# renmengye/rec-attend-public

Hardware: AMD Instinct MI355X
Metric: instance-timesteps/sec, full_model forward 512x512 T=16 (whole job; pipelined throughput: 8 batches in flight per GPU, fill and drain of the pipeline inside the timed region; config.lone_batch_* = one sync-bracketed forward) (higher is better)
Workload: dtype f32; 1 GPU; cfg2: CVPPP-arch full_model eval forward, 512x512, T=16, B=8 per GPU, y_out+s_out; arch=cvppp, H=512, W=512, T=16, batch_per_gpu=8, global_batch=8, parallelism=batch-sharded x1, no collective, ranks_in_communicator=1, hip_graph=True, tile_tickets=False, batches_in_flight=8, pipeline_slots=4, batches_per_launch=2, input=resident in HBM, output=left in HBM

## Files before the change

### include/recattend.h

```cpp
#ifndef RECATTEND_H_
#define RECATTEND_H_

#include <stddef.h>
#include <stdint.h>

#ifdef __cplusplus
extern "C" {
#endif

#define RA_E_INVALID (-1)
#define RA_E_SHAPE (-2)
#define RA_E_WORKSPACE (-3)
#define RA_E_HUNG_BFS (-12)
#define RA_E_HUNG_PATH (-13)
#define RA_E_HUNG_FLOW (-14)
#define RA_E_HUNG_EQUALIZE (-15)

#define RA_ABI_VERSION 115
int ra_version(void);
const char *ra_last_error_string(void);

int ra_debug_poison_lds(void *stream);
int ra_debug_park_xcd(int xcd, int n_wg, int lds_bytes, int millis, int *resident, void *stream);

#define RA_PLAN_INTS 24
#define RA_PLAN_FAMILY 0
#define RA_PLAN_FORM 1
#define RA_PLAN_CK 2
#define RA_PLAN_NC 3
#define RA_PLAN_WN 4
#define RA_PLAN_GX 5
#define RA_PLAN_GY 6
#define RA_PLAN_KF 7
#define RA_PLAN_TILE_H 8
#define RA_PLAN_TILE_W 9
#define RA_PLAN_TILES_X 10
#define RA_PLAN_TILES_Y 11
#define RA_PLAN_NTILES 12
#define RA_PLAN_GRID 13
#define RA_PLAN_TILES_MIN 14
#define RA_PLAN_TILES_MAX 15
#define RA_PLAN_XCD_MAP 16
#define RA_PLAN_TICKETS 17
#define RA_PLAN_CMID 18
#define RA_PLAN_SLICES 19
#define RA_PLAN_POOL 20
#define RA_PLAN_FAMILY_K1 1
#define RA_PLAN_FAMILY_CONV8 2
#define RA_PLAN_FAMILY_PAIR 3
#define RA_PLAN_FAMILY_SPLIT 4
#define RA_PLAN_FAMILY_WINO 5
#define RA_PLAN_FAMILY_PAIR_WINO 6
#define RA_PLAN_FORM_SWAP 1
#define RA_PLAN_FORM_SUBPIXEL 2
#define RA_PLAN_FORM_BF16 4
#define RA_PLAN_FORM_MOMENTS 8
#define RA_PLAN_FORM_KXK 16
#define RA_PLAN_FORM_PERSIST 32
#define RA_PLAN_FORM_NPACKED 64
#define RA_PLAN_FORM_CACHED 128
#define RA_PLAN_FORM_SPLIT 256
#define RA_PLAN_FORM_PLANE 512
int ra_conv3x3_plan(int C0, int C1, int B, int Hs, int Ws, int upsample, int KF, int Cout, int pool, int has_plane,
                    int bf16_operands, int moments, int store_flags, int *plan);
int ra_conv_pair_plan(int Cin, int B, int Hs, int Ws, int upsampleA, int CoutA, int CoutB, int poolB, int has_plane,
                      int cache_form, int *plan);
int ra_conv_split_plan(int B, int H, int W, int Cin, int Cout, int pool, int has_plane, int *plan);
int ra_conv_wino_plan(int B, int H, int W, int Cin, int Cout, int pool, int *plan);
int ra_conv_pair_wino_plan(int B, int H, int W, int *plan);
int ra_conv_pair16_plan(int B, int H, int W, int *plan);
#define RA_PASTE_PLAN_INTS 8
#define RA_PASTE_PLAN_KERNEL 0
#define RA_PASTE_PLAN_ROWS 1
#define RA_PASTE_PLAN_GRID_X 2
#define RA_PASTE_PLAN_THREADS 3
#define RA_PASTE_PLAN_LDS 4
#define RA_PASTE_KERNEL_GENERAL 1
#define RA_PASTE_KERNEL_WINDOW 2
int ra_paste_plan(int mode, int B, int H, int W, int Fh, int Fw, int Cp, int pc, int has_canvas, int has_img,
                  size_t y_stride_b, int aligned16, int *plan);

int ra_hungarian_f32(const float *weights, int B, int N, int M, float *matching,
                     float *cover_x, float *cover_y);

size_t ra_hungarian_dev_workspace_bytes(int B, int N, int M);
int ra_hungarian_f32_dev(const float *weights, int B, int N, int M, float *matching,
                         float *cover_x, float *cover_y, int *status_dev, void *ws,
                         size_t ws_bytes, void *stream);

#define RA_CONV_TRANSPOSED 1

int ra_conv_cout_padded(int Cout);
size_t ra_conv_packed_floats(int Cin, int Cout);
int ra_conv_pack_weights(const float *w, int Cin_w, int Cout, int Cin, const int *chan_map,
                         int flags, float *out);
size_t ra_conv_packed_floats_k(int KF, int Cin, int Cout);
int ra_conv_pack_weights_k(const float *w, int KF, int Cin_w, int Cout, int Cin, const int *chan_map, int flags,
                           float *out);
int ra_conv_fold_bn(const float *bias, const float *beta, const float *gamma, const float *mean,
                    const float *var, int Cout, float eps, float *scale, float *shift);

int ra_conv3x3_f32(const float *src0, int C0, const float *src1, int C1, int B, int Hs, int Ws,
                   int upsample, const float *wpacked, const float *scale, const float *shift,
                   int Cout, int relu, int pool, const float *plane, int plane_chan, float *y,
                   void *stream);

int ra_convkxk_f32(const float *src0, int C0, const float *src1, int C1, int B, int Hs, int Ws, int upsample,
                   const float *wpacked, int KF, const float *scale, const float *shift, int Cout, int relu, int pool,
                   const float *plane, int plane_chan, float *y, void *stream);

int ra_conv_wide_supported(int Cin, int Cout);
size_t ra_conv_wide_packed_floats(int Cin, int Cout);
int ra_conv_wide_pack_weights(const float *w, int Cin_w, int Cout, int Cin, const int *chan_map, int flags, float *out);
int ra_conv3x3_wide_f32(const float *src0, int C0, const float *src1, int C1, int B, int Hs, int Ws, int upsample,
                        const float *wpacked, const float *scale, const float *shift, int Cout, int relu, int pool,
                        float *y, void *stream);

int ra_fg_head_f32(const float *logits, size_t npix, int nsc, int no, int quantise, float *y_out, float *d_out,
                   const float *x, int D, float *packed, int Cp, float *canvas_plane, void *stream);

int ra_conv3x3_bf16ops_f32(const float *src0, int C0, const float *src1, int C1, int B, int Hs, int Ws,
                           int upsample, const float *wpacked, const float *scale, const float *shift,
                           int Cout, int relu, int pool, const float *plane, int plane_chan, float *y,
                           void *stream);

int ra_conv3x3_bf16_f32(const void *src0, int C0, const void *src1, int C1, int B, int Hs, int Ws, int upsample,
                        const float *wpacked, const float *scale, const float *shift, int Cout, int relu, int pool, void *y,
                        float *part, size_t part_floats, int *nparts, int store_flags, void *stream);
int ra_bn_act_pool_bf16_f32(const void *u, const float *mean, const float *var, const float *gamma, const float *beta, float eps,
                            int relu, int pool, int B, int H, int W, int C, void *y, int flags, void *stream);
int ra_bn_act_pool_bwd_acc_bf16_f32(const void *u, const void *dy, const float *mean, const float *var, const float *gamma,
                                    const float *beta, float eps, int relu, int pool, int B, int H, int W, int C, float *ws,
                                    size_t ws_floats, float *dgamma, float *dbeta, void *du, float *acc_gamma, float *acc_beta,
                                    int flags, void *stream);
int ra_bn_act_pool_bwd_grouped_bf16_f32(const void *u, const void *dy, const void *const *tabs, int G, float eps, int relu, int pool,
                                        int B, int H, int W, int C, float *ws, size_t ws_floats, float *dgamma, float *dbeta,
                                        void *du, int flags, void *stream);
int ra_conv3x3_wgrad_acc_bf16_f32(const void *x, int Cin, int B, int Hs, int Ws, int upsample, const void *du, int Cout, float *ws,
                                  size_t ws_floats, const int *chan_map, int cin_w, int transposed, float *gw, float *gb, int fmt,
                                  void *stream);

size_t ra_conv3x3_moments_part_floats(int Cout);
int ra_conv3x3_moments_f32(const float *src0, int C0, const float *src1, int C1, int B, int Hs, int Ws,
                           int upsample, const float *wpacked, const float *scale, const float *shift,
                           int Cout, int relu, int bf16_operands, float *y, float *part, size_t part_floats,
                           int *nparts, void *stream);
int ra_bn_moments_from_partials_f32(const float *part, int nparts, int C, float *mean, float *var, void *stream);

int ra_conv_pair_supported(int Cin, int CoutA, int CoutB);
int ra_conv_pair_f32(const float *src, int Cin, int B, int Hs, int Ws, int upsampleA,
                     const float *wpA, const float *scaleA, const float *shiftA, int CoutA, int reluA,
                     const float *wpB, const float *scaleB, const float *shiftB, int CoutB, int reluB,
                     int poolB, const float *plane, int plane_chan, float *y, void *stream);

int ra_conv_split_supported(int Cin, int Cout, int pool, int H, int W);
size_t ra_conv_split_packed_halfs(int Cin, int Cout);
int ra_conv_split_pack_weights(const float *w, int Cin, int Cout, unsigned short *out);
int ra_conv_split_pack_weights_dev(const float *w, int Cin, int Cout, int transposed, unsigned short *out, void *stream);
int ra_conv_split_f32(const float *x, int B, int H, int W, int Cin, const unsigned short *wpacked, const float *scale,
                      const float *shift, int Cout, int relu, int pool, float *y, void *stream);
int ra_conv_split_plane_f32(const float *x, int B, int H, int W, int Cin, const float *plane, int plane_chan,
                            const unsigned short *wpacked, const float *scale, const float *shift, int Cout, int relu, int pool,
                            float *y, void *stream);

int ra_conv_wino_supported(int Cin, int Cout, int pool, int H, int W);
size_t ra_conv_wino_packed_floats(int Cin, int Cout);
int ra_conv_wino_pack_weights(const float *w, int Cin, int Cout, float *out);
int ra_conv_wino_f32(const float *x, int B, int H, int W, int Cin, const float *wpacked,
                     const float *scale, const float *shift, int Cout, int relu, int pool, float *y,
                     void *stream);

int ra_conv_pair_wino_supported(int Cin, int CoutA, int CoutB, int poolB, int H, int W);
int ra_conv_pair_wino_f32(const float *x, int B, int H, int W, const float *wpA, const float *scaleA,
                          const float *shiftA, int reluA, const float *wpB_wino, const float *scaleB,
                          const float *shiftB, int reluB, float *y, void *stream);

int ra_conv_pair16_supported(int Cin, int CoutA, int CoutB, int poolB, int H, int W);
int ra_conv_pair16_f32(const float *x, int B, int H, int W, const float *wpA, const float *scaleA, const float *shiftA,
                       int reluA, const float *wpB, const float *scaleB, const float *shiftB, int reluB, float *y,
                       void *stream);

int ra_conv_first_cache_supported(int Cin, int CoutA, int CoutB, int poolB, int H, int W);
size_t ra_conv_first_cache_floats(int B, int H, int W);
int ra_conv_first_cache_f32(const float *src, int B, int H, int W, const float *wpA, int CoutA,
                            int plane_chan, float *cache, void *stream);
int ra_conv_pair_fill_cache_f32(const float *src, const float *plane, int plane_chan, int B, int H,
                                int W, const float *wpA, const float *scaleA, const float *shiftA,
                                int reluA, const float *wpB, const float *scaleB,
                                const float *shiftB, int CoutB, int reluB, float *cache, float *y,
                                void *stream);
int ra_conv_pair_fill_cache_rider_f32(const float *src, const float *plane, int plane_chan, int B, int H, int W,
                                      const float *wpA, const float *scaleA, const float *shiftA, int reluA,
                                      const float *wpB, const float *scaleB, const float *shiftB, int CoutB,
                                      int reluB, float *cache, float *y, float *fill_dst, size_t fill_floats,
                                      float fill_value, void *stream);
int ra_conv_pair_cached_f32(const float *cache, const float *plane, int plane_chan, int B, int H,
                            int W, const float *wpA, const float *scaleA, const float *shiftA,
                            int reluA, const float *wpB, const float *scaleB, const float *shiftB,
                            int CoutB, int reluB, float *y, void *stream);

typedef struct ra_ctrl_desc {
  int G;
  int Cf;
  int hid;
  int iters;
  int n_gmlp;
  int n_cmlp;
  int mlp_dim;
  int H, W;
  int Fh, Fw;
  int squash;
  int fixed_var;
  int dynamic_var;
  int fixed_gamma;
} ra_ctrl_desc;

size_t ra_ctrl_packed_floats(const ra_ctrl_desc *d);
int ra_ctrl_pack_weights(const ra_ctrl_desc *d, const float *const *lstm_w,
                         const float *const *gmlp_w, const float *const *cmlp_w, float *out);

#define RA_ATTN_STRIDE 16
int ra_controller_f32(const ra_ctrl_desc *d, const float *feat , const float *wpacked,
                      int B, float *h_last , float *ctrl_out ,
                      float *glimpse_maps ,
                      float *attn , void *stream);

int ra_ctrl_split_supported(const ra_ctrl_desc *d);
size_t ra_ctrl_split_packed_floats(const ra_ctrl_desc *d);
size_t ra_ctrl_split_workspace_bytes(const ra_ctrl_desc *d, int B);
int ra_ctrl_split_pack_weights(const ra_ctrl_desc *d, const float *const *lstm_w,
                               const float *const *gmlp_w, const float *const *cmlp_w, float *out);
int ra_controller_split_f32(const ra_ctrl_desc *d, const float *feat, const float *wpacked, int B,
                            float *h_last, float *ctrl_out, float *glimpse_maps, float *attn,
                            void *ws, size_t ws_bytes, int *status_dev, void *stream);
int ra_ctrl_batch_group_images(const ra_ctrl_desc *d, int B);
int ra_ctrl_batch_supported(const ra_ctrl_desc *d);
size_t ra_ctrl_batch_workspace_bytes(const ra_ctrl_desc *d, int B);
int ra_controller_batch_f32(const ra_ctrl_desc *d, const float *feat, const float *wpacked, int B,
                            float *h_last, float *ctrl_out, float *glimpse_maps, float *attn, void *ws,
                            size_t ws_bytes, int *status_dev, void *stream);
int ra_controller_batch_xcd_f32(const ra_ctrl_desc *d, const float *feat, const float *wpacked, int B,
                                float *h_last, float *ctrl_out, float *glimpse_maps, float *attn, void *ws,
                                size_t ws_bytes, int *status_dev, int xcd_offset, void *stream);

int ra_gaussian_filter_f32(const float *center, const float *size, const float *lg_var, int B,
                           int L, int F, float *out, void *stream);

int ra_extract_direct_f32(const float *img, int Ci, int chan0, const float *canvas, int canvas_chan,
                          const float *attn, int B, int H, int W, int Fh, int Fw, int Cp,
                          int use_gamma, float *patch, void *stream);
int ra_extract_conv0_supported(int Cp, int Fh, int Fw, int Cout, int pool);
int ra_extract_conv0_f32(const float *img, int Ci, int chan0, const float *canvas, int canvas_chan,
                         const float *attn_rec, int B, int H, int W, int Fh, int Fw, int use_gamma, float *patch,
                         const float *w0, const float *scale, const float *shift, int Cout, int relu, float *y0,
                         void *stream);
#define RA_PASTE_Y_PREFILLED 1
#define RA_PASTE_CANVAS_FLOORED 2
int ra_paste_direct_f32(const float *patch, int Cp, int pc, const float *attn, int B, int H, int W,
                        int Fh, int Fw, float beta, int disable_overwrite, float *canvas, float *img,
                        int Ci, int canvas_chan, float *y_out, size_t y_stride_b, int flags,
                        void *stream);
int ra_paste_score_direct_f32(const float *patch, int Cp, int pc, const float *attn, int B, int H,
                              int W, int Fh, int Fw, float beta, int disable_overwrite,
                              float *canvas, float *y_out, size_t y_stride_b, int flags,
                              const float *h, int K0, const float *core, int K1, const float *w,
                              const float *bias, float *s_out, size_t s_stride_b, void *stream);

#define RA_RESAMPLE_READ 0
#define RA_RESAMPLE_WRITE 1
#define RA_RESAMPLE_BOX 2
int ra_ctrl_train_supported(int G, int Cf, int hid, int iters, int nout);
size_t ra_ctrl_train_save_floats(int G, int Cf, int hid, int iters);
int ra_ctrl_train_fwd_f32(int B, int G, int Cf, int hid, int iters, int nout, const float *feat, const float *Wg,
                          const float *bg, const float *W0, const float *b0, const float *W1, const float *b1,
                          const float *Wc, const float *bc, float *h_last, float *co, float *save, void *stream);
int ra_ctrl_train_bwd_f32(int B, int G, int Cf, int hid, int iters, int nout, const float *feat, const float *Wg,
                          const float *W0, const float *W1, const float *Wc, const float *save, const float *dh_last,
                          const float *dco, float *dfeat, float *dpre, float *dz1, float *dlog, void *stream);
int ra_ctrl_train_supported_n(int G, int Cf, int hid, int iters, int nout, int n_glimpse, int n_ctrl, int mlp_dim);
size_t ra_ctrl_train_save_floats_n(int G, int Cf, int hid, int iters, int n_glimpse);
int ra_ctrl_train_fwd_n_f32(int B, int G, int Cf, int hid, int iters, int nout, int n_glimpse, int n_ctrl, int mlp_dim,
                            const float *feat, const float *Wg, const float *bg, const float *const *gW,
                            const float *const *gb, const float *const *cW, const float *const *cb, float *h_last,
                            float *co, float *save, float *save_c, void *stream);
int ra_ctrl_train_bwd_n_f32(int B, int G, int Cf, int hid, int iters, int nout, int n_glimpse, int n_ctrl, int mlp_dim,
                            const float *feat, const float *Wg, const float *const *gW, const float *const *cW,
                            const float *save, const float *save_c, const float *dh_last, const float *dco, float *dfeat,
                            float *dpre, float *dlog, float *dzg, size_t dzg_stride, float *dzc, size_t dzc_stride,
                            void *stream);

size_t ra_resample_bwd_workspace_floats(int B, int Fh, int C);
int ra_resample_bwd_f32(int mode, const float *X, int Cx, int chan0, int C, const float *dY, const float *Y,
                        const float *attn_rec, const float *Q, int Cq, float *E, int Ce, int B, int H, int W, int Fh,
                        int Fw, const float *scale, int scale_stride, const float *div, int div_stride, float *ws,
                        size_t ws_floats, float *out, void *stream);
int ra_attn_box_direct_f32(const float *attn, int B, int H, int W, int Fh, int Fw, float beta,
                           float *box_out, size_t stride_b, void *stream);

int ra_extract_patch_dense_f32(const float *x, const float *f_y, const float *f_x, int B, int H,
                               int W, int D, int FH, int FW, float *out, void *stream);

int ra_dense_f32(const float *x0, int K0, const float *x1, int K1, const float *W, const float *b,
                 int B, int N, int act, float *out, size_t out_stride_b, void *stream);

int ra_pack_input_f32(const float *x, int D, const float *d_in, int Dd, const float *y_in, int Dy,
                      int B, int H, int W, int Cp, float *packed, void *stream);
int ra_pack_input_plane_f32(const float *x, int D, const float *d_in, int Dd, const float *y_in, int Dy,
                            int B, int H, int W, int Cp, float *packed, float *canvas_plane, void *stream);
int ra_canvas_max_f32(float *img, int Ci, int canvas_chan, const float *ysel, const float *noise,
                      int B, int H, int W, void *stream);

int ra_affine_act_f32(const float *x, const float *scale, const float *shift, size_t npix, int C,
                      int relu, float *y, void *stream);
int ra_max_pool_f32(const float *x, int B, int H, int W, int C, int ratio, float *y, void *stream);

enum {
  RA_STAT_LOSS = 0, RA_STAT_BOX_LOSS, RA_STAT_SEGM_LOSS, RA_STAT_CONF_LOSS, RA_STAT_IOU_SOFT,
  RA_STAT_IOU_SOFT_BOX, RA_STAT_WT_COV_SOFT, RA_STAT_UNWT_COV_SOFT, RA_STAT_IOU_HARD,
  RA_STAT_WT_COV_HARD, RA_STAT_UNWT_COV_HARD, RA_STAT_DICE, RA_STAT_COUNT_ACC, RA_STAT_DIC,
  RA_STAT_DIC_ABS, RA_STAT_COUNT
};
size_t ra_pair_stats_workspace_floats(int B, int HW);
int ra_pair_stats_f32(const float *a, const float *b, int B, int N, int M, int HW, float *ws,
                      size_t ws_floats, float *iou_soft, float *iou_hard, float *dice_hard,
                      float *sum_a, float *sum_b, float *inter, float *sum_a_hard, void *stream);
int ra_pair_stats_strided_f32(const float *a, size_t a_img, size_t a_row, const float *b, int B, int N, int M, int HW, float *ws,
                              size_t ws_floats, float *iou_soft, float *iou_hard, float *dice_hard, float *sum_a, float *sum_b,
                              float *inter, float *sum_a_hard, void *stream);
size_t ra_box_iou_rects_workspace_floats(int B);
int ra_box_iou_rects_f32(const float *box, const float *params, int B, int T, int H, int W, float *ws,
                         size_t ws_floats, float *iou, void *stream);
size_t ra_gt_box_workspace_floats(int B, int T);
int ra_gt_box_f32(const float *y_gt, int B, int T, int H, int W, float padding_ratio,
                  float min_padding, float *ws, size_t ws_floats, float *params, float *box,
                  void *stream);

int ra_knob_setup_f32(const float *gt_box_ws, int B, int T, const float *pad, const float *shift, const float *u_box,
                      const float *u_segm, const float *sched, float min_padding, int timescale, float *ctr, float *size,
                      float *knob_box, float *knob_segm, void *stream);
size_t ra_segm_match_workspace_bytes(int B, int N);
int ra_segm_match_f32(const float *iou, const float *s_gt, int B, int N, void *ws, size_t ws_bytes,
                      float *match, int *status, void *stream);
size_t ra_segm_match_host_block_bytes(int B, int N);
int ra_segm_match_host_f32(const float *iou, const float *s_gt, int B, int N, float *w_dev, void *pinned, size_t pinned_bytes,
                           int threads, float *match, int *status, void *stream);
int ra_loss_stats_f32(const float *iou_soft, const float *iou_hard, const float *dice,
                      const float *match_real, const float *iou_box, const float *match_box,
                      const float *s_out, const float *s_gt, const float *sum_gt, int B, int T,
                      int fixed_order, int segm_loss_fn, float loss_mix_ratio, float *ws,
                      size_t ws_floats, float *out, void *stream);
size_t ra_loss_stats_workspace_floats(int B);

enum {
  RA_EVAL_SBD = 0, RA_EVAL_WT_COV, RA_EVAL_UNWT_COV, RA_EVAL_FG_IOU, RA_EVAL_FG_DICE, RA_EVAL_FP,
  RA_EVAL_FN, RA_EVAL_COUNT_ACC, RA_EVAL_COUNT_MSE, RA_EVAL_DIC, RA_EVAL_DIC_ABS, RA_EVAL_NUM_OBJ,
  RA_EVAL_COUNT_OUT, RA_EVAL_COUNT
};
enum {
  RA_EVALI_OBJ_PR = 0, RA_EVALI_OBJ_RE, RA_EVALI_PIX_PR, RA_EVALI_PIX_RE, RA_EVALI_HAS_OUT,
  RA_EVALI_IS_GT, RA_EVALI_COUNT
};
int ra_postprocess_f32(const float *y_out, const float *s_out, int B, int T, int H, int W,
                       float thresh, const float *fg, float *y_bin, float *s_hard,
                       float *union_out, void *stream);
int ra_union_f32(const float *y, int B, int T, int HW, float *union_out, void *stream);
int ra_dilate_f32(const float *y, int N, int H, int W, int radius, float *out, void *stream);
int ra_resize_linear_f32(const float *y, int N, int Hs, int Ws, int H, int W, float *out, void *stream);
int ra_bilateral5_f32(const float *y, int N, int H, int W, float sigma_color, float sigma_space, float *out, void *stream);
int ra_remove_tiny_f32(float *y_bin, const float *sizes, float *conf, int B, int T, int HW,
                       float threshold, void *stream);
int ra_eval_metrics_f32(const float *inter, const float *sum_a, const float *sum_b,
                        const float *s_gt, const float *fg_inter, const float *fg_a,
                        const float *fg_b, const float *a_in_fgb, const float *b_in_fga, int B,
                        int T, float *iou_pairwise, float *stats, float *inst, void *stream);

int ra_random_transform_f32(const float *x, int N, int H, int W, int C, int padding, int off_y,
                            int off_x, int flip_v, int flip_h, int transpose, float *out,
                            void *stream);
size_t ra_colour_jitter_workspace_floats(int B);
int ra_colour_jitter_f32(const float *x, int B, int HW, float hue_delta, float saturation_factor, float brightness_delta,
                         float contrast_factor, float *ws, size_t ws_floats, float *out, void *stream);

int ra_weighted_sum_f32(const float *w, const float *y, int B, int T, int HW, float *out,
                        void *stream);

int ra_sem_foreground_f32(const float *sem, int B, int Hs, int Ws, int C, int H, int W, float thresh, float *fg,
                          void *stream);
size_t ra_instance_class_vote_workspace_floats(int B, int T, int H, int W, int C);
int ra_instance_class_vote_f32(const float *y, const float *sem, int B, int T, int H, int W, int Hs, int Ws, int C,
                               const float *conf, float *ws, size_t ws_floats, float *vote, int *class_idx,
                               int *label_id, void *stream);
int ra_instance_class_pick_f32(const float *vote, const float *conf, int B, int T, int C, int *class_idx, int *label_id,
                               void *stream);

int ra_label_vote_sweep_f32(const float *y, const unsigned char *labels, const unsigned char *lut, int B, int T, int H,
                            int W, const double *thresholds, int K, const float *conf_in, int remove_tiny, int *counts,
                            int *sizes, unsigned char *keep, float *conf, float *vote, int *class_idx, int *label_id,
                            void *stream);
int ra_label_planes_f32(const float *y, const unsigned char *labels, const unsigned char *lut, int B, int T, int H, int W,
                        double thresh, const unsigned char *keep, float *y_bin, void *stream);

#define RA_OVERLAP_MAX_GT 256
#define RA_GT_STATUS_RANGE 1
#define RA_GT_STATUS_COUNT 2
size_t ra_gt_instance_catalog_workspace_ints(int B, int H, int W);
int ra_gt_instance_catalog_i32(const int *gt_ids, int B, int H, int W, int *ws, size_t ws_ints, int *ids, int *pixels,
                               int *count, int *status, void *stream);
size_t ra_instance_overlap_workspace_ints(int B, int T, int H, int W);
int ra_instance_overlap_f32(const float *y, const int *gt_ids, const int *ids, const int *count, int B, int T, int H, int W,
                            int *ws, size_t ws_ints, int *inter, int *pred_pixels, void *stream);

#define RA_PIXEL_LABELS 34
#define RA_PIXEL_TILE 1024
#define RA_PIXEL_STATUS_GT 1
#define RA_PIXEL_STATUS_PRED 2
int ra_sem_labels_u8(const float *sem, int B, int Hs, int Ws, int C, int H, int W, unsigned char *labels, void *stream);
size_t ra_pixel_confusion_workspace_ints(int B, int H, int W);
int ra_pixel_confusion_u8(const unsigned char *pred, const int *gt_ids, const unsigned char *gt_labels, const int *ids,
                          const int *count, int B, int H, int W, int *ws, size_t ws_ints, unsigned long long *conf,
                          int *inst_tp, int *inst_cat_tp, int *status, void *stream);
int ra_pixel_confusion_sem_f32(const float *sem, int Hs, int Ws, int C, const int *gt_ids, const unsigned char *gt_labels,
                               const int *ids, const int *count, int B, int H, int W, int *ws, size_t ws_ints,
                               unsigned long long *conf, int *inst_tp, int *inst_cat_tp, int *status, void *stream);

#define RA_LABELS_PLAIN 0
#define RA_LABELS_CITYSCAPES 1
#define RA_LABELS_MAX_T 32
size_t ra_labels_workspace_bytes(int B, int H, int W);
int ra_labels_assemble_i32(const int *gt_ids, const int *ids, const int *count, int B, int Hf, int Wf, int H, int W, int T,
                           int dataset, void *ws, size_t ws_bytes, int *num_obj, float *s_gt, int *inst_id, int *area,
                           int *sem_cls, float *y_gt, unsigned char *d_cls, float *d_gt, float *c_gt,
                           unsigned char *fg_gt_full, void *stream);

int ra_resize_cubic_tables(int S, int D, int *ofs, short *coef);
int ra_resize_cubic_u8(const unsigned char *src, int N, int Hs, int Ws, int C, int H, int W, const int *ofs_y,
                       const short *coef_y, const int *ofs_x, const short *coef_x, unsigned char *dst_u8, float *dst_f32,
                       void *stream);
int ra_png_unfilter_u8(const unsigned char *raw, int H, int stride, int bpp, unsigned char *out);

#define RA_RENDER_ADD 0
#define RA_RENDER_FIRST 1
#define RA_RENDER_MAX_T 1024
int ra_render_instances_u8(const float *y, int B, int T, int H, int W, const unsigned char *colour, int mode,
                           unsigned char *img, void *stream);
int ra_render_orientation_u8(const float *d, int B, int Hs, int Ws, int C, const float *mask, int H, int W,
                             const unsigned char *wheel, unsigned char *img, void *stream);

#define RA_PNG_GRAY8 0
#define RA_PNG_BGR8 1
#define RA_PNG_F32 2
#define RA_PNG_MAX_ROW_BYTES 24576
#define RA_PNG_MAX_IMAGES 65535
int ra_png_deflate_bound(int N, int H, int W, int bpp, unsigned long long *stream_bytes, unsigned long long *workspace_bytes);
int ra_png_deflate_u8(const void *src, int kind, int M, int N, int H, int W, const int *plane, unsigned char *out,
                      size_t out_bytes, int *sizes, unsigned long long *offsets, unsigned int *adler, void *ws, size_t ws_bytes,
                      void *stream);
int ra_png_deflate_host(const void *src, int kind, int M, int N, int H, int W, const int *plane, unsigned char *out,
                        size_t out_bytes, int *sizes, unsigned long long *offsets, unsigned int *adler, void *ws,
                        size_t ws_bytes);

#define RA_FG_STAT_INTER_SOFT 0
#define RA_FG_STAT_SUM_SOFT 1
#define RA_FG_STAT_SUM_GT 2
#define RA_FG_STAT_INTER_HARD 3
#define RA_FG_STAT_SUM_HARD 4
#define RA_FG_STAT_SEG_CE 5
#define RA_FG_STAT_ORI_CE 6
#define RA_FG_STAT_ORI_CORRECT 7
#define RA_FG_STAT_MASK 8
#define RA_FG_STAT_COUNT 9
#define RA_FG_SWEEP_MAX_K 16
#define RA_FG_SWEEP_SLOTS 33
size_t ra_fg_stats_workspace_bytes(size_t npix);
int ra_fg_stats_f32(const float *logits, const float *y_gt, const float *d_gt, size_t npix, int nsc, int no, void *ws,
                    size_t ws_bytes, double *sums, void *stream);
int ra_fg_sweep_counts_f32(const float *src, const unsigned char *gt, int N, int Hs, int Ws, int H, int W,
                           const float *thresholds, int K, unsigned long long *counts, void *stream);

#define RA_INS_EVAL_MAX_K 16
int ra_instance_eval_counts_f32(const float *yc, const int *gt_ids, const int *inst_id, const unsigned char *fg, int B, int T,
                                int Hs, int Ws, int Hf, int Wf, int morph, const float *thresholds, int K, int *inter,
                                int *area_b, void *stream);

typedef struct ra_image_geo {
  long long offset;
  int h;
  int w;
} ra_image_geo;
size_t ra_gt_instance_catalog_ragged_workspace_ints(const ra_image_geo *geo, int B);
int ra_gt_instance_catalog_ragged_i32(const int *gt_ids, size_t total, const ra_image_geo *geo, ra_image_geo *geo_dev, int B,
                                      int *ws, size_t ws_ints, int *ids, int *pixels, int *count, int *status, void *stream);
int ra_labels_assemble_ragged_i32(const int *gt_ids, size_t total, const ra_image_geo *geo, ra_image_geo *geo_dev,
                                  const int *ids, const int *count, int B, int H, int W, int T, int dataset, void *ws,
                                  size_t ws_bytes, int *num_obj, float *s_gt, int *inst_id, int *area, int *sem_cls, float *y_gt,
// ... 181 lines not shown
```

### rec-attend-public_amd/csrc/ra_conv_pair.hip

```cpp
#include <cstdlib>

#include "ra_conv_pair_parts.h"
#include "ra_split3.h"

namespace ra {
namespace cpair {

template <int CINA, int CMID, int NCB, int GX, int GYB>
struct PGeo {
  static constexpr int NCA = (CMID + 15) / 16;
  static constexpr int TWB = 8 * GX, THB = 8 * GYB, PMB = GX * GYB;
  static constexpr int GXA = GX + 1, GRA = THB / 2 + 1, NGA = GXA * GRA;
  static constexpr int AW = 8 * GXA, AH = 2 * GRA;
  static constexpr int LWA = AW + 2, LHA = AH + 2;
  static constexpr int NCGA = CINA / 4, CKA = CINA < 16 ? CINA : 16, NCHA = CINA / CKA, NCGAC = CKA / 4;
  static constexpr int NCGB = CMID / 4, CKB = CMID < 16 ? CMID : 16, NCHB = CMID / CKB, NCGBC = CKB / 4;
  static constexpr int KSA = 9 * NCGAC, KSB = 9 * NCGBC;
  static constexpr int IN_FLOATS = LHA * LWA * CINA;
  static constexpr int MID_FLOATS = AH * AW * CMID;
  static constexpr int RA = 4;
  static constexpr int GPW = (NGA + 3) / 4;
  static constexpr int ROUNDS = (GPW + RA - 1) / RA;
  typedef typename vec_of<NCGAC>::type avecA;
  typedef typename vec_of<NCGBC>::type avecB;
// ... 227 lines not shown
                &tin[gbase[j] + (ky * G::LWA + kx) * CINA + ch * G::NCGAC]);
#pragma unroll
          for (int cg = 0; cg < G::NCGAC; ++cg)
#pragma unroll
            for (int j = 0; j < G::RA; ++j)
#pragma unroll
              for (int n = 0; n < NCA; ++n)
                acc[j][n] = __builtin_amdgcn_mfma_f32_16x16x4f32(av[j][cg], bregA[tap * G::NCGAC + cg][n],
                                                                 acc[j][n], 0, 0, 0);
        }
      }
      const bool interior = (ty0 >= 1) & (ty0 - 1 + G::AH <= a.H) & (tx0 >= 1) & (tx0 + G::TWB + 1 <= a.W);
      const float loA = a.reluA ? 0.f : -__builtin_inff();
#pragma unroll
      for (int j = 0; j < G::RA; ++j) {
        const bool live = (wave + 4 * (rd * G::RA + j)) < G::NGA;
#pragma unroll
        for (int n = 0; n < NCA; ++n) {
          const int co = 16 * n + co_lane;
          float o[4];
#pragma unroll
          for (int r = 0; r < 4; ++r) o[r] = fmaxf(acc[j][n][r] * scA[n] + shA[n], loA);
          if (!interior) {
#pragma unroll
            for (int r = 0; r < 4; ++r) {
              const int Y = ty0 - 1 + 2 * gr[j] + (r >> 1), X = tx0 - 1 + 8 * gc[j] + 2 * qo + (r & 1);
              o[r] = ((Y >= 0) & (Y < a.H) & (X >= 0) & (X < a.W)) ? o[r] : 0.f;
            }
          }
          if (live && co < CMID) {
            float *dst = tmid + ((2 * gr[j]) * G::AW + 8 * gc[j] + 2 * qo) * CMID + (co & 3) * G::NCGB + (co >> 2);
#pragma unroll
            for (int r = 0; r < 4; ++r) dst[((r >> 1) * G::AW + (r & 1)) * CMID] = o[r];
          }
        }
      }
    }
  }
  __syncthreads();

  {
    f32x4 acc[G::PMB][NCB];
#pragma unroll
    for (int g = 0; g < G::PMB; ++g)
#pragma unroll
      for (int n = 0; n < NCB; ++n) acc[g][n] = f32x4{0.f, 0.f, 0.f, 0.f};
    const int a_base = ((wave * 2 * GYB + dy) * G::AW + 2 * q + dx) * CMID + ksub * G::NCGB;
    float bregB[G::KSB][NCB];
    for (int ch = 0; ch < G::NCHB; ++ch) {
      {
        const float *wrow = a.wpB + ((size_t)ch * G::KSB * 4 + ksub) * a.CoutBP + co_lane;
#pragma unroll
        for (int s = 0; s < G::KSB; ++s)
#pragma unroll
          for (int n = 0; n < NCB; ++n) bregB[s][n] = wrow[(size_t)s * 4 * a.CoutBP + 16 * n];
      }
#pragma unroll
      for (int tap = 0; tap < 9; ++tap) {
        const int ky = tap / 3, kx = tap % 3;
        avecB av[G::PMB];
#pragma unroll
        for (int g = 0; g < G::PMB; ++g) {
          const int gx = g % GX, gy = g / GX;
          av[g] = *reinterpret_cast<const avecB *>(
              &tmid[a_base + ((2 * gy + ky) * G::AW + 8 * gx + kx) * CMID + ch * G::NCGBC]);
        }
#pragma unroll
        for (int cg = 0; cg < G::NCGBC; ++cg)
#pragma unroll
          for (int g = 0; g < G::PMB; ++g)
#pragma unroll
            for (int n = 0; n < NCB; ++n)
              acc[g][n] = __builtin_amdgcn_mfma_f32_16x16x4f32(av[g][cg], bregB[tap * G::NCGBC + cg][n],
                                                               acc[g][n], 0, 0, 0);
      }
    }
    G::phase_b_store(a, wave, co_lane, qo, b, ty0, tx0, acc);
  }
}

template <int CINA, int CMID, int NCB, int GX, int GYB>
__global__ __launch_bounds__(256) void conv_pair_persist_mfma(const PArgs a, int tiles_x, int tiles_y, int ntiles) {
  using G = PGeo<CINA, CMID, NCB, GX, GYB>;
  constexpr int NCA = G::NCA;
  extern __shared__ __attribute__((aligned(16))) float lds[];
  float *tin = lds;
  float *tmid = lds + G::IN_FLOATS;

  const int tid = threadIdx.x, lane = tid & 63;
  const int wave = __builtin_amdgcn_readfirstlane(tid >> 6);
  const int m = lane & 15, ksub = lane >> 4;
  const int q = m >> 2, dy = (m >> 1) & 1, dx = m & 1;
  const int co_lane = lane & 15, qo = lane >> 4;
  const int per = tiles_x * tiles_y;
  static_assert(G::NCHA == 1 && G::NCHB == 1, "persistent pair: single-chunk layers");
  float scA[NCA], shA[NCA];
#pragma unroll
  for (int n = 0; n < NCA; ++n) {
    scA[n] = a.scA[16 * n + co_lane];
    shA[n] = a.shA[16 * n + co_lane];
  }
  float bregA[G::KSA][NCA], bregB[G::KSB][NCB];
  {
    const float *wrow = a.wpA + (size_t)ksub * a.CoutAP + co_lane;
#pragma unroll
    for (int s = 0; s < G::KSA; ++s)
#pragma unroll
      for (int n = 0; n < NCA; ++n) bregA[s][n] = wrow[(size_t)s * 4 * a.CoutAP + 16 * n];
    const float *wrowb = a.wpB + (size_t)ksub * a.CoutBP + co_lane;
#pragma unroll
    for (int s = 0; s < G::KSB; ++s)
#pragma unroll
      for (int n = 0; n < NCB; ++n) bregB[s][n] = wrowb[(size_t)s * 4 * a.CoutBP + 16 * n];
  }
  constexpr int NPIXA = G::LHA * G::LWA, NIT = (NPIXA + 255) / 256;
  const __amdgpu_buffer_rsrc_t rs = __builtin_amdgcn_make_buffer_rsrc(const_cast<float *>(a.src), 0, a.bytes0, 0x00020000);
  int e_r[NIT], e_c[NIT];
#pragma unroll
  for (int i = 0; i < NIT; ++i) {
    const int e = tid + 256 * i;
    e_r[i] = e / G::LWA - 2;
    e_c[i] = e % G::LWA - 2;
    if (e >= NPIXA) e_r[i] = -(1 << 20);
  }
  f32x4 pre[NIT][G::NCGA];
  auto fetch = [&](int T) {
    const int fb = T / per, fr = T - fb * per;
    const int fy0 = (fr / tiles_x) * G::THB, fx0 = (fr % tiles_x) * G::TWB;
#pragma unroll
    for (int i = 0; i < NIT; ++i) {
      const int Y = fy0 + e_r[i], X = fx0 + e_c[i];
      const bool ok = (Y >= 0) & (Y < a.H) & (X >= 0) & (X < a.W);
      const int off = ok ? (((fb * a.Hs + Y) * a.Ws + X) * a.C0) * 4 : 0x7fffffff;
#pragma unroll
      for (int cg = 0; cg < G::NCGA; ++cg)
        pre[i][cg] = __builtin_bit_cast(f32x4, __builtin_amdgcn_raw_buffer_load_b128(rs, off, 16 * cg, 0));
    }
  };
  int tile = blockIdx.x;
  if (tile < ntiles) fetch(tile);
  for (; tile < ntiles; tile += gridDim.x) {
    const int b = tile / per;
    const int trem = tile - b * per;
    const int ty0 = (trem / tiles_x) * G::THB, tx0 = (trem % tiles_x) * G::TWB;

#pragma unroll
    for (int i = 0; i < NIT; ++i) {
      const int e = tid + 256 * i;
      if (e < NPIXA) G::write_record(tin + e * CINA, pre[i]);
    }
    __syncthreads();
    {
      const int next = tile + gridDim.x;
      if (next < ntiles) fetch(next);
    }

    {
      const int lane_in = (dy * G::LWA + 2 * q + dx) * CINA + ksub * G::NCGA;
      G::phase_a(a, wave, lane_in, co_lane, qo, ty0, tx0, tin, tmid, scA, shA, bregA);
    }
    __syncthreads();

    {
      f32x4 acc[G::PMB][NCB];
#pragma unroll
      for (int g = 0; g < G::PMB; ++g)
#pragma unroll
        for (int n = 0; n < NCB; ++n) acc[g][n] = f32x4{0.f, 0.f, 0.f, 0.f};
      const int a_base = ((wave * 2 * GYB + dy) * G::AW + 2 * q + dx) * CMID + ksub * G::NCGB;
      G::phase_b_taps(tmid, a_base, 0, bregB, acc);
      G::phase_b_store(a, wave, co_lane, qo, b, ty0, tx0, acc);
    }
  }
}

template <int CINA, int CMID, int NCB, int GX, int GYB>
int launch(const PArgs &a, int B, hipStream_t st, int *plan) {
  using G = PGeo<CINA, CMID, NCB, GX, GYB>;
  auto kern = conv_pair_mfma<CINA, CMID, NCB, GX, GYB>;
  constexpr size_t lds = (size_t)(G::IN_FLOATS + G::MID_FLOATS) * sizeof(float);
  static_assert(lds <= 160 * 1024, "pair tile does not fit LDS");
  const int tiles_x = ceil_div(a.W, G::TWB), tiles_y = ceil_div(a.H, G::THB);
  const int ntiles = tiles_x * tiles_y * B;
  if (plan) {
    plan[RA_PLAN_FAMILY] = RA_PLAN_FAMILY_PAIR;
    plan[RA_PLAN_CK] = CINA, plan[RA_PLAN_CMID] = CMID, plan[RA_PLAN_NC] = NCB, plan[RA_PLAN_GX] = GX, plan[RA_PLAN_GY] = GYB;
    plan[RA_PLAN_KF] = 3, plan[RA_PLAN_TILE_H] = G::THB, plan[RA_PLAN_TILE_W] = G::TWB;
    plan[RA_PLAN_TILES_X] = tiles_x, plan[RA_PLAN_TILES_Y] = tiles_y, plan[RA_PLAN_NTILES] = ntiles;
    plan[RA_PLAN_GRID] = ntiles, plan[RA_PLAN_TILES_MIN] = plan[RA_PLAN_TILES_MAX] = 1;
    if (!(G::NCHA == 1 && G::NCHB == 1) || a.ups || a.plane) return 0;
    if (!plan_have_device()) {
      plan[RA_PLAN_GRID] = plan[RA_PLAN_TILES_MIN] = plan[RA_PLAN_TILES_MAX] = -1;
      return 0;
    }
  } else {
    static const MaxDynamicLds lds_limit(kern, lds);
  }
  if constexpr (G::NCHA == 1 && G::NCHB == 1) {
    static const int pers = env_int("RA_PAIR_PERSIST", 1);
    static const int cap = wgs_per_cu(conv_pair_persist_mfma<CINA, CMID, NCB, GX, GYB>, lds) * cu_count();
    if (pers && !a.ups && !a.plane && ntiles > cap && a.bytes0 > 0) {
      if (plan) {
        plan[RA_PLAN_FORM] = RA_PLAN_FORM_PERSIST;
        plan_walk(plan, ntiles, cap, 0);
        return 0;
      }
      hipLaunchKernelGGL((conv_pair_persist_mfma<CINA, CMID, NCB, GX, GYB>), dim3(cap), dim3(256), lds, st, a, tiles_x,
                         tiles_y, ntiles);
      return launch_status("ra_conv_pair_f32");
    }
  }
  if (plan) return 0;
  hipLaunchKernelGGL(kern, dim3(ntiles), dim3(256), lds, st, a, tiles_x, tiles_y);
  return launch_status("ra_conv_pair_f32");
}

template <int CINA, int CMID, int NCB>
int dispatch_geo(const PArgs &a, int B, hipStream_t st, int *plan) {
  using Big = PGeo<CINA, CMID, NCB, 4, 2>;
  constexpr bool big_fits = (size_t)(Big::IN_FLOATS + Big::MID_FLOATS) * 4 <= 80 * 1024;
  const bool narrow = (a.W % 32 != 0) && (a.W % 32 <= 16);
  auto wgs = [&](int gx, int gyb) { return (long)ceil_div(a.W, 8 * gx) * ceil_div(a.H, 8 * gyb) * B; };
  static const int force = env_int("RA_PAIR_GEO", 0);
  constexpr bool single_chunk = Big::NCHA == 1 && Big::NCHB == 1;
  if (!force && single_chunk && !a.ups && !a.plane && !narrow && wgs(4, 1) >= 2048)
    return launch<CINA, CMID, NCB, 4, 1>(a, B, st, plan);
  if constexpr (big_fits) {
    if (force == 42 || (!force && !narrow && wgs(4, 2) >= 512)) return launch<CINA, CMID, NCB, 4, 2>(a, B, st, plan);
  }
  if (force == 41 || (!force && !narrow)) return launch<CINA, CMID, NCB, 4, 1>(a, B, st, plan);
  if (force == 22 || (!force && wgs(2, 2) >= 512)) return launch<CINA, CMID, NCB, 2, 2>(a, B, st, plan);
  return launch<CINA, CMID, NCB, 2, 1>(a, B, st, plan);
}

template <int CINA, int CMID>
int dispatch_b(const PArgs &a, int B, hipStream_t st, int *plan) {
  if (a.CoutBP == 16) return dispatch_geo<CINA, CMID, 1>(a, B, st, plan);
  if (a.CoutBP == 32) return dispatch_geo<CINA, CMID, 2>(a, B, st, plan);
  return fail(RA_E_SHAPE, "ra_conv_pair_f32: CoutB %d unsupported", a.CoutB);
}

template <int CINA>
int dispatch_mid(const PArgs &a, int cmid, int B, hipStream_t st, int *plan) {
  switch (cmid) {
    case 8: return dispatch_b<CINA, 8>(a, B, st, plan);
    case 16: return dispatch_b<CINA, 16>(a, B, st, plan);
    case 32: return dispatch_b<CINA, 32>(a, B, st, plan);
    default: return fail(RA_E_SHAPE, "ra_conv_pair_f32: CoutA %d unsupported", cmid);
  }
}

}
}

using namespace ra;

extern "C" int ra_conv_pair_supported(int Cin, int CoutA, int CoutB) {
  const bool cin_ok = Cin == 4 || Cin == 8 || Cin == 16 || Cin == 32;
  const bool mid_ok = CoutA == 8 || CoutA == 16 || CoutA == 32;
  return cin_ok && mid_ok && CoutB >= 1 && CoutB <= 32;
}

static int pair_entry(const float *src, int Cin, int B, int Hs, int Ws, int upsampleA, const float *wpA, const float *scaleA,
                      const float *shiftA, int CoutA, int reluA, const float *wpB, const float *scaleB, const float *shiftB,
                      int CoutB, int reluB, int poolB, const float *plane, int plane_chan, float *y, void *stream, int *plan) {
  if (cpair::missing_pointer(plan, {src, wpA, scaleA, shiftA, wpB, scaleB, shiftB, y}) || B <= 0 || Hs <= 0 || Ws <= 0)
    return fail(RA_E_INVALID, "ra_conv_pair_f32: bad argument");
  if (!ra_conv_pair_supported(Cin, CoutA, CoutB))
    return fail(RA_E_SHAPE, "ra_conv_pair_f32: Cin=%d CoutA=%d CoutB=%d", Cin, CoutA, CoutB);
  if (poolB != 1 && poolB != 2) return fail(RA_E_SHAPE, "ra_conv_pair_f32: pool %d", poolB);
  cpair::PArgs a = cpair::pair_args(src, Cin, B, Hs, Ws, upsampleA, wpA, scaleA, shiftA, CoutA, reluA, wpB, scaleB, shiftB, CoutB, reluB,
                                    poolB, plane, plane_chan, y);
  if (poolB == 2 && ((a.H | a.W) & 1)) return fail(RA_E_SHAPE, "ra_conv_pair_f32: odd size with pool 2");
  if (plane && (plane_chan < 0 || plane_chan >= Cin)) return fail(RA_E_INVALID, "ra_conv_pair_f32: plane channel");
  hipStream_t st = as_stream(stream);
  const size_t bytes0 = (size_t)B * Hs * Ws * Cin * 4;
  a.bytes0 = (int)bytes0;
  static int no8 = -1;
  if (no8 < 0) no8 = getenv("RA_PAIR_NO8") ? 1 : 0;
  if (!no8 && (Cin == 4 || Cin == 8) && CoutA == 8 && CoutB <= 8 && poolB == 2 && !a.ups && bytes0 < (1u << 31) && a.W > 16)
    return cpair::launch_npacked(a, B, st, plan);
  switch (Cin) {
    case 4: return cpair::dispatch_mid<4>(a, CoutA, B, st, plan);
    case 8: return cpair::dispatch_mid<8>(a, CoutA, B, st, plan);
    case 16: return cpair::dispatch_mid<16>(a, CoutA, B, st, plan);
    default: return cpair::dispatch_mid<32>(a, CoutA, B, st, plan);
  }
}

extern "C" int ra_conv_pair_f32(const float *src, int Cin, int B, int Hs, int Ws, int upsampleA,
                                const float *wpA, const float *scaleA, const float *shiftA, int CoutA,
                                int reluA, const float *wpB, const float *scaleB, const float *shiftB,
                                int CoutB, int reluB, int poolB, const float *plane, int plane_chan,
                                float *y, void *stream) {
  return pair_entry(src, Cin, B, Hs, Ws, upsampleA, wpA, scaleA, shiftA, CoutA, reluA, wpB, scaleB, shiftB, CoutB, reluB, poolB, plane,
                    plane_chan, y, stream, nullptr);
}

extern "C" int ra_conv_pair_plan(int Cin, int B, int Hs, int Ws, int upsampleA, int CoutA, int CoutB, int poolB, int has_plane,
                                 int cache_form, int *plan) {
  if (!plan) return fail(RA_E_INVALID, "ra_conv_pair_plan: bad argument");
  for (int i = 0; i < RA_PLAN_INTS; ++i) plan[i] = 0;
  static float mark;
  if (cache_form == 1)
    return cpair::fill_cache_entry(nullptr, &mark, 3, B, Hs, Ws, nullptr, nullptr, nullptr, 0, nullptr, nullptr, nullptr, CoutB, 0, nullptr, nullptr,
                                   nullptr, 0, 0.0f, nullptr, plan);
  if (cache_form == 2)
    return cpair::cached_entry(nullptr, &mark, 3, B, Hs, Ws, nullptr, nullptr, nullptr, 0, nullptr, nullptr, nullptr, CoutB, 0, nullptr, nullptr, plan);
  if (cache_form) return fail(RA_E_INVALID, "ra_conv_pair_plan: cache_form %d", cache_form);
  return pair_entry(nullptr, Cin, B, Hs, Ws, upsampleA, nullptr, nullptr, nullptr, CoutA, 0, nullptr, nullptr, nullptr, CoutB, 0, poolB,
                    has_plane ? &mark : nullptr, has_plane ? 0 : -1, nullptr, nullptr, plan);
}
```

### rec-attend-public_amd/csrc/ra_conv_pair16.hip

```cpp
#include "ra_common.h"
#include "ra_split3.h"

#ifndef RA_PAIR16_OCC
#define RA_PAIR16_OCC 3
#endif
namespace ra {
namespace cpair {

constexpr int P16_TSY = 8, P16_TS = 16;
constexpr int P16_WS = P16_TS + 2;
constexpr int P16_AWY = P16_TSY + 2;
constexpr int P16_IWY = P16_TSY + 4, P16_IWX = P16_TS + 4;
constexpr int P16_WST = 24;
constexpr int P16_PLI = P16_IWY * P16_IWX * 16;
constexpr int P16_PLW = P16_AWY * P16_WST * 32;
constexpr int P16_WB = 5 * 3 * 64 * 16;
constexpr size_t P16_LDS = 3 * (size_t)(P16_PLI + P16_PLW) + P16_WB;

struct P16Args {
  const float *x, *wpA, *scA, *shA, *wpB, *scB, *shB;
  float *y;
  int B, H, W, CoutAP, CoutBP, reluA, reluB;
  int bytes_x;
  int xcd_map;
  unsigned *tickets;
};

struct P16Walk {
  int first, end, step;
};
__device__ inline P16Walk p16_tile_walk(int ntiles, int xcd_map) {
  P16Walk w;
  if (!xcd_map) {
    w.first = blockIdx.x;
    w.end = ntiles;
    w.step = gridDim.x;
    return w;
  }
  const int chunk = (ntiles + 7) >> 3, x = blockIdx.x & 7;
  w.first = x * chunk + ((int)blockIdx.x >> 3);
  w.end = (x * chunk + chunk < ntiles) ? x * chunk + chunk : ntiles;
  w.step = (int)gridDim.x >> 3;
  return w;
}

#ifdef RA_PROBE16
__device__ long long *ra_probe16_buf;
#define RA_PHASE_PROBE_BUF ra_probe16_buf
#define RA_PHASE_PROBE_WG blockIdx.x
#endif
#include "ra_phase_probe.h"

__global__ __launch_bounds__(256, RA_PAIR16_OCC) void conv_pair16_mfma(const P16Args a, int tiles_x, int tiles_y, int ntiles) {
  constexpr int TSY = P16_TSY, TS = P16_TS, WS = P16_WS, AWY = P16_AWY, IWX = P16_IWX, WST = P16_WST, CINA = 8;
  constexpr int NPA = AWY * WS, NGA = (NPA + 15) / 16, GPW = (NGA + 3) / 4;
  constexpr int NPI = P16_IWY * IWX, NIT = (NPI * 2 + 255) / 256;
  constexpr int PLI = P16_PLI, PLW = P16_PLW;
  static_assert(NGA == 4 * GPW, "layer A's groups divide among the four waves");
  __shared__ unsigned tk_sh[2];
  TicketWalk tk;
  const bool dyn = a.tickets != nullptr;
  if (dyn) tk.issue(a.tickets, ntiles);
  extern __shared__ __attribute__((aligned(16))) unsigned char lds16[];
  unsigned char *tinp = lds16;
  unsigned char *twin = lds16 + 3 * PLI;
  unsigned char *twb = twin + 3 * PLW;
  const int tid = threadIdx.x, lane = tid & 63;
  const int p = __builtin_amdgcn_readfirstlane(tid >> 6);
  const int m = lane & 15, ksub = lane >> 4;
  const int per = tiles_x * tiles_y;

  s16x8 wA[3][3];
  const float scA = a.scA[m];
#pragma unroll
  for (int blk = 0; blk < 3; ++blk) {
    const int tap = 4 * blk + ksub;
    const bool ok = tap < 9;
    const int tp = ok ? tap : 0;
#pragma unroll
    for (int j = 0; j < 8; j += 2) {
      const float w0 = a.wpA[(size_t)((tp * 2 + (j >> 2)) * 4 + (j & 3)) * a.CoutAP + m];
      const float w1 = a.wpA[(size_t)((tp * 2 + ((j + 1) >> 2)) * 4 + ((j + 1) & 3)) * a.CoutAP + m];
      unsigned H, M, L;
      split3_pair(ok ? w0 * scA : 0.f, ok ? w1 * scA : 0.f, H, M, L);
      wA[blk][0][j] = (short)(H & 0xffffu), wA[blk][0][j + 1] = (short)(H >> 16);
      wA[blk][1][j] = (short)(M & 0xffffu), wA[blk][1][j + 1] = (short)(M >> 16);
      wA[blk][2][j] = (short)(L & 0xffffu), wA[blk][2][j + 1] = (short)(L >> 16);
    }
  }
  f32x4 shA4;
#pragma unroll
  for (int j = 0; j < 4; ++j) shA4[j] = a.shA[4 * ksub + j];
  const float loA = a.reluA ? 0.f : -__builtin_inff();
  {
    const float scB = a.scB[m];
#pragma unroll
    for (int blk = 0; blk < 5; ++blk) {
      if ((blk & 3) != p) continue;
      const int tap = 2 * blk + (ksub >> 1);
      const bool ok = tap < 9;
      const int tp = ok ? tap : 0;
      s16x8 w[3];
#pragma unroll
      for (int j = 0; j < 8; j += 2) {
        const int c = 8 * (ksub & 1) + j;
        const float w0 = a.wpB[(size_t)((tp * 4 + (c >> 2)) * 4 + (c & 3)) * a.CoutBP + m];
        const float w1 = a.wpB[(size_t)((tp * 4 + ((c + 1) >> 2)) * 4 + ((c + 1) & 3)) * a.CoutBP + m];
        unsigned H, M, L;
        split3_pair(ok ? w0 * scB : 0.f, ok ? w1 * scB : 0.f, H, M, L);
        w[0][j] = (short)(H & 0xffffu), w[0][j + 1] = (short)(H >> 16);
        w[1][j] = (short)(M & 0xffffu), w[1][j + 1] = (short)(M >> 16);
        w[2][j] = (short)(L & 0xffffu), w[2][j + 1] = (short)(L >> 16);
      }
#pragma unroll
      for (int pc = 0; pc < 3; ++pc) *reinterpret_cast<s16x8 *>(twb + ((blk * 3 + pc) * 64 + lane) * 16) = w[pc];
    }
  }
  const float shB = a.shB[m];
  const float loB = a.reluB ? 0.f : -__builtin_inff();
  const int Ho = a.H / 2, Wo = a.W / 2;

  int ain[GPW], aout[GPW];
#pragma unroll
  for (int s = 0; s < GPW; ++s) {
    const int li = 16 * (p + 4 * s) + m;
    const int lc = li < NPA ? li : NPA - 1;
    const int r = lc / WS, c = lc - r * WS;
    ain[s] = (r * IWX + c) * 16;
    aout[s] = li < NPA ? (r * WST + c) * 32 + (((ksub >> 1) ^ (r & 1)) * 16) + (ksub & 1) * 8 : -1;
  }
  const int pr = (m >> 1) & 1;
  const int bin = ((2 * p + pr) * WST + 2 * (m >> 2) + (m & 1)) * 32;
  int toffB[5];
#pragma unroll
  for (int blk = 0; blk < 5; ++blk) {
    const int tap = 2 * blk + (ksub >> 1) < 9 ? 2 * blk + (ksub >> 1) : 8;
    const int ky = tap / 3, kx = tap - 3 * ky;
    toffB[blk] = (ky * WST + kx) * 32 + (((ksub & 1) ^ ((pr + ky) & 1)) * 16);
  }

  const __amdgpu_buffer_rsrc_t rx = __builtin_amdgcn_make_buffer_rsrc(const_cast<float *>(a.x), 0, a.bytes_x, 0x00020000);
  f32x4 pre[NIT];
  auto fetch = [&](int T) {
    const int fb = T / per, fr = T - fb * per;
    const int fy0 = (fr / tiles_x) * TSY - 2, fx0 = (fr % tiles_x) * TS - 2;
#pragma unroll
    for (int i = 0; i < NIT; ++i) {
      const int e = tid + 256 * i, cg = e & 1, pix = e >> 1;
      const int r = pix / IWX, c = pix - r * IWX;
      const int Y = fy0 + r, X = fx0 + c;
      const bool ok = (e < NPI * 2) & (Y >= 0) & (Y < a.H) & (X >= 0) & (X < a.W);
      const int off = ok ? (((fb * a.H + Y) * a.W + X) * CINA + 4 * cg) * 4 : 0x7fffffff;
      pre[i] = __builtin_bit_cast(f32x4, __builtin_amdgcn_raw_buffer_load_b128(rx, off, 0, 0));
    }
  };

  const P16Walk tw = p16_tile_walk(ntiles, a.xcd_map);
  int tile = tw.first, tnext = 0;
  const int t_end = dyn ? ntiles : tw.end;
  if (dyn) {
    tk.begin(tk_sh);
    tile = tk.cur >= 0 ? tk.cur : t_end;
  }
  if (tile < t_end) fetch(tile);
  RA_PHASE_DECL;
  for (; tile < t_end; tile = tnext) {
    const int b = tile / per, trem = tile - b * per;
    const int ty = trem / tiles_x, tx = trem - ty * tiles_x;
    RA_PHASE_AT(0);
#pragma unroll
    for (int i = 0; i < NIT; ++i) {
      const int e = tid + 256 * i, cg = e & 1, pix = e >> 1;
      unsigned H0, M0, L0, H1, M1, L1;
      split3_pair(pre[i].x, pre[i].y, H0, M0, L0);
      split3_pair(pre[i].z, pre[i].w, H1, M1, L1);
      if (e < NPI * 2) {
        unsigned char *rec = tinp + pix * 16 + cg * 8;
        *reinterpret_cast<u32x2 *>(rec) = u32x2{H0, H1};
        *reinterpret_cast<u32x2 *>(rec + PLI) = u32x2{M0, M1};
        *reinterpret_cast<u32x2 *>(rec + 2 * PLI) = u32x2{L0, L1};
      }
    }
    if (dyn) tk.publish(tk_sh);
    __syncthreads();
    RA_PHASE_AT(1);
    if (dyn) {
      tk.read_next(tk_sh);
      tk.request();
      tk.step();
      tnext = tk.cur >= 0 ? tk.cur : t_end;
    } else {
      tnext = tile + tw.step;
    }
    if (tnext < t_end) fetch(tnext);

    {
      const int oyA = ty * TSY - 1, oxA = tx * TS - 1;
      const bool interior = (oyA >= 0) & (oyA + AWY <= a.H) & (oxA >= 0) & (oxA + WS <= a.W);
      f32x4 acc[GPW];
#pragma unroll
      for (int s = 0; s < GPW; ++s) acc[s] = shA4;
      const int t0 = ksub, t1 = 4 + ksub, t2 = 8;
      const int toff[3] = {((t0 / 3) * IWX + t0 % 3) * 16, ((t1 / 3) * IWX + t1 % 3) * 16, ((t2 / 3) * IWX + t2 % 3) * 16};
      constexpr int PA[6] = {1, 0, 2, 0, 1, 0}, PB[6] = {1, 2, 0, 1, 0, 0};
#pragma unroll
      for (int blk = 0; blk < 3; ++blk)
#pragma unroll
        for (int s = 0; s < GPW; ++s) {
          s16x8 av[3];
#pragma unroll
          for (int pc = 0; pc < 3; ++pc) av[pc] = *reinterpret_cast<const s16x8 *>(tinp + ain[s] + toff[blk] + pc * PLI);
#pragma unroll
          for (int t = 0; t < 6; ++t)
            acc[s] = __builtin_amdgcn_mfma_f32_16x16x32_bf16(__builtin_bit_cast(bf16x8, wA[blk][PB[t]]), __builtin_bit_cast(bf16x8, av[PA[t]]),
                                                             acc[s], 0, 0, 0);
        }
      RA_PHASE_AT(2);
#pragma unroll
      for (int s = 0; s < GPW; ++s) {
        f32x4 o = acc[s];
#pragma unroll
        for (int j = 0; j < 4; ++j) o[j] = fmaxf(o[j], loA);
        if (!interior) {
          const int li = 16 * (p + 4 * s) + m;
          const int wr = li / WS, wc = li - wr * WS;
          const int Y = oyA + wr, X = oxA + wc;
          const bool ok = (Y >= 0) & (Y < a.H) & (X >= 0) & (X < a.W);
#pragma unroll
          for (int j = 0; j < 4; ++j) o[j] = ok ? o[j] : 0.f;
        }
        unsigned H01, M01, L01, H23, M23, L23;
        split3_pair(o[0], o[1], H01, M01, L01);
        split3_pair(o[2], o[3], H23, M23, L23);
        if (aout[s] >= 0) {
          unsigned char *d = twin + aout[s];
          *reinterpret_cast<u32x2 *>(d) = u32x2{H01, H23};
          *reinterpret_cast<u32x2 *>(d + PLW) = u32x2{M01, M23};
          *reinterpret_cast<u32x2 *>(d + 2 * PLW) = u32x2{L01, L23};
        }
      }
    }
    RA_PHASE_AT(3);
    __syncthreads();
    RA_PHASE_AT(4);

    {
      f32x4 acc[2];
#pragma unroll
      for (int u = 0; u < 2; ++u) acc[u] = f32x4{shB, shB, shB, shB};
      constexpr int PA[6] = {1, 0, 2, 0, 1, 0}, PB[6] = {1, 2, 0, 1, 0, 0};
#pragma unroll
      for (int blk = 0; blk < 5; ++blk) {
        s16x8 av[2][3], wB[3];
#pragma unroll
        for (int pc = 0; pc < 3; ++pc) wB[pc] = *reinterpret_cast<const s16x8 *>(twb + ((blk * 3 + pc) * 64 + lane) * 16);
#pragma unroll
        for (int u = 0; u < 2; ++u)
#pragma unroll
          for (int pc = 0; pc < 3; ++pc) av[u][pc] = *reinterpret_cast<const s16x8 *>(twin + bin + u * 8 * 32 + toffB[blk] + pc * PLW);
#pragma unroll
        for (int t = 0; t < 6; ++t)
#pragma unroll
          for (int u = 0; u < 2; ++u)
            acc[u] = __builtin_amdgcn_mfma_f32_16x16x32_bf16(__builtin_bit_cast(bf16x8, av[u][PA[t]]), __builtin_bit_cast(bf16x8, wB[PB[t]]),
                                                             acc[u], 0, 0, 0);
      }
      RA_PHASE_AT(5);
      const int oty = ty * (TSY / 2) + p;
#pragma unroll
      for (int u = 0; u < 2; ++u) {
        const float best = fmaxf(fmaxf(fmaxf(acc[u][0], acc[u][1]), fmaxf(acc[u][2], acc[u][3])), loB);
        const int otx = tx * (TS / 2) + 4 * u + ksub;
        a.y[((size_t)(b * Ho + oty) * Wo + otx) * 16 + m] = best;
      }
      RA_PHASE_AT(6);
    }
  }
  RA_PHASE_END;
}

int launch_pair16(const P16Args &a, hipStream_t st, int *plan) {
  auto kern = conv_pair16_mfma;
  static const int resident = wgs_per_cu(kern, P16_LDS) * cu_count();
  static const int wgs = env_int("RA_PAIR16_WGS", 0);
  static const int cap = wgs > 0 ? wgs : resident;
  const int tiles_x = a.W / P16_TS, tiles_y = a.H / P16_TSY, ntiles = tiles_x * tiles_y * a.B;
  const int grid = ntiles < cap ? ntiles : cap;
  P16Args a2 = a;
  a2.xcd_map = (grid % 8 == 0 && grid >= 8) ? 1 : 0;
  const bool draws = ntiles >= 2 * kTicketMinTilesPerWg * grid;
  if (plan) {
    plan[RA_PLAN_FAMILY] = RA_PLAN_FAMILY_PAIR, plan[RA_PLAN_FORM] = RA_PLAN_FORM_SPLIT | RA_PLAN_FORM_PERSIST;
    plan[RA_PLAN_CK] = 8, plan[RA_PLAN_CMID] = 16, plan[RA_PLAN_NC] = 1, plan[RA_PLAN_KF] = 3, plan[RA_PLAN_POOL] = 2, plan[RA_PLAN_SLICES] = 1;
    plan[RA_PLAN_TILE_H] = P16_TSY, plan[RA_PLAN_TILE_W] = P16_TS, plan[RA_PLAN_TILES_X] = tiles_x, plan[RA_PLAN_TILES_Y] = tiles_y;
    plan[RA_PLAN_TICKETS] = draws ? 1 : 0;
    plan_walk(plan, ntiles, grid, a2.xcd_map);
    return 0;
  }
  a2.tickets = draws ? take_ticket_slots(1, grid) : nullptr;
  hipLaunchKernelGGL(kern, dim3(grid), dim3(256), P16_LDS, st, a2, tiles_x, tiles_y, ntiles);
  return launch_status("ra_conv_pair16_f32");
}

}
}

using namespace ra;

extern "C" int ra_conv_pair16_supported(int Cin, int CoutA, int CoutB, int poolB, int H, int W) {
  return Cin == 8 && CoutA == 16 && CoutB == 16 && poolB == 2 && H > 0 && W > 0 && H % 16 == 0 && W % 16 == 0;
}

static int pair16_entry(const float *x, int B, int H, int W, const float *wpA, const float *scaleA, const float *shiftA, int reluA,
                        const float *wpB, const float *scaleB, const float *shiftB, int reluB, float *y, void *stream, int *plan) {
  if ((!plan && (!x || !wpA || !scaleA || !shiftA || !wpB || !scaleB || !shiftB || !y)) || B <= 0)
    return fail(RA_E_INVALID, "ra_conv_pair16_f32: bad argument");
  if (!ra_conv_pair16_supported(8, 16, 16, 2, H, W)) return fail(RA_E_SHAPE, "ra_conv_pair16_f32: %dx%d", H, W);
  const size_t bytes = (size_t)B * H * W * 8 * sizeof(float);
  if (bytes >= (1ull << 31)) return fail(RA_E_SHAPE, "ra_conv_pair16_f32: input exceeds 2 GiB");
  cpair::P16Args a{};
  a.x = x;
  a.wpA = wpA;
  a.scA = scaleA;
  a.shA = shiftA;
  a.wpB = wpB;
  a.scB = scaleB;
  a.shB = shiftB;
  a.y = y;
  a.B = B;
  a.H = H;
  a.W = W;
  a.CoutAP = a.CoutBP = ra_conv_cout_padded(16);
  a.reluA = reluA;
  a.reluB = reluB;
  a.bytes_x = (int)bytes;
  a.xcd_map = 0;
  return cpair::launch_pair16(a, as_stream(stream), plan);
}

extern "C" int ra_conv_pair16_f32(const float *x, int B, int H, int W, const float *wpA, const float *scaleA, const float *shiftA,
                                  int reluA, const float *wpB, const float *scaleB, const float *shiftB, int reluB, float *y,
                                  void *stream) {
  return pair16_entry(x, B, H, W, wpA, scaleA, shiftA, reluA, wpB, scaleB, shiftB, reluB, y, stream, nullptr);
}

extern "C" int ra_conv_pair16_plan(int B, int H, int W, int *plan) {
  if (!plan) return fail(RA_E_INVALID, "ra_conv_pair16_plan: bad argument");
  for (int i = 0; i < RA_PLAN_INTS; ++i) plan[i] = 0;
  if (!plan_have_device()) return fail(RA_E_INVALID, "ra_conv_pair16_plan: the grid follows the device's CU count and occupancy: no device");
  return pair16_entry(nullptr, B, H, W, nullptr, nullptr, nullptr, 0, nullptr, nullptr, nullptr, 0, nullptr, nullptr, plan);
}
```

### rec-attend-public_amd/csrc/ra_conv_pair8.hip

```cpp
#include <type_traits>

#include "ra_conv_pair_parts.h"
#include "ra_split3.h"

namespace ra {
namespace cpair {

template <int CINA>
struct NGeo {
  static constexpr int TH = 16, TW = 32;
  static constexpr int NCGA = CINA / 4;
  static constexpr int AW = 41, AHS = TH + 2;
  static constexpr int LW = 43, LH = 22;
  static constexpr int NGA = 21, GPW = 5, NSLOT = GPW + 1, AR = AHS, AP = TW / 2 + 2;
  struct Cell {
    int row, pair;
    bool live;
  };
  static constexpr __host__ __device__ int group_of(int wave, int s) { return s < 4 ? 4 * s + wave : s == 4 ? 16 + wave : 20; }
  static constexpr __host__ __device__ Cell cell(int wave, int s, int m) {
    if (s < 4) return Cell{4 * s + (m >> 2), 4 * wave + (m & 3), true};
    if (s == 4) return wave < 2 ? Cell{8 * wave + (m >> 1), 16 + (m & 1), true} : Cell{16 + (m >> 3), 8 * (wave - 2) + (m & 7), true};
    return Cell{16 + ((m >> 1) & 1), 16 + (m & 1), m < 4};
  }
  static constexpr bool map_exact() {
    int hits[AR * AP] = {};
    bool seen[NGA] = {};
    for (int s = 0; s < NSLOT; ++s)
      for (int w = 0; w < (s == GPW ? 1 : 4); ++w) {
        const int g = group_of(w, s);
        if (g < 0 || g >= NGA || seen[g]) return false;
        seen[g] = true;
        for (int m = 0; m < 16; ++m) {
          const Cell c = cell(w, s, m);
          if (c.row < 0 || c.row >= AR || c.pair < 0 || c.pair >= AP) return false;
          if (c.live) ++hits[c.row * AP + c.pair];
        }
      }
    for (int g = 0; g < NGA; ++g)
      if (!seen[g]) return false;
    for (int i = 0; i < AR * AP; ++i)
      if (hits[i] != 1) return false;
    return true;
  }
  static_assert(AR * AP == 324 && NGA * 16 - 12 == AR * AP, "18 rows x 18 pairs = 21 groups less the corner's 12 spare rows");
  static constexpr int LHL = TH + 4, LWL = TW + 6;
  static_assert(AR - 1 + 2 < LHL && 2 * (AP - 1) + 3 < LWL && LHL <= LH && LWL <= LW, "every cell's 3 x 4 window is staged");
  static constexpr int PLANE_B = AHS * AW * 16;
  template <bool CACHED>
  static constexpr int tin_floats() {
    return (LH * LW * (CACHED ? 1 : CINA) + 3) & ~3;
  }
  template <bool SPLIT>
  static constexpr int tmid_floats() {
    return SPLIT ? 3 * PLANE_B / 4 : AHS * AW * 8;
  }
  template <bool CACHED, bool SPLIT>
  static constexpr int lds_floats() {
    return tin_floats<CACHED>() + tmid_floats<SPLIT>();
  }
};
static_assert(NGeo<4>::map_exact() && NGeo<8>::map_exact(), "phase A's groups cover the 18 x 18 pair-rows exactly once");

#ifndef RA_PAIR8_OCC
#define RA_PAIR8_OCC 3
#endif
#ifdef RA_PROBE8
__device__ long long *ra_probe8_buf;
#define RA_PHASE_PROBE_BUF ra_probe8_buf
#define RA_PHASE_PROBE_WG blockIdx.x
#endif
#include "ra_phase_probe.h"
#ifdef RA_P8_NOBAR
#define RA_P8_SYNC() __builtin_amdgcn_s_waitcnt(0xc07f)
#else
#define RA_P8_SYNC() __syncthreads()
#endif
template <int CINA, bool CACHED, bool SPLIT = false>
__global__ __launch_bounds__(256, CACHED ? (SPLIT ? 3 : 4) : RA_PAIR8_OCC) void conv_pair8_mfma(const PArgs a, int tiles_x, int tiles_y, int ntiles) {
  using G = NGeo<CINA>;
  constexpr int NCGA = G::NCGA;
  static_assert(!CACHED || CINA == 4, "cached form: 4 input channels");
  static_assert(!SPLIT || CACHED, "the split-precision layer B exists for the cached (steady-state) form");
  constexpr int PLANE_B = G::PLANE_B;
  constexpr int RECA = CACHED ? 1 : CINA;
  extern __shared__ __attribute__((aligned(16))) float lds[];
  constexpr int IN_FLOATS = G::template tin_floats<CACHED>();
  float *tin = lds;
  float *tmid = lds + IN_FLOATS;
  typedef typename vec_of<NCGA>::type avecA;

  const int tid = threadIdx.x, lane = tid & 63;
  __shared__ unsigned tk_sh[2];
  TicketWalk tk;
  const bool dyn = a.tickets != nullptr;
  if (dyn) tk.issue(a.tickets, ntiles);
  const int wave = __builtin_amdgcn_readfirstlane(tid >> 6);
  const int m = lane & 15, ksub = lane >> 4;
  const int n = lane & 15, qo = lane >> 4;
  const int p = n >> 3, co = n & 7;
  const int per = tiles_x * tiles_y;

  const float scA = a.scA[co], scB = a.scB[co], shB = a.shB[co];
  const float loA = a.reluA ? 0.f : -__builtin_inff(), loB = a.reluB ? 0.f : -__builtin_inff();
  const int pA = ksub >> 1, coA0 = 4 * (ksub & 1);
  f32x4 scA4, shA4;
#pragma unroll
  for (int j = 0; j < 4; ++j) scA4[j] = a.scA[coA0 + j], shA4[j] = a.shA[coA0 + j];
  const bool fill = !CACHED && a.cache != nullptr;
  float bA[CACHED ? 1 : 12][NCGA], bB[12][2];
  float bAc[3];
#pragma unroll
  for (int ky = 0; ky < 3; ++ky) {
    const int kx = ksub - p;
    const bool ok = (kx >= 0) & (kx <= 2);
    const int tap = ok ? ky * 3 + kx : 0;
    const float w = a.wpA[((tap * NCGA + (a.plane_chan >> 2)) * 4 + (a.plane_chan & 3)) * a.CoutAP + co];
    bAc[ky] = (CACHED && ok) ? w * scA : 0.f;
  }
#pragma unroll
  for (int ky = 0; ky < 3; ++ky)
#pragma unroll
    for (int kxp = 0; kxp < 4; ++kxp) {
      const int kx = kxp - p;
      const bool ok = (kx >= 0) & (kx <= 2);
      const int tap = ok ? ky * 3 + kx : 0;
      if constexpr (!CACHED) {
#pragma unroll
        for (int cg = 0; cg < NCGA; ++cg) {
          const float w = a.wpA[((tap * NCGA + cg) * 4 + ksub) * a.CoutAP + co];
          bA[ky * 4 + kxp][cg] = ok ? w * (fill ? 1.f : scA) : 0.f;
        }
      }
#pragma unroll
      for (int cg = 0; cg < 2; ++cg) {
        const float w = a.wpB[((tap * 2 + cg) * 4 + ksub) * a.CoutBP + co];
        bB[ky * 4 + kxp][cg] = ok ? w * scB : 0.f;
      }
    }

  s16x8 wB[SPLIT ? 3 : 1][SPLIT ? 3 : 1];
  if constexpr (SPLIT) {
#pragma unroll
    for (int ky = 0; ky < 3; ++ky) {
      const int kx = ksub - p;
      const bool ok = (kx >= 0) & (kx <= 2);
      const int tap = ok ? ky * 3 + kx : 0;
#pragma unroll
      for (int j = 0; j < 8; j += 2) {
        const float w0 = a.wpB[((tap * 2 + (j >> 2)) * 4 + (j & 3)) * a.CoutBP + co];
        const float w1 = a.wpB[((tap * 2 + ((j + 1) >> 2)) * 4 + ((j + 1) & 3)) * a.CoutBP + co];
        unsigned H, M, L;
        split3_pair(ok ? w0 * scB : 0.f, ok ? w1 * scB : 0.f, H, M, L);
        wB[ky][0][j] = (short)(H & 0xffffu), wB[ky][0][j + 1] = (short)(H >> 16);
        wB[ky][1][j] = (short)(M & 0xffffu), wB[ky][1][j + 1] = (short)(M >> 16);
        wB[ky][2][j] = (short)(L & 0xffffu), wB[ky][2][j + 1] = (short)(L >> 16);
      }
    }
  }
  const __amdgpu_buffer_rsrc_t rs = __builtin_amdgcn_make_buffer_rsrc(const_cast<float *>(a.src), 0, a.bytes0, 0x00020000);
  const __amdgpu_buffer_rsrc_t rp = __builtin_amdgcn_make_buffer_rsrc(
      const_cast<float *>(a.plane ? a.plane : a.src), 0, a.plane ? a.bytes_p : 0, 0x00020000);
  constexpr int NE = G::LHL * G::LWL, NIT = (NE + 255) / 256;
  int e_rr[NIT], e_cc[NIT];
#pragma unroll
  for (int i = 0; i < NIT; ++i) {
    const int e = tid + 256 * i;
    e_rr[i] = e / G::LWL;
    e_cc[i] = e - e_rr[i] * G::LWL;
    if (e >= NE) e_rr[i] = -(1 << 20);
  }
  unsigned e_offp[NIT], e_offs[NIT];
#pragma unroll
  for (int i = 0; i < NIT; ++i) {
    const bool in = tid + 256 * i < NE;
    const unsigned o = (unsigned)(e_rr[i] * a.W + e_cc[i]) * 4u;
    e_offp[i] = in ? o : 0x80000000u;
    e_offs[i] = in ? o * CINA : 0x80000000u;
  }
  struct TC {
    int b, ty, tx;
  };
  auto split = [&](int t) {
    TC c;
    c.b = t / per;
    const int r = t - c.b * per;
    c.ty = r / tiles_x;
    c.tx = r - c.ty * tiles_x;
    return c;
  };
  const int nwx = a.xcd_map ? (int)gridDim.x >> 3 : (int)gridDim.x;
  const int chunk = (ntiles + 7) >> 3;
  const int t_first = a.xcd_map ? ((int)blockIdx.x & 7) * chunk + ((int)blockIdx.x >> 3) : (int)blockIdx.x;
  const int t_end = a.xcd_map ? (((int)blockIdx.x & 7) * chunk + chunk < ntiles ? ((int)blockIdx.x & 7) * chunk + chunk : ntiles) : ntiles;
  const TC stride = split(nwx);
  auto advance = [&](TC c) {
    c.tx += stride.tx;
    if (c.tx >= tiles_x) {
      c.tx -= tiles_x;
      ++c.ty;
    }
    c.ty += stride.ty;
    if (c.ty >= tiles_y) {
      c.ty -= tiles_y;
      ++c.b;
    }
    c.b += stride.b;
    return c;
  };
  f32x4 v[NIT][NCGA];
  float pv[NIT];
  auto fetch = [&](const TC &c) {
    const int fb = c.b, fy0 = c.ty * G::TH - 2, fx0 = c.tx * G::TW - 3;
    const bool inside = (fy0 >= 0) & (fy0 + G::LHL <= a.H) & (fx0 >= 0) & (fx0 + G::LWL <= a.W);
    if (inside) {
      const unsigned base = (unsigned)((fb * a.H + fy0) * a.W + fx0) * 4u;
#pragma unroll
      for (int i = 0; i < NIT; ++i) {
        if constexpr (!CACHED) {
#pragma unroll
          for (int cg = 0; cg < NCGA; ++cg)
            v[i][cg] = __builtin_bit_cast(
                f32x4, __builtin_amdgcn_raw_buffer_load_b128(rs, (int)(base * CINA + e_offs[i] + 16u * cg), 0, 0));
        }
        pv[i] = __builtin_bit_cast(float, __builtin_amdgcn_raw_buffer_load_b32(rp, (int)(base + e_offp[i]), 0, 0));
      }
      return;
    }
#pragma unroll
    for (int i = 0; i < NIT; ++i) {
      const int Y = fy0 + e_rr[i], X = fx0 + e_cc[i];
      const bool ok = (Y >= 0) & (Y < a.H) & (X >= 0) & (X < a.W);
      const int pix = (fb * a.H + Y) * a.W + X;
      if constexpr (!CACHED) {
#pragma unroll
        for (int cg = 0; cg < NCGA; ++cg)
          v[i][cg] = __builtin_bit_cast(
              f32x4, __builtin_amdgcn_raw_buffer_load_b128(rs, ok ? (pix * CINA + 4 * cg) * 4 : 0x7fffffff, 0, 0));
      }
      pv[i] = __builtin_bit_cast(float, __builtin_amdgcn_raw_buffer_load_b32(rp, ok ? pix * 4 : 0x7fffffff, 0, 0));
    }
  };

  const __amdgpu_buffer_rsrc_t rc = __builtin_amdgcn_make_buffer_rsrc(
      const_cast<float *>(a.cache ? a.cache : a.src), 0, a.cache ? a.bytes_c : 0, 0x00020000);
  const int lane_b = ((m & 1) * G::AW + 2 * (m >> 1) + 1) * 8 + ksub * 2;
  const int pg = a.plane_chan >> 2, slot = a.plane_chan & 3;

  struct LaneCell {
    int in, c, pix;
  };
  auto lane_cell = [&](int s, int mm) {
    const typename G::Cell c = G::cell(wave, s, mm);
    return LaneCell{(c.row * G::LW + 2 * c.pair) * RECA + ksub * (CACHED ? 1 : NCGA),
                    (c.row * a.cache_gx + (c.pair >> 2)) * 256 + (c.pair & 3) * 64 + ksub * 16, c.row * G::AW + 2 * c.pair + pA};
  };
  auto lane_rowcol = [&](int s) {
    int mm = m;
    asm volatile("" : "+v"(mm));
    const typename G::Cell c = G::cell(wave, s, mm);
    return c.row | (2 * c.pair + pA) << 8;
  };
  const LaneCell cell_i = lane_cell(0, m), cell_s = lane_cell(G::GPW - 1, m);
  auto corner_cell = [&]() {
    int mm = m;
    asm volatile("" : "+v"(mm));
    return lane_cell(G::GPW, mm);
  };
  const int rows4_c = 4 * a.cache_gx * 256;
  const __amdgpu_buffer_rsrc_t ry = __builtin_amdgcn_make_buffer_rsrc(a.y, 0, a.bytes_y, 0x00020000);
  const unsigned lane_y = co < a.CoutB ? (unsigned)(((2 * qo + p) * a.CoutB + co) * 4) : 0x80000000u;
  int g_y[4];
#pragma unroll
  for (int g = 0; g < 4; ++g) g_y[g] = ((g >> 1) * a.Wo + 8 * (g & 1)) * a.CoutB * 4;

  int tile = t_first;
  if (dyn) {
    tk.begin(tk_sh);
    tile = tk.cur;
  }
  bool have = dyn ? tile >= 0 : tile < t_end;
  TC cur = split(have ? tile : 0), nxt = cur;
  if (have) fetch(cur);
  RA_PHASE_DECL;
  for (int e = tid; e < G::template lds_floats<CACHED, SPLIT>() / 4; e += 256)
    reinterpret_cast<f32x4 *>(lds)[e] = f32x4{0.f, 0.f, 0.f, 0.f};
  __syncthreads();
  const bool rider = !CACHED && a.rider_dst != nullptr;
  const __amdgpu_buffer_rsrc_t rr = __builtin_amdgcn_make_buffer_rsrc(rider ? a.rider_dst : a.y, 0,
                                                                       rider ? a.rider_quads * 16 : 0, 0x00020000);
  const int r_chunk = rider ? (a.rider_quads + (int)gridDim.x - 1) / (int)gridDim.x : 0;
  int r_idx = (int)blockIdx.x * r_chunk + tid;
  const int r_end = ((int)blockIdx.x + 1) * r_chunk < a.rider_quads ? ((int)blockIdx.x + 1) * r_chunk : a.rider_quads;
  const int my_tiles = t_end > t_first ? (t_end - t_first + nwx - 1) / nwx : 1;
  const int r_per_tile = (r_chunk + 256 * my_tiles - 1) / (256 * my_tiles);
  const u32x4 r_bits = __builtin_bit_cast(u32x4, f32x4{a.rider_val, a.rider_val, a.rider_val, a.rider_val});
  bool have_n = false;
  f32x4 cpre[CACHED ? G::NSLOT : 1];
  LaneCell cell_c{};
  auto load_cache = [&](const TC &tc, bool own) {
    const int tile_c0 = ((tc.b * a.cache_rows + tc.ty * G::TH) * a.cache_gx + ((tc.tx * G::TW) >> 3)) * 256;
#pragma unroll
    for (int s = 0; s < (CACHED ? G::GPW : 1); ++s)
      cpre[s] = __builtin_bit_cast(f32x4, __builtin_amdgcn_raw_buffer_load_b128(
                                              rc, tile_c0 + (s < 4 ? s * rows4_c + cell_i.c : cell_s.c), 0, 0));
    if constexpr (CACHED)
      if (own) {
        cell_c = corner_cell();
        cpre[G::GPW] = __builtin_bit_cast(f32x4, __builtin_amdgcn_raw_buffer_load_b128(rc, tile_c0 + cell_c.c, 0, 0));
      }
  };
  for (; have; tile = dyn ? (tk.step(), tk.cur) : tile + nwx, cur = nxt, have = have_n) {
    const int b = cur.b, ty0 = cur.ty * G::TH, tx0 = cur.tx * G::TW;
    const bool own = wave == (tile & 3);
    if constexpr (CACHED) load_cache(cur, own);

#pragma unroll
    for (int i = 0; i < NIT; ++i) {
      if constexpr (CACHED) {
        if (e_rr[i] >= 0) tin[e_rr[i] * G::LW + e_cc[i]] = pv[i];
        continue;
      }
      if (a.plane) {
#pragma unroll
        for (int cg = 0; cg < NCGA; ++cg) {
          v[i][cg].x = (cg == pg && slot == 0) ? pv[i] : v[i][cg].x;
          v[i][cg].y = (cg == pg && slot == 1) ? pv[i] : v[i][cg].y;
          v[i][cg].z = (cg == pg && slot == 2) ? pv[i] : v[i][cg].z;
          v[i][cg].w = (cg == pg && slot == 3) ? pv[i] : v[i][cg].w;
        }
      }
      if (e_rr[i] >= 0) {
        float *rec = tin + (e_rr[i] * G::LW + e_cc[i]) * CINA;
        if constexpr (NCGA == 1) {
          *reinterpret_cast<f32x4 *>(rec) = v[i][0];
        } else {
#pragma unroll
          for (int ks = 0; ks < 4; ++ks)
#pragma unroll
            for (int cg = 0; cg < NCGA; ++cg) rec[ks * NCGA + cg] = v[i][cg][ks];
        }
      }
    }
    if (dyn) tk.publish(tk_sh);
    RA_P8_SYNC();
    RA_PHASE_AT(0);
    if (dyn) {
      tk.read_next(tk_sh);
      tk.request();
      have_n = tk.nxt >= 0;
      nxt = split(have_n ? tk.nxt : 0);
    } else {
      have_n = tile + nwx < t_end;
      nxt = advance(cur);
    }
    if (have_n) fetch(nxt);
    if constexpr (!CACHED) {
      if (rider)
        for (int u = 0; u < r_per_tile; ++u, r_idx += 256)
          __builtin_amdgcn_raw_buffer_store_b128(r_bits, rr, r_idx < r_end ? r_idx * 16 : 0x7fffffff, 0, 0);
    }

    {
      const bool interior = (ty0 >= 1) & (ty0 + G::TH + 1 <= a.H) & (tx0 >= 2) & (tx0 + G::TW + 1 <= a.W);
      const int tile_c = ((b * a.cache_rows + ty0) * a.cache_gx + (tx0 >> 3)) * 256;
      auto groups = [&](auto s0c, auto s1c, const LaneCell &edge, int rowcol_i, int rowcol_e) __attribute__((always_inline)) {
        constexpr int S0 = decltype(s0c)::value, NS = decltype(s1c)::value - S0;
        f32x4 acc[NS];
        int gin[NS];
#pragma unroll
        for (int s = 0; s < NS; ++s) gin[s] = S0 + s < 4 ? cell_i.in + 4 * (S0 + s) * G::LW * RECA : edge.in;
#pragma unroll
        for (int s = 0; s < NS; ++s) {
          if constexpr (CACHED) {
            acc[s] = cpre[S0 + s] * scA4 + shA4;
          } else {
            acc[s] = fill ? f32x4{0.f, 0.f, 0.f, 0.f} : shA4;
          }
        }
        if constexpr (S0 == 0) RA_PHASE_AT(1);
        if constexpr (CACHED) {
#pragma unroll
          for (int ky = 0; ky < 3; ++ky) {
            float av[NS];
#pragma unroll
            for (int s = 0; s < NS; ++s) av[s] = tin[gin[s] + ky * G::LW];
#pragma unroll
            for (int s = 0; s < NS; ++s)
              acc[s] = __builtin_amdgcn_mfma_f32_16x16x4f32(bAc[ky], av[s], acc[s], 0, 0, 0);
          }
        } else {
#pragma unroll
          for (int ky = 0; ky < 3; ++ky)
#pragma unroll
            for (int kxp = 0; kxp < 4; ++kxp) {
              avecA av[NS];
#pragma unroll
              for (int s = 0; s < NS; ++s)
                av[s] = *reinterpret_cast<const avecA *>(&tin[gin[s] + (ky * G::LW + kxp) * CINA]);
#pragma unroll
              for (int cg = 0; cg < NCGA; ++cg)
#pragma unroll
                for (int s = 0; s < NS; ++s)
                  acc[s] = __builtin_amdgcn_mfma_f32_16x16x4f32(bA[ky * 4 + kxp][cg], av[s][cg], acc[s], 0, 0, 0);
            }
        }
#pragma unroll
        for (int s = 0; s < NS; ++s) {
          const int S = S0 + s < 4 ? S0 + s : 0;
          const bool inner = S0 + s < 4;
          const bool live = S0 + s < G::GPW || m < 4;
          if (fill) {
            const int off = live ? tile_c + (inner ? S * rows4_c + cell_i.c : edge.c) : 0x7fffffff;
            __builtin_amdgcn_raw_buffer_store_b128(__builtin_bit_cast(__attribute__((ext_vector_type(4))) unsigned, acc[s]), rc, off, 0, 0);
            acc[s] = acc[s] * scA4 + shA4;
          }
          float o[4];
#pragma unroll
          for (int j = 0; j < 4; ++j) o[j] = fmaxf(acc[s][j], loA);
          if (!interior) {
            const int rowcol = inner ? rowcol_i + 4 * S : rowcol_e;
            const int Y = ty0 - 1 + (rowcol & 255), X = tx0 - 2 + (rowcol >> 8);
            const bool ok = (Y >= 0) & (Y < a.H) & (X >= 0) & (X < a.W);
#pragma unroll
            for (int j = 0; j < 4; ++j) o[j] = ok ? o[j] : 0.f;
          }
          const int pix = inner ? cell_i.pix + 4 * S * G::AW : edge.pix;
          if constexpr (SPLIT) {
            unsigned H01, M01, L01, H23, M23, L23;
            split3_pair(o[0], o[1], H01, M01, L01);
            split3_pair(o[2], o[3], H23, M23, L23);
            if (live) {
              unsigned char *d0 = reinterpret_cast<unsigned char *>(tmid) + pix * 16 + coA0 * 2;
              *reinterpret_cast<u32x2 *>(d0) = u32x2{H01, H23};
              *reinterpret_cast<u32x2 *>(d0 + PLANE_B) = u32x2{M01, M23};
              *reinterpret_cast<u32x2 *>(d0 + 2 * PLANE_B) = u32x2{L01, L23};
            }
          } else if (live) {
            float *dst = tmid + pix * 8 + (ksub & 1);
#pragma unroll
            for (int j = 0; j < 4; ++j) dst[2 * j] = o[j];
          }
        }
      };
      groups(std::integral_constant<int, 0>{}, std::integral_constant<int, G::GPW>{}, cell_s, interior ? 0 : lane_rowcol(0),
             interior ? 0 : lane_rowcol(G::GPW - 1));
      if (own) {
        if constexpr (!CACHED) cell_c = corner_cell();
        groups(std::integral_constant<int, G::GPW>{}, std::integral_constant<int, G::NSLOT>{}, cell_c, 0, interior ? 0 : lane_rowcol(G::GPW));
      }
    }
    RA_PHASE_AT(2);
    RA_P8_SYNC();
    RA_PHASE_AT(3);

    {
      f32x4 acc[4];
      int gmid[4];
#pragma unroll
      for (int g = 0; g < 4; ++g) {
        const int gy = 2 * wave + (g >> 1), gx = g & 1;
        gmid[g] = (2 * gy * G::AW + 16 * gx) * 8 + lane_b;
        acc[g] = f32x4{shB, shB, shB, shB};
      }
      if constexpr (SPLIT) {
        const unsigned char *tb = reinterpret_cast<const unsigned char *>(tmid);
        const int lane_px = ((m & 1) * G::AW + 2 * (m >> 1) + 1 + ksub) * 16;
#pragma unroll
        for (int ky = 0; ky < 3; ++ky)
#pragma unroll
          for (int gh = 0; gh < 2; ++gh) {
            s16x8 av[2][3];
#pragma unroll
            for (int u = 0; u < 2; ++u) {
              const int g = 2 * gh + u;
              const int gy = 2 * wave + (g >> 1), gx = g & 1;
              const int off = ((2 * gy + ky) * G::AW + 16 * gx) * 16 + lane_px;
#pragma unroll
              for (int pc = 0; pc < 3; ++pc) av[u][pc] = *reinterpret_cast<const s16x8 *>(tb + off + pc * PLANE_B);
            }
            constexpr int PA[6] = {1, 0, 2, 0, 1, 0}, PB[6] = {1, 2, 0, 1, 0, 0};
#pragma unroll
            for (int t = 0; t < 6; ++t)
#pragma unroll
              for (int u = 0; u < 2; ++u)
                acc[2 * gh + u] = __builtin_amdgcn_mfma_f32_16x16x32_bf16(__builtin_bit_cast(bf16x8, av[u][PA[t]]),
                                                                          __builtin_bit_cast(bf16x8, wB[ky][PB[t]]), acc[2 * gh + u], 0, 0, 0);
          }
      } else {
#pragma unroll
      for (int ky = 0; ky < 3; ++ky)
#pragma unroll
        for (int kxp = 0; kxp < 4; ++kxp) {
          f32x2 av[4];
#pragma unroll
          for (int g = 0; g < 4; ++g)
            av[g] = *reinterpret_cast<const f32x2 *>(&tmid[gmid[g] + (ky * G::AW + kxp) * 8]);
#pragma unroll
          for (int cg = 0; cg < 2; ++cg)
#pragma unroll
            for (int g = 0; g < 4; ++g)
              acc[g] = __builtin_amdgcn_mfma_f32_16x16x4f32(av[g][cg], bB[ky * 4 + kxp][cg], acc[g], 0, 0, 0);
        }
      }
      const int prow0 = (ty0 >> 1) + wave * 2, pcol0 = (tx0 >> 1) + 2 * qo + p;
      const bool whole = ((ty0 >> 1) + G::TH / 2 <= a.Ho) & ((tx0 >> 1) + G::TW / 2 <= a.Wo);
      const unsigned tile_y = (unsigned)(((b * a.Ho + prow0) * a.Wo + (tx0 >> 1)) * a.CoutB * 4) + lane_y;
#pragma unroll
      for (int g = 0; g < 4; ++g) {
        const float t0 = fmaxf(fmaxf(acc[g][0], acc[g][1]), loB), t1 = fmaxf(fmaxf(acc[g][2], acc[g][3]), loB);
        const float u0 = fmaxf(t0, __builtin_bit_cast(float, __builtin_amdgcn_mov_dpp(__builtin_bit_cast(int, t0), 0x128, 0xf, 0xf, true)));
        const float u1 = fmaxf(t1, __builtin_bit_cast(float, __builtin_amdgcn_mov_dpp(__builtin_bit_cast(int, t1), 0x128, 0xf, 0xf, true)));
        const float ov = p ? u1 : u0;
        const int prow = prow0 + (g >> 1), pcol = pcol0 + 8 * (g & 1);
        unsigned off = tile_y + (unsigned)g_y[g];
        if (!whole) off = ((prow < a.Ho) & (pcol < a.Wo)) ? off : 0x80000000u;
        __builtin_amdgcn_raw_buffer_store_b32(__builtin_bit_cast(unsigned, ov), ry, (int)off, 0, 0);
      }
    }
    RA_PHASE_AT(4);
  }
  RA_PHASE_END;
  if constexpr (!CACHED) {
    if (rider)
      for (; r_idx < r_end; r_idx += 256) __builtin_amdgcn_raw_buffer_store_b128(r_bits, rr, r_idx * 16, 0, 0);
  }
}

template <int CINA, bool CACHED = false, bool SPLIT = false>
int launch8(PArgs a, int B, hipStream_t st, int *plan) {
  using G = NGeo<CINA>;
  a.bytes_y = (int)((size_t)B * a.Ho * a.Wo * a.CoutB * sizeof(float));
  auto kern = conv_pair8_mfma<CINA, CACHED, SPLIT>;
  constexpr size_t lds = (size_t)G::template lds_floats<CACHED, SPLIT>() * sizeof(float);
  const int tiles_x = ceil_div(a.W, G::TW), tiles_y = ceil_div(a.H, G::TH);
  const int ntiles = tiles_x * tiles_y * B;
  static const int wgs = env_int("RA_PAIR8_WGS", 768);
  static const int xcd = env_int("RA_PAIR8_XCD", 1);
  const int grid = ntiles < wgs ? ntiles : wgs;
  a.xcd_map = (xcd && grid % 8 == 0 && grid >= 8) ? 1 : 0;
  const bool draws = CACHED && ntiles >= kTicketMinTilesPerWg * grid;
  if (plan) {
    plan[RA_PLAN_FAMILY] = RA_PLAN_FAMILY_PAIR;
    plan[RA_PLAN_FORM] = RA_PLAN_FORM_NPACKED | (CACHED ? RA_PLAN_FORM_CACHED : 0) | (SPLIT ? RA_PLAN_FORM_SPLIT : 0);
    plan[RA_PLAN_CK] = CINA, plan[RA_PLAN_CMID] = 8, plan[RA_PLAN_KF] = 3, plan[RA_PLAN_TILE_H] = G::TH, plan[RA_PLAN_TILE_W] = G::TW;
    plan[RA_PLAN_TILES_X] = tiles_x, plan[RA_PLAN_TILES_Y] = tiles_y, plan[RA_PLAN_TICKETS] = draws ? 1 : 0;
    plan_walk(plan, ntiles, grid, a.xcd_map);
    return 0;
  }
  static const MaxDynamicLds lds_limit(kern, lds);
  a.tickets = draws ? take_ticket_slots(1, grid) : nullptr;
  hipLaunchKernelGGL(kern, dim3(grid), dim3(256), lds, st, a, tiles_x, tiles_y, ntiles);
  return launch_status("ra_conv_pair_f32");
}

__global__ __launch_bounds__(256) void first_cache_kernel(const float *x, const float *wpA, int CoutAP, int plane_chan,
                                                          int B, int H, int W, int rows, int ngx, float *cache) {
  __shared__ float sm[4][64][9];
  const int xl = threadIdx.x & 63, yl = threadIdx.x >> 6;
  const int X = blockIdx.x * 64 - 2 + xl, Y = blockIdx.y * 4 + yl, b = blockIdx.z;
  float acc[8];
#pragma unroll
  for (int co = 0; co < 8; ++co) acc[co] = 0.f;
  if (X >= 0 && X < W && Y < H) {
#pragma unroll
    for (int ky = 0; ky < 3; ++ky) {
      const int yy = Y + ky - 1;
#pragma unroll
      for (int kx = 0; kx < 3; ++kx) {
        const int xx = X + kx - 1;
        const bool ok = (yy >= 0) & (yy < H) & (xx >= 0) & (xx < W);
        f32x4 v = f32x4{0.f, 0.f, 0.f, 0.f};
        if (ok) v = *reinterpret_cast<const f32x4 *>(x + ((size_t)(b * H + yy) * W + xx) * 4);
        const float *wt = wpA + (size_t)((ky * 3 + kx) * 4) * CoutAP;
#pragma unroll
        for (int ci = 0; ci < 4; ++ci) {
          const float xv = ci == plane_chan ? 0.f : v[ci];
#pragma unroll
          for (int co = 0; co < 8; ++co) acc[co] = fmaf(xv, wt[ci * CoutAP + co], acc[co]);
        }
      }
    }
  }
#pragma unroll
  for (int co = 0; co < 8; ++co) sm[yl][xl][co] = acc[co];
  __syncthreads();
  for (int e = threadIdx.x; e < 4 * 8 * 16; e += 256) {
    const int n4 = e & 3, r = (e >> 2) & 3, g = (e >> 4) & 7, row = e >> 7;
    const int p = n4 >> 1, co0 = 4 * (n4 & 1);
    const int Yo = blockIdx.y * 4 + row, gx = blockIdx.x * 8 + g;
    if (Yo < H && gx < ngx) {
      f32x4 o;
#pragma unroll
      for (int j = 0; j < 4; ++j) o[j] = sm[row][8 * g + 2 * r + p][co0 + j];
      *reinterpret_cast<f32x4 *>(cache + (((size_t)b * rows + (Yo + 1)) * ngx + gx) * 64 + r * 16 + 4 * n4) = o;
    }
  }
}

void cache_dims(int H, int W, int &rows, int &ngx) {
  rows = ceil_div(H, NGeo<4>::TH) * NGeo<4>::TH + 4;
  ngx = ceil_div(W, NGeo<4>::TW) * (NGeo<4>::TW / 8) + 1;
}
int launch_npacked(const PArgs &a, int B, hipStream_t st, int *plan) {
  return a.C0 == 4 ? launch8<4>(a, B, st, plan) : launch8<8>(a, B, st, plan);
}

int fill_cache_entry(const float *src, const float *plane, int plane_chan, int B, int H, int W, const float *wpA, const float *scaleA,
                     const float *shiftA, int reluA, const float *wpB, const float *scaleB, const float *shiftB, int CoutB, int reluB,
                     float *cache, float *y, float *fill_dst, size_t fill_floats, float fill_value, void *stream, int *plan) {
  if (missing_pointer(plan, {src, plane, cache, wpA, scaleA, shiftA, wpB, scaleB, shiftB, y}) || B <= 0)
    return fail(RA_E_INVALID, "ra_conv_pair_fill_cache_f32: bad argument");
  if (fill_dst && ((reinterpret_cast<uintptr_t>(fill_dst) & 15) || (fill_floats & 3) || fill_floats * 4 >= (1ull << 31)))
    return fail(RA_E_SHAPE, "ra_conv_pair_fill_cache_rider_f32: the fill must be 16-byte aligned, a multiple of 4 floats, < 2 GiB");
  if (!ra_conv_first_cache_supported(4, 8, CoutB, 2, H, W) || plane_chan < 0 || plane_chan > 3)
    return fail(RA_E_SHAPE, "ra_conv_pair_fill_cache_f32: unsupported shape");
  PArgs a = pair_args(src, 4, B, H, W, 0, wpA, scaleA, shiftA, 8, reluA, wpB, scaleB, shiftB, CoutB, reluB, 2, plane, plane_chan, y);
  const size_t b0 = (size_t)B * H * W * 4 * sizeof(float);
  if (b0 >= (1ull << 31)) return fail(RA_E_SHAPE, "ra_conv_pair_fill_cache_f32: input exceeds 2 GiB");
  a.bytes0 = (int)b0;
  if (int rc = pair_args_cache(a, cache, B, "ra_conv_pair_fill_cache_f32")) return rc;
  a.rider_dst = fill_floats ? fill_dst : nullptr;
  a.rider_quads = (int)(fill_floats / 4);
  a.rider_val = fill_value;
  return launch8<4, false>(a, B, as_stream(stream), plan);
}

int cached_entry(const float *cache, const float *plane, int plane_chan, int B, int H, int W, const float *wpA, const float *scaleA,
                 const float *shiftA, int reluA, const float *wpB, const float *scaleB, const float *shiftB, int CoutB, int reluB,
                 float *y, void *stream, int *plan) {
  if (missing_pointer(plan, {cache, plane, wpA, scaleA, shiftA, wpB, scaleB, shiftB, y}) || B <= 0)
    return fail(RA_E_INVALID, "ra_conv_pair_cached_f32: bad argument");
  if (!ra_conv_first_cache_supported(4, 8, CoutB, 2, H, W) || plane_chan < 0 || plane_chan > 3)
    return fail(RA_E_SHAPE, "ra_conv_pair_cached_f32: unsupported shape");
  PArgs a = pair_args(plane, 4, B, H, W, 0, wpA, scaleA, shiftA, 8, reluA, wpB, scaleB, shiftB, CoutB, reluB, 2, plane, plane_chan, y);
  if (int rc = pair_args_cache(a, cache, B, "ra_conv_pair_cached_f32")) return rc;
  static const int split = env_int("RA_PAIR8_SPLIT", 1);
  if (split) return launch8<4, true, true>(a, B, as_stream(stream), plan);
  return launch8<4, true>(a, B, as_stream(stream), plan);
}

}
}

using namespace ra;

extern "C" int ra_conv_first_cache_supported(int Cin, int CoutA, int CoutB, int poolB, int H, int W) {
  return Cin == 4 && CoutA == 8 && CoutB >= 1 && CoutB <= 8 && poolB == 2 && W > 16 && !((H | W) & 1);
}

extern "C" size_t ra_conv_first_cache_floats(int B, int H, int W) {
  if (B <= 0 || H <= 0 || W <= 0) return 0;
  int rows, ngx;
  cpair::cache_dims(H, W, rows, ngx);
  return (size_t)B * rows * ngx * 64;
}

extern "C" int ra_conv_first_cache_f32(const float *src, int B, int H, int W, const float *wpA, int CoutA,
                                       int plane_chan, float *cache, void *stream) {
  if (!src || !wpA || !cache || B <= 0 || H <= 0 || W <= 0 || plane_chan < 0 || plane_chan > 3)
    return fail(RA_E_INVALID, "ra_conv_first_cache_f32: bad argument");
  if (CoutA != 8) return fail(RA_E_SHAPE, "ra_conv_first_cache_f32: CoutA %d", CoutA);
  int rows, ngx;
  cpair::cache_dims(H, W, rows, ngx);
  const size_t total = (size_t)B * rows * ngx * 16;
  if (total * 16 >= (1ull << 31)) return fail(RA_E_SHAPE, "ra_conv_first_cache_f32: cache exceeds 2 GiB");
  hipLaunchKernelGGL(cpair::first_cache_kernel, dim3(ceil_div(W + 2, 64), ceil_div(H, 4), B), dim3(256), 0,
                     as_stream(stream), src, wpA, ra_conv_cout_padded(CoutA), plane_chan, B, H, W, rows, ngx, cache);
  return launch_status("ra_conv_first_cache_f32");
}

extern "C" int ra_conv_pair_fill_cache_rider_f32(const float *src, const float *plane, int plane_chan, int B, int H, int W,
                                                 const float *wpA, const float *scaleA, const float *shiftA, int reluA,
                                                 const float *wpB, const float *scaleB, const float *shiftB, int CoutB,
                                                 int reluB, float *cache, float *y, float *fill_dst, size_t fill_floats,
                                                 float fill_value, void *stream) {
  return cpair::fill_cache_entry(src, plane, plane_chan, B, H, W, wpA, scaleA, shiftA, reluA, wpB, scaleB, shiftB, CoutB, reluB, cache, y,
                                 fill_dst, fill_floats, fill_value, stream, nullptr);
}

extern "C" int ra_conv_pair_fill_cache_f32(const float *src, const float *plane, int plane_chan, int B, int H, int W,
                                           const float *wpA, const float *scaleA, const float *shiftA, int reluA,
                                           const float *wpB, const float *scaleB, const float *shiftB, int CoutB,
                                           int reluB, float *cache, float *y, void *stream) {
  return ra_conv_pair_fill_cache_rider_f32(src, plane, plane_chan, B, H, W, wpA, scaleA, shiftA, reluA, wpB, scaleB, shiftB,
                                           CoutB, reluB, cache, y, nullptr, 0, 0.0f, stream);
}

extern "C" int ra_conv_pair_cached_f32(const float *cache, const float *plane, int plane_chan, int B, int H, int W,
                                       const float *wpA, const float *scaleA, const float *shiftA, int reluA,
                                       const float *wpB, const float *scaleB, const float *shiftB, int CoutB,
                                       int reluB, float *y, void *stream) {
  return cpair::cached_entry(cache, plane, plane_chan, B, H, W, wpA, scaleA, shiftA, reluA, wpB, scaleB, shiftB, CoutB, reluB, y, stream,
                             nullptr);
}
```

### rec-attend-public_amd/csrc/ra_conv_pair_parts.h

```cpp
#pragma once
#include <cstdint>
#include <initializer_list>

#include "ra_common.h"

namespace ra {
namespace cpair {

struct PArgs {
  const float *src;
  float *y;
  const float *wpA, *scA, *shA, *wpB, *scB, *shB;
  int C0, Hs, Ws, H, W, ups;
  int CoutAP, CoutB, CoutBP, poolB, Ho, Wo, reluA, reluB;
  const float *plane;
  int plane_chan;
  int bytes0, bytes_p;
  const float *cache;
  int cache_rows, cache_gx, bytes_c;
  int bytes_y;
  int xcd_map;
  float *rider_dst;
  int rider_quads;
  float rider_val;
  unsigned *tickets;
};

template <int N>
struct vec_of {
  typedef float type __attribute__((ext_vector_type(N)));
};

inline bool missing_pointer(const int *plan, std::initializer_list<const void *> ptrs) {
  if (plan) return false;
  for (const void *p : ptrs)
    if (!p) return true;
  return false;
}

inline PArgs pair_args(const float *src, int Cin, int B, int Hs, int Ws, int upsampleA, const float *wpA, const float *scaleA,
                       const float *shiftA, int CoutA, int reluA, const float *wpB, const float *scaleB, const float *shiftB,
                       int CoutB, int reluB, int poolB, const float *plane, int plane_chan, float *y) {
  PArgs a{};
  a.src = src;
  a.y = y;
  a.wpA = wpA;
  a.scA = scaleA;
  a.shA = shiftA;
  a.wpB = wpB;
  a.scB = scaleB;
  a.shB = shiftB;
  a.C0 = Cin;
  a.Hs = Hs;
  a.Ws = Ws;
  a.ups = upsampleA ? 1 : 0;
  a.H = Hs * (1 + a.ups);
  a.W = Ws * (1 + a.ups);
  a.CoutAP = ra_conv_cout_padded(CoutA);
  a.CoutB = CoutB;
  a.CoutBP = ra_conv_cout_padded(CoutB);
  a.poolB = poolB;
  a.Ho = a.H / poolB;
  a.Wo = a.W / poolB;
  a.reluA = reluA;
  a.reluB = reluB;
  a.plane = plane;
  a.plane_chan = plane_chan;
  a.bytes_p = (int)((size_t)B * Hs * Ws * 4);
  return a;
}

void cache_dims(int H, int W, int &rows, int &ngx);

inline int pair_args_cache(PArgs &a, const float *cache, int B, const char *what) {
  a.cache = cache;
  cache_dims(a.H, a.W, a.cache_rows, a.cache_gx);
  const size_t cb = (size_t)B * a.cache_rows * a.cache_gx * 64 * sizeof(float);
  if (cb >= (1ull << 31)) return fail(RA_E_SHAPE, "%s: cache exceeds 2 GiB", what);
  a.bytes_c = (int)cb;
  return 0;
}

int launch_npacked(const PArgs &a, int B, hipStream_t st, int *plan);
int fill_cache_entry(const float *src, const float *plane, int plane_chan, int B, int H, int W, const float *wpA, const float *scaleA,
                     const float *shiftA, int reluA, const float *wpB, const float *scaleB, const float *shiftB, int CoutB, int reluB,
                     float *cache, float *y, float *fill_dst, size_t fill_floats, float fill_value, void *stream, int *plan);
int cached_entry(const float *cache, const float *plane, int plane_chan, int B, int H, int W, const float *wpA, const float *scaleA,
                 const float *shiftA, int reluA, const float *wpB, const float *scaleB, const float *shiftB, int CoutB, int reluB,
                 float *y, void *stream, int *plan);

}
}
```

### rec-attend-public_amd/ra_engine.py

```python
import numpy as np
import math
import os

import torch

import operator

import ra_native as rn
import ra_ops as ops


def _dev(a, device):
  return torch.from_numpy(np.ascontiguousarray(a)).to(device)


def _r4(n):
  return -(-n // 4) * 4


_TENSOR_VERSION = operator.attrgetter('_version')


class DecodeEngine(object):

  def __init__(self, dims, model, box_model=False):
    self.d = dims
    self.model = model
    self.box = box_model
    self._stamp = None
    self._B = None
    self._graphs = {}
    self.fuse_pairs = True
    self.fuse_patch_pairs = False
    self.ctrl_split = True
    self.fuse_score = True
    self.wino_unfuse = False
    self.pair_wino = True
    self.pair_direct16 = os.environ.get('RA_PAIR16', '1') != '0'
    self.use_wino = True
    self.cache_first = True
    self.fill_cache_inline = True
    self.co_resident = 1
    self.tile_tickets = os.environ.get('RA_ENGINE_TICKETS', '0') != '0'
    self.nsub = 0
    self.use_graph = True
    self.prefill_ride = True
    self.use_split = os.environ.get('RA_USE_SPLIT', '1') != '0'
    self.split_first = os.environ.get('RA_SPLIT_FIRST', '1') != '0'
    self.ctrl_batch_xcd = os.environ.get('RA_CTRL_BATCH_XCD', '1') != '0'
    self.xcd_slot, self.xcd_slots = 0, 1
    self.box_iou_rects = os.environ.get('RA_BOX_IOU_RECTS', '1') != '0'
    self.split_patch = os.environ.get('RA_SPLIT_PATCH', 'auto')
    self.fuse_extract_conv0 = os.environ.get('RA_FUSE_EXTRACT_CONV0', '0') == '1'
    self.timing = None

  def _weights_stamp(self):
    m = self.model
    mut = getattr(m, '_mut', None)
    if mut is None:
      return tuple((k, v.data_ptr(), v._version) for k, v in sorted(m.items())
                   if isinstance(v, torch.Tensor) and '_' in k and not k.startswith('__'))
    if getattr(self, '_wlist_mut', None) != mut:
      self._wlist = [v for k, v in sorted(m.items()) if isinstance(v, torch.Tensor) and '_' in k and not k.startswith('__')]
      self._wlist_mut = mut
    return (mut, sum(map(_TENSOR_VERSION, self._wlist)))

  def _chan_map(self, flags):
    d = self.d
    groups = [(d['D'], True, flags[0]), (1, True, flags[1]), (8, d['add_d_out'], flags[2]),
              (d['nsc'], d['add_y_out'], flags[3])]
    cmap, idx = [], 0
    for n, present, used in groups:
      if not present:
        if used:
          raise rn.RecAttendError('input group used by the model but not fed')
        continue
      for _ in range(n):
        if used:
          cmap.append(idx)
          idx += 1
        else:
          cmap.append(-1)
    cmap += [-1] * (d['C0p'] - len(cmap))
    return cmap, idx

  def prepare(self, device):
    stamp = self._weights_stamp()
    if stamp == self._stamp:
      return
    d, M, T = self.d, self.model, self.d['T']
    bn = lambda scope, i, t: tuple(M['%s_%d_%d_%s' % (scope, i, t, n)]
                                   for n in ('beta', 'gamma', 'ema_mean', 'ema_var'))

    def fold_all(scope, i, cout):
      sc, sh = [], []
      for t in range(T):
        a, b = ops.fold_bn(M['%s_b_%d' % (scope, i)], cout, bn(scope, i, t) if d['use_bn'] else None)
        sc.append(a)
        sh.append(b)
      return _dev(np.stack(sc), device), _dev(np.stack(sh), device)

    W = {}
    ks = self.ksize = {'ccnn': list(d['ccnn_filters'])}
    if not self.box:
      ks['acnn'], ks['adcnn'] = list(d['acnn_filters']), list(d['adcnn_filters'])
    cmap_c, n_c = self._chan_map(d['ctrl_in'])
    assert n_c == d['ccnn_channels'][0]
    W['ccnn'], W['ccnn_wino'], W['ccnn_split'] = [], [], []
    hh, ww = d['H'], d['W']
    for i in range(d['ccnn_nlayers']):
      cin, cout = d['ccnn_channels'][i], d['ccnn_channels'][i + 1]
      k3 = ks['ccnn'][i] == 3
      if i == 0:
        wp = ops.pack_conv_weights(M['ctrl_cnn_w_0'], cin_kernel=d['C0p'], chan_map=cmap_c)
      else:
        wp = ops.pack_conv_weights(M['ctrl_cnn_w_%d' % i], cin_kernel=_r4(cin))
      sc, sh = fold_all('ctrl_cnn', i, cout)
      W['ccnn'].append((_dev(wp, device), sc, sh, cout, d['ccnn_pool'][i]))
      wino = i > 0 and k3 and self.use_wino and ops.conv_wino_supported(cin, cout, d['ccnn_pool'][i], hh, ww)
      W['ccnn_wino'].append(_dev(ops.pack_wino_weights(M['ctrl_cnn_w_%d' % i]), device) if wino else None)
      split = (i > 0 and k3 and self.use_split and (cin >= int(os.environ.get('RA_SPLIT_MIN_CIN', '32')) or not wino or cout == 16) and
               ops.conv_split_supported(_r4(cin), cout, d['ccnn_pool'][i], hh, ww))
      if (i == 0 and k3 and self.use_split and self.split_first and d['C0p'] != 4 and
          ops.conv_split_supported(d['C0p'], cout, d['ccnn_pool'][0], hh, ww)):
        W['ccnn_split'].append(torch.from_numpy(ops.pack_split_weights(M['ctrl_cnn_w_0'], cin_kernel=d['C0p'], chan_map=cmap_c)).to(device))
      else:
        W['ccnn_split'].append(torch.from_numpy(ops.pack_split_weights(M['ctrl_cnn_w_%d' % i])).to(device) if split else None)
      hh, ww = hh // d['ccnn_pool'][i], ww // d['ccnn_pool'][i]
    Cf = d['ccnn_channels'][-1]
    self.desc = ops.make_ctrl_desc(d['G'], Cf, d['hid'], d['iters'], d['n_gmlp'], d['n_cmlp'],
                                   d['mlp_dim'], d['H'], d['W'], d['Fh'], d['Fw'], d['squash'],
                                   d['fixed_var'], d['dynamic_var'],
                                   d.get('fixed_gamma', True))
    lstm = {k: M['ctrl_lstm_' + k] for k in ('w_xi', 'w_hi', 'b_i', 'w_xf', 'w_hf', 'b_f', 'w_xu',
                                             'w_hu', 'b_u', 'w_xo', 'w_ho', 'b_o')}
    gm = [(M['glimpse_mlp_w_%d' % i], M['glimpse_mlp_b_%d' % i]) for i in range(d['n_gmlp'])]
    cm = [(M['ctrl_mlp_w_%d' % i], M['ctrl_mlp_b_%d' % i]) for i in range(d['n_cmlp'])]
    W['ctrl'] = _dev(ops.pack_ctrl_weights(self.desc, lstm, gm, cm), device)
    self.split_ok = self.ctrl_split and ops.ctrl_split_supported(self.desc)
    if self.split_ok:
      W['ctrl_split'] = _dev(ops.pack_ctrl_split_weights(self.desc, lstm, gm, cm), device)
    W['smlp_w'] = M['score_mlp_w_0']
    W['smlp_b'] = M['score_mlp_b_0']
    if not self.box:
      cmap_a, n_a = self._chan_map(d['attn_in'])
      assert n_a == d['acnn_channels'][0]
      self.attn_sel = [c for c, m in enumerate(cmap_a) if m >= 0]
      W['acnn'], W['acnn_split'] = [], []
      ph, pw = d['Fh'], d['Fw']
      for i in range(d['acnn_nlayers']):
        cin, cout = d['acnn_channels'][i], d['acnn_channels'][i + 1]
        if i == 0:
          wp = ops.pack_conv_weights(M['attn_cnn_w_0'], cin_kernel=d['C0p'], chan_map=cmap_a)
        else:
          wp = ops.pack_conv_weights(M['attn_cnn_w_%d' % i], cin_kernel=_r4(cin))
        sc, sh = fold_all('attn_cnn', i, cout)
        W['acnn'].append((_dev(wp, device), sc, sh, cout, d['acnn_pool'][i]))
        ck = d['C0p'] if i == 0 else _r4(cin)
        k3 = ks['acnn'][i] == 3
        sp = None
        if k3 and self.use_split and self.split_patch != '0' and ops.conv_split_supported(ck, cout, d['acnn_pool'][i], ph, pw):
          mf = 2e-6 * 9 * cin * cout * ph * pw
          if self.split_patch == '1' or mf >= float(os.environ.get('RA_SPLIT_PATCH_MIN_MF', '4')):
            sp = torch.from_numpy(ops.pack_split_weights(M['attn_cnn_w_%d' % i], cin_kernel=ck, chan_map=cmap_a if i == 0 else None)).to(device)
        W['acnn_split'].append(sp)
        ph, pw = ph // d['acnn_pool'][i], pw // d['acnn_pool'][i]
        if i == 0 and k3 and ops.extract_conv0_supported(d['C0p'], d['Fh'], d['Fw'], cout, d['acnn_pool'][0]):
          w0 = M['attn_cnn_w_0'].detach().cpu().numpy().astype(np.float32)
          plain = np.zeros((3, 3, d['C0p'], cout), np.float32)
          for c, m_ in enumerate(cmap_a):
            if m_ >= 0:
              plain[:, :, c, :] = w0[:, :, m_, :]
          W['acnn0_plain'] = _dev(plain, device)
      W['adcnn'] = []
      L = d['acnn_nlayers']
      prev_c = d['adcnn_channels'][0]
      for i in range(d['adcnn_nlayers']):
        cout = d['adcnn_channels'][i + 1]
        n_skip = d['skip_ch'][i] if d['skip_ch'] is not None else 0
        src = None
        if n_skip:
          src = i - 1
        c_prev = _r4(prev_c)
        cmap = [k if k < prev_c else -1 for k in range(c_prev)]
        c_skip = 0
        if src is not None:
          if src == L - 1:
            cmap += [prev_c + m if m >= 0 else -1 for m in cmap_a]
            c_skip = d['C0p']
          else:
            sc_real = d['acnn_channels'][L - 1 - src]
            c_skip = _r4(sc_real)
            cmap += [prev_c + k if k < sc_real else -1 for k in range(c_skip)]
        wp = ops.pack_conv_weights(M['attn_dcnn_w_%d' % i], cin_kernel=c_prev + c_skip,
                                   chan_map=cmap, transposed=True)
        sc, sh = fold_all('attn_dcnn', i, cout)
        W['adcnn'].append((_dev(wp, device), sc, sh, cout, d['adcnn_unpool'][i], src))
        prev_c = cout
    self.W = W
    self.plan = self._make_plan(W)
    self._stamp = stamp
    self._graphs = {}
    for k, (g_, s_, st_, _) in list(self.__dict__.get('_states', {}).items()):
      self._states[k] = (g_, s_, st_, {})

  def _make_plan(self, W):
    d = self.d
    plan = {}

    def pair_up(n, cin, cout, a_ok, b_ok, unfuse=lambda i: False, ks=None):
      steps, i = [], 0
      while i < n:
        if (self.fuse_pairs and i + 1 < n and ks[i] == 3 and ks[i + 1] == 3 and a_ok(i) and b_ok(i + 1) and cout(i) <= 16 and
            ops.conv_pair_supported(cin(i), cout(i), cout(i + 1)) and not unfuse(i + 1)):
          steps.append(('pair', i, i + 1))
          i += 2
        else:
          steps.append(('single', i))
          i += 1
      return steps

    cc = d['ccnn_channels']
    wino_alone = lambda i: self.use_wino and self.wino_unfuse and W['ccnn_wino'][i] is not None
    plan['ccnn'] = pair_up(d['ccnn_nlayers'], lambda i: d['C0p'] if i == 0 else _r4(cc[i]),
                           lambda i: cc[i + 1], lambda i: d['ccnn_pool'][i] == 1, lambda i: True, wino_alone, ks=self.ksize['ccnn'])
    if not self.box:
      ac = d['acnn_channels']
      L = d['acnn_nlayers']
      skip_used = set(L - 2 - lay_[5] for lay_ in W['adcnn'] if lay_[5] is not None and lay_[5] < L - 1)
      fuse_patch = self.fuse_patch_pairs
      plan['acnn'] = pair_up(L, lambda i: d['C0p'] if i == 0 else _r4(ac[i]), lambda i: ac[i + 1],
                             lambda i: fuse_patch and d['acnn_pool'][i] == 1 and i not in skip_used,
                             lambda i: True, ks=self.ksize['acnn'])
      dc = d['adcnn_channels']
      lay = W['adcnn']
      plan['adcnn'] = pair_up(d['adcnn_nlayers'], lambda i: _r4(dc[i]), lambda i: dc[i + 1],
                              lambda i: fuse_patch and lay[i][5] is None,
                              lambda i: lay[i][5] is None and lay[i][4] == 1, ks=self.ksize['adcnn'])
    return plan

  def alloc(self, B, device):
    nsub = self.nsub if self.nsub else 1
    if B % nsub:
      nsub = 1
    if self._B == (B, nsub):
      return
    states = self.__dict__.setdefault('_states', {})
    if self._B is not None:
      states[self._B] = (self.glob, self.subs, self.streams, self._graphs)
      while len(states) > 3:
        states.pop(next(iter(states)))
    hit = states.pop((B, nsub), None)
    if hit is not None:
      self.glob, self.subs, self.streams, self._graphs = hit
      self._B = (B, nsub)
      return
    d, T = self.d, self.d['T']
    f = lambda *s: torch.zeros(s, dtype=torch.float32, device=device)
    H, W, Fh, Fw = d['H'], d['W'], d['Fh'], d['Fw']
    g = {}
    g['x'] = f(B, H, W, d['D'])
    if d['add_d_out']:
      g['d_in'] = f(B, H, W, 8)
    if d['add_y_out']:
      g['y_in'] = f(B, H, W, d['nsc'])
    g['s_out'] = f(B, T) if (self.box is False or d['nsc'] == 1) else f(B, T, d['nsc'])
    g['attn_box'] = f(B, T, H, W)
    if self.box:
      g['y_gt'] = f(B, T, H, W)
      g['noise'] = f(T, B, H, W)
    else:
      g['y_out'] = f(B, T, H, W)
    Bs = B // nsub
    subs = []
    for k in range(nsub):
      b = {kk: v[k * Bs:(k + 1) * Bs] for kk, v in g.items() if kk != 'noise'}
      b['img'] = f(Bs, H, W, d['C0p'])
      b['canvas'] = f(Bs, H, W)
      hh, ww = H, W
      b['ccnn'] = []
      for i in range(d['ccnn_nlayers']):
        hh, ww = hh // d['ccnn_pool'][i], ww // d['ccnn_pool'][i]
        b['ccnn'].append(f(Bs, hh, ww, d['ccnn_channels'][i + 1]))
      b['tickets'] = ops.tickets_alloc(16 * T, device)
      b['h_last'] = f(T, Bs, d['hid'])
      b['ctrl_out'] = f(T, Bs, 9)
      b['gmaps'] = f(T, Bs, d['iters'], d['G'])
      b['attn'] = f(T, Bs, rn.RA_ATTN_STRIDE)
      st0 = self.plan['ccnn'][0]
      if self.cache_first and st0[0] == 'pair' and d['C0p'] == 4 and self.ksize['ccnn'][:2] == [3, 3] and \
          ops.first_cache_supported(4, d['ccnn_channels'][1], d['ccnn_channels'][2], d['ccnn_pool'][1], H, W):
        b['l0cache'] = ops.first_cache_alloc(Bs, H, W, device)
      form = ops.ctrl_form(self.desc, Bs, self.co_resident) if self.split_ok else None
      if form == 'split':
        b['ctrl_ws'], b['ctrl_status'] = ops.ctrl_split_workspace(self.desc, Bs, device)
      elif form == 'batch':
        b['ctrl_ws'], b['ctrl_status'] = ops.ctrl_batch_workspace(self.desc, Bs, device)
        b['ctrl_batch'] = True
        ng = -(-Bs // ops.ctrl_batch_group(self.desc, Bs))
        if self.ctrl_batch_xcd and self.xcd_slots >= 1 and self.xcd_slots * ng <= int(os.environ.get('RA_CTRL_BATCH_XCD_MAX_TEAMS', '4')):
          b['ctrl_xcd_off'] = (self.xcd_slot % self.xcd_slots) * ng
      if self.box:
        b['noise'] = f(T, Bs, H, W)
        b['ysel'] = f(Bs, H, W)
        b['match'] = f(Bs, T)
        b['box1'] = f(Bs, 1, H, W)
      else:
        b['x_patch'] = f(T, Bs, Fh, Fw, d['C0p'])
        hh, ww = Fh, Fw
        b['acnn'] = []
        for i in range(d['acnn_nlayers']):
          hh, ww = hh // d['acnn_pool'][i], ww // d['acnn_pool'][i]
          b['acnn'].append(f(Bs, hh, ww, d['acnn_channels'][i + 1]))
        b['adcnn'] = []
        for i in range(d['adcnn_nlayers']):
          hh, ww = hh * d['adcnn_unpool'][i], ww * d['adcnn_unpool'][i]
          if i == d['adcnn_nlayers'] - 1:
            b['y_out_patch'] = f(T, Bs, hh, ww, d['adcnn_channels'][i + 1])
            b['adcnn'].append(None)
          else:
            b['adcnn'].append(f(Bs, hh, ww, d['adcnn_channels'][i + 1]))
      subs.append(b)
    self.glob = g
    self.subs = subs
    self.streams = [torch.cuda.Stream(device=device) for _ in range(nsub)] if nsub > 1 else []
    self._B = (B, nsub)
    self._graphs = {}

  def fetch(self, name):
    if name in self.glob:
      return self.glob[name]
    parts = [sb[name] for sb in self.subs]
    if len(parts) == 1:
      return parts[0]
    dim = 0 if name in ('img', 'canvas') else 1
    return torch.cat(parts, dim=dim)

  def check_status(self, recover=True):
    bad = False
    for sb in self.subs:
      st = sb.get('ctrl_status')
      if st is not None and int(st.item()) != 0:
        st.zero_()
        bad = True
    if not bad:
      return False
    if not recover:
      raise rn.RecAttendError('controller_split: a workgroup timed out waiting for its peers (the launch was '
                              'not fully resident); decode with engine.ctrl_split = False')
    import warnings
    warnings.warn('controller_split: a workgroup timed out waiting for its peers (the launch was not fully resident: is '
                  'something else using this GPU?); the batch is decoded again on the one-workgroup controller, which this '
                  'engine keeps from now on')
    torch.cuda.synchronize()
    keep = {k: self.glob[k].clone() for k in ('x', 'd_in', 'y_in', 'y_gt', 'noise') if k in self.glob}
    want_box = getattr(self, '_last_want_box', False)
    self.ctrl_split = False
    self._stamp = None
    self._B = None
    self._states = {}
    self._graphs = {}
    self.forward(keep['x'], d_in=keep.get('d_in'), y_in=keep.get('y_in'), y_gt=keep.get('y_gt'), noise=keep.get('noise'),
                 want_box=want_box)
    torch.cuda.synchronize()
    return True

  def _mark(self, name):
    if self.timing is not None:
      ev = torch.cuda.Event(enable_timing=True)
      ev.record()
      self.timing.append((name, ev))

  def stage_times_ms(self):
    out = {}
    for (_, e0), (name, e1) in zip(self.timing[:-1], self.timing[1:]):
      tot, n = out.get(name, (0.0, 0))
      out[name] = (tot + e0.elapsed_time(e1), n + 1)
    return out

  def _launch_all(self, want_box):
    if len(self.subs) == 1:
      self._launch_sub(self.subs[0], want_box)
      return
    main = torch.cuda.current_stream()
    for sb, st in zip(self.subs, self.streams):
      st.wait_stream(main)
      with torch.cuda.stream(st):
        self._launch_sub(sb, want_box)
    for st in self.streams:
      main.wait_stream(st)

  def _launch_sub(self, b, want_box):
    self._launch_pack(b)
    bound = self.tile_tickets and 'tickets' in b and ops.tickets_bind(b['tickets'])
    try:
      for tt in range(self.d['T']):
        self._launch_tail(b, tt, want_box, self._launch_encoder(b, tt))
    finally:
      if bound:
        ops.tickets_unbind()

  def _launch_encoder(self, b, tt):
    fill = b['y_out'] if (tt == 0 and b.pop('_fill_rider', False)) else None
    return self._run_cnn(self.plan['ccnn'], self.W['ccnn'], b['img'], b['ccnn'], tt, 'ctrl_cnn',
                         plane=b['canvas'], cache=b.get('l0cache'), fill=fill)

  def _prefill_rides(self, b):
    st0 = self.plan['ccnn'][0]
    return (self.prefill_ride and 'l0cache' in b and self.fill_cache_inline and st0[0] == 'pair' and
            ops.fill_rider_ok(b['y_out']))

  def _launch_pack(self, b):
    if self._prepacked:
      b['canvas'].zero_()
    else:
      ops.pack_input(b['x'], b.get('d_in'), b.get('y_in'), self.d['C0p'], b['img'],
                     canvas_plane=b['canvas'])
    if not self.box and not self.d['disable_overwrite']:
      if self._prefill_rides(b):
        b['_fill_rider'] = True
      else:
        ops.fill(b['y_out'], 1.0 / (1.0 + math.exp(5.0)))
    if 'l0cache' in b and not self.fill_cache_inline:
      ops.first_cache(b['img'], self.W['ccnn'][0][0], self.d['ccnn_channels'][1], self.d['D'], b['l0cache'])
    self._mark('pack')

  def _launch_tail(self, b, tt, want_box, src):
    d, Wt, T = self.d, self.W, self.d['T']
    H, W, Fh, Fw = d['H'], d['W'], d['Fh'], d['Fw']
    if 'ctrl_ws' in b and b.get('ctrl_batch'):
      ops.controller_batch(self.desc, src, Wt['ctrl_split'], b['h_last'][tt], b['ctrl_out'][tt], b['gmaps'][tt], b['attn'][tt],
                           b['ctrl_ws'], b['ctrl_status'], xcd_offset=b.get('ctrl_xcd_off', -1))
    elif 'ctrl_ws' in b:
      ops.controller_split(
          self.desc, src, Wt['ctrl_split'], b['h_last'][tt], b['ctrl_out'][tt], b['gmaps'][tt], b['attn'][tt],
          b['ctrl_ws'], b['ctrl_status'])
    else:
      ops.controller(self.desc, src, Wt['ctrl'], b['h_last'][tt], b['ctrl_out'][tt],
                     b['gmaps'][tt], b['attn'][tt])
    self._mark('controller')
    if want_box or self.box:
      ops.attn_box_direct(b['attn'][tt], H, W, Fh, Fw, -5.0, b['attn_box'].data_ptr() + tt * H * W * 4, T * H * W)
      if self.box:
        ops.attn_box_direct(b['attn'][tt], H, W, Fh, Fw, -5.0, b['box1'].data_ptr(), H * W)
      self._mark('attn_box')
    if self.box:
      self._box_step(b, tt)
      return
    xp = b['x_patch'][tt]
    if self.fuse_extract_conv0 and 'acnn0_plain' in Wt and self.plan['acnn'][0] == ('single', 0):
      _, sc0, sh0, c0, _ = Wt['acnn'][0]
      ops.extract_conv0(b['img'], 0, b['attn'][tt], Fh, Fw, True, xp, Wt['acnn0_plain'], sc0[tt], sh0[tt], c0, True, b['acnn'][0],
                        canvas=b['canvas'], canvas_chan=d['D'])
      self._mark('extract+attn_cnn_L0')
      src = self._run_cnn(self.plan['acnn'][1:], Wt['acnn'], b['acnn'][0], b['acnn'], tt, 'attn_cnn')
    else:
      ops.extract_direct(b['img'], 0, b['attn'][tt], Fh, Fw, d['C0p'], True, xp, canvas=b['canvas'], canvas_chan=d['D'])
      self._mark('extract')
      src = self._run_cnn(self.plan['acnn'], Wt['acnn'], xp, b['acnn'], tt, 'attn_cnn')
    core = src
    L = d['acnn_nlayers']
    skips = [b['acnn'][L - 2 - k] for k in range(L - 1)] + [xp]
    for step in self.plan['adcnn']:
      if step[0] == 'pair':
        (wpa, sca, sha, ca, upa, _), (wpb, scb, shb, cb, _, _) = Wt['adcnn'][step[1]], Wt['adcnn'][step[2]]
        out = b['y_out_patch'][tt] if b['adcnn'][step[2]] is None else b['adcnn'][step[2]]
        ops.conv_pair(src, wpa, sca[tt], sha[tt], ca, wpb, scb[tt], shb[tt], cb, poolB=1,
                      upsampleA=(upa == 2), out=out)
      else:
        i = step[1]
        wp, sc, sh, cout, unpool, sidx = Wt['adcnn'][i]
        out = b['y_out_patch'][tt] if b['adcnn'][i] is None else b['adcnn'][i]
        if self.ksize['adcnn'][i] != 3:
          ops.conv2d_fused(src, wp, sc[tt], sh[tt], cout, self.ksize['adcnn'][i], relu=True, pool=1,
                           src1=None if sidx is None else skips[sidx], upsample=(unpool == 2), out=out)
        else:
          ops.conv3x3(src, wp, sc[tt], sh[tt], cout, relu=True, pool=1,
                      src1=None if sidx is None else skips[sidx], upsample=(unpool == 2), out=out)
      src = out
    self._mark('attn_dcnn')
    fused_score = self.fuse_score and self.timing is None
    if not fused_score:
      ops.dense(b['h_last'][tt], Wt['smlp_w'], Wt['smlp_b'], 'sigmoid',
                b['s_out'].data_ptr() + tt * 4, T, x1=core.view(core.shape[0], -1))
      self._mark('score')
    flags = (0 if d['disable_overwrite'] else ops.PASTE_Y_PREFILLED) | (ops.PASTE_CANVAS_FLOORED if tt > 0 else 0)
    if fused_score:
      ops.paste_score_direct(src, 0, b['attn'][tt], -5.0, d['disable_overwrite'],
                             b['y_out'].data_ptr() + tt * H * W * 4, T * H * W, H, W, b['canvas'], flags,
                             b['h_last'][tt], core.view(core.shape[0], -1), Wt['smlp_w'], Wt['smlp_b'],
                             b['s_out'].data_ptr() + tt * 4, T)
    else:
      ops.paste_direct(src, 0, b['attn'][tt], -5.0, d['disable_overwrite'],
                       b['y_out'].data_ptr() + tt * H * W * 4, T * H * W, H, W, canvas=b['canvas'], flags=flags)
    self._mark('paste')

  def _run_cnn(self, steps, layers, src, bufs, tt, name, plane=None, cache=None, fill=None):
    pc = self.d['D'] if plane is not None else -1
    ks = self.ksize['acnn'] if layers is self.W.get('acnn') else self.ksize['ccnn']
    for step in steps:
      pl = plane if step[1] == 0 else None
      if step[0] == 'pair':
        (wpa, sca, sha, ca, _), (wpb, scb, shb, cb, poolb) = layers[step[1]], layers[step[2]]
        if cache is not None and pl is not None and tt == 0 and self.fill_cache_inline:
          ops.conv_pair_fill_cache(src, pl, pc, wpa, sca[tt], sha[tt], wpb, scb[tt], shb[tt], cb, cache, bufs[step[2]],
                                   fill=fill, fill_value=1.0 / (1.0 + math.exp(5.0)))
        elif cache is not None and pl is not None:
          ops.conv_pair_cached(cache, pl, pc, wpa, sca[tt], sha[tt], wpb, scb[tt], shb[tt], cb, bufs[step[2]])
        elif (self.pair_direct16 and self.pair_wino and layers is self.W.get('ccnn') and pl is None and
              ops.conv_pair16_supported(src.shape[3], ca, cb, poolb, src.shape[1], src.shape[2])):
          ops.conv_pair16(src, wpa, sca[tt], sha[tt], wpb, scb[tt], shb[tt], out=bufs[step[2]])
        elif (self.use_wino and self.pair_wino and layers is self.W.get('ccnn') and pl is None and
              self.W['ccnn_wino'][step[2]] is not None and
              ops.conv_pair_wino_supported(src.shape[3], ca, cb, poolb, src.shape[1], src.shape[2])):
          ops.conv_pair_wino(src, wpa, sca[tt], sha[tt], self.W['ccnn_wino'][step[2]], scb[tt], shb[tt], out=bufs[step[2]])
        else:
          ops.conv_pair(src, wpa, sca[tt], sha[tt], ca, wpb, scb[tt], shb[tt], cb, poolB=poolb,
                        out=bufs[step[2]], plane=pl, plane_chan=pc if pl is not None else -1)
        src = bufs[step[2]]
        self._mark('%s_L%d+%d' % (name, step[1], step[2]))
      else:
        i = step[1]
        wp, sc, sh, cout, pool = layers[i]
        wino = self.W['ccnn_wino'][i] if (layers is self.W.get('ccnn') and pl is None and self.use_wino) else None
        split = None
        if self.use_split and layers is self.W.get('ccnn') and (pl is None or i == 0):
          split = self.W['ccnn_split'][i]
        elif self.use_split and layers is self.W.get('acnn'):
          split = self.W['acnn_split'][i]
        if ks[i] != 3:
          ops.conv2d_fused(src, wp, sc[tt], sh[tt], cout, ks[i], relu=True, pool=pool, out=bufs[i], plane=pl,
                           plane_chan=pc if pl is not None else -1)
        elif split is not None:
          ops.conv_split(src, split, sc[tt], sh[tt], cout, relu=True, pool=pool, out=bufs[i], plane=pl, plane_chan=pc if pl is not None else -1)
        elif wino is not None:
          ops.conv_wino(src, wino, sc[tt], sh[tt], cout, relu=True, pool=pool, out=bufs[i])
        else:
          ops.conv3x3(src, wp, sc[tt], sh[tt], cout, relu=True, pool=pool, out=bufs[i], plane=pl,
                      plane_chan=pc if pl is not None else -1)
        src = bufs[i]
        self._mark('%s_L%d' % (name, i))
    return src

  def _box_step(self, b, tt):
    d, T = self.d, self.d['T']
    box = b['box1']
    if self.box_iou_rects and 'gt_params' in b and d['W'] % 4 == 0 and T <= 32:
      iou = ops.box_iou_rects(box.view(box.shape[0], d['H'], d['W']), b['gt_params'])
    else:
      iou = ops.pair_stats(box, b['box_gt'], want=('iou_soft',))['iou_soft']
    ops.greedy_match(iou.view(iou.shape[0], T), out=b['match'])
    ops.weighted_sum(b['match'], b['y_gt'], b['ysel'])
    ops.canvas_max(b['canvas'].view(b['canvas'].shape + (1,)), 0, b['ysel'], b['noise'][tt])
    nsc = d['nsc']
    ops.dense(b['h_last'][tt], self.W['smlp_w'], self.W['smlp_b'],
              'sigmoid' if nsc == 1 else 'softmax', b['s_out'].data_ptr() + tt * nsc * 4,
              T * nsc)
    self._mark('box_step')

  _prepacked = False

  def prestage_slots(self, B):
    if not torch.cuda.is_available():
      raise rn.RecAttendError('the decode loop needs an MI355X (HIP device); no CPU fallback')
    device = torch.device('cuda')
    if self._stamp is None:
      self.prepare(device)
    self.alloc(B, device)
    return self.subs

  def forward(self, x, d_in=None, y_in=None, y_gt=None, noise=None, want_box=False, prepacked=False):
    if not torch.cuda.is_available():
      raise rn.RecAttendError('the decode loop needs an MI355X (HIP device); no CPU fallback')
    self._prepacked = bool(prepacked)
    device = torch.device('cuda')
    as_t = lambda a: (a if isinstance(a, torch.Tensor) else torch.from_numpy(
        np.ascontiguousarray(a, dtype=np.float32))).to(device=device, dtype=torch.float32)
    x = as_t(x)
    B = x.shape[0]
    late_check = self._stamp is not None
    if not late_check:
      self.prepare(device)
    self.alloc(B, device)
    b = self.glob
    b['x'].copy_(x)
    if 'd_in' in b and not prepacked:
      b['d_in'].copy_(as_t(d_in))
    if 'y_in' in b and not prepacked:
      b['y_in'].copy_(as_t(y_in))
    if self.box:
      b['y_gt'].copy_(as_t(y_gt))
      if noise is None:
        b['noise'].uniform_(0.0, 0.3)
      else:
        b['noise'].copy_(as_t(noise).reshape(b['noise'].shape))
      Bs = B // len(self.subs)
      for k, sb in enumerate(self.subs):
        sb['noise'].copy_(b['noise'][:, k * Bs:(k + 1) * Bs])
        sb['gt_params'], sb['box_gt'] = ops.gt_box(sb['y_gt'].contiguous(), float(self.d['attn_box_padding_ratio']), 10.0)
    self._last_want_box = bool(want_box)
    self._launch_forward(want_box)
    if late_check and self._weights_stamp() != self._stamp:
      self.prepare(device)
      self._launch_forward(want_box)
    return self

  def _launch_forward(self, want_box):
    graphable = self.use_graph and self.timing is None
    if not graphable:
      self._launch_all(want_box)
      return self
    key = (bool(want_box), True) if self._prepacked else bool(want_box)
    if self.box:
      for sb in self.subs:
        if 'box_gt_buf' not in sb:
          sb['box_gt_buf'] = torch.empty_like(sb['box_gt'])
          sb['gt_params_buf'] = torch.empty_like(sb['gt_params'])
        sb['box_gt_buf'].copy_(sb['box_gt'])
        sb['box_gt'] = sb['box_gt_buf']
        sb['gt_params_buf'].copy_(sb['gt_params'])
        sb['gt_params'] = sb['gt_params_buf']
    g = self._graphs.get(key)
    if g is None:
      self._launch_all(want_box)
      torch.cuda.synchronize()
      g = torch.cuda.CUDAGraph()
      with rn.quiet_capture(), torch.cuda.graph(g):
        self._launch_all(want_box)
      self._graphs[key] = g
    g.replay()
    return self
```

### rec-attend-public_amd/ra_ops.py

```python
import ctypes as C
import os

import numpy as np
import torch

import ra_native as rn
from ra_native import check, ptr

BN_EPS = 1e-3


def _need_cuda(*ts, f32=True):
  for t in ts:
    if t is not None and not t.is_cuda:
      raise rn.RecAttendError('recattend kernels need CUDA (HIP) tensors; got a CPU tensor. '
                              'There is no CPU fallback.')
    if t is not None and ((f32 and t.dtype != torch.float32) or not t.is_contiguous()):
      raise rn.RecAttendError('recattend kernels need contiguous float32 tensors')


def _np32(a):
  if isinstance(a, torch.Tensor):
    a = a.detach().cpu().numpy()
  return np.ascontiguousarray(a, dtype=np.float32)
# ... 410 lines not shown
    ws = torch.empty(n, dtype=torch.float32, device=x.device)
  check(rn.lib().ra_conv3x3_wgrad_wide_acc_f32(ptr(x), cin, B, Hs, Ws, int(bool(upsample)), ptr(du), cout, ptr(ws), ws.numel(), ptr(chan_map),
                                               int(cin_w), int(bool(transposed)), ptr(gw), ptr(gb), rn.stream_ptr()),
        'ra_conv3x3_wgrad_wide_acc_f32')
  return gw



_POISON = os.environ.get('RA_POISON')


def _f(*shape, device):
  if _POISON:
    return torch.full(shape, float(_POISON), dtype=torch.float32, device=device)
  return torch.empty(shape, dtype=torch.float32, device=device)


def bn_workspace(C_, like, ws=None, groups=1, wide=False):
  n = groups * (rn.lib().ra_bn_wide_workspace_floats if wide else rn.lib().ra_bn_workspace_floats)(int(C_))
  return ws if ws is not None and ws.numel() >= n else _f(n, device=like.device)


def bn_moments(u, ws=None, out=None, wide=False):
  _need_cuda(u, ws)
  C_ = u.shape[-1]
  mean, var = out if out is not None else (_f(C_, device=u.device), _f(C_, device=u.device))
  ws = bn_workspace(C_, u, ws, wide=wide)
  name = 'ra_bn_wide_moments_f32' if wide else 'ra_bn_moments_f32'
  check(getattr(rn.lib(), name)(ptr(u), u.numel() // C_, C_, ptr(ws), ws.numel(), ptr(mean), ptr(var), rn.stream_ptr()), name)
  return mean, var


def conv3x3_train(x, wp, scale, shift, cout, upsample=False, bf16=False, out=None, store_flags=None, moments=True):
  _need_cuda(x, wp, scale, shift, out, f32=False)
  B, Hs, Ws, cin = x.shape
  u = _conv_out(x, cout, 1, upsample, out)
  part = _f(rn.lib().ra_conv3x3_moments_part_floats(int(cout)), device=x.device) if moments else None
  nparts = C.c_int(0)
  head = (ptr(x), cin, None, 0, B, Hs, Ws, int(bool(upsample)), ptr(wp), ptr(scale), ptr(shift), int(cout), 0)
  tail = (ptr(part), part.numel(), C.byref(nparts)) if moments else (None, 0, None)
  if store_flags is None:
    check(rn.lib().ra_conv3x3_moments_f32(*head, int(bool(bf16)), ptr(u), *tail, rn.stream_ptr()), 'ra_conv3x3_moments_f32')
  else:
    check(rn.lib().ra_conv3x3_bf16_f32(*head, 1, ptr(u), *tail, int(store_flags), rn.stream_ptr()), 'ra_conv3x3_bf16_f32')
  return u, part, nparts.value


def bn_moments_from_partials(part, nparts, C_, out=None):
  _need_cuda(part)
  mean, var = out if out is not None else (_f(C_, device=part.device), _f(C_, device=part.device))
  check(rn.lib().ra_bn_moments_from_partials_f32(ptr(part), int(nparts), int(C_), ptr(mean), ptr(var), rn.stream_ptr()),
        'ra_bn_moments_from_partials_f32')
  return mean, var


def bn_act_pool(u, mean, var, gamma, beta, relu=True, pool=1, out=None, store_flags=None, wide=False):
  _need_cuda(u, out, f32=False)
  _need_cuda(mean, var, gamma, beta)
  B, H, W, C_ = u.shape
  if out is None:
    out = torch.empty((B, H // pool, W // pool, C_), dtype=torch.float32, device=u.device)
  head = (ptr(u), ptr(mean), ptr(var), ptr(gamma), ptr(beta), C.c_float(BN_EPS), int(relu), int(pool), B, H, W, C_, ptr(out))
  if store_flags is not None:
    assert not wide
    check(rn.lib().ra_bn_act_pool_bf16_f32(*head, int(store_flags), rn.stream_ptr()), 'ra_bn_act_pool_bf16_f32')
  else:
    name = 'ra_bn_wide_act_pool_f32' if wide else 'ra_bn_act_pool_f32'
    check(getattr(rn.lib(), name)(*head, rn.stream_ptr()), name)
  return out


def bn_act_pool_bwd(u, dy, mean, var, gamma, beta, relu=True, pool=1, acc=None, ws=None, du=None, wide=False):
  acc = (None, None) if wide and acc is None else acc
  _need_cuda(u, dy, mean, var, gamma, beta, ws, du, *(acc or ()))
  C_ = u.shape[3]
  du = torch.empty_like(u) if du is None else du
  dgamma, dbeta = _f(C_, device=u.device), _f(C_, device=u.device)
  ws = bn_workspace(C_, u, ws, wide=wide)
  head = (ptr(u), ptr(dy), ptr(mean), ptr(var), ptr(gamma), ptr(beta), C.c_float(BN_EPS), int(relu), int(pool), *u.shape, ptr(ws), ws.numel(),
          ptr(dgamma), ptr(dbeta), ptr(du))
  if acc is None:
    check(rn.lib().ra_bn_act_pool_bwd_f32(*head, rn.stream_ptr()), 'ra_bn_act_pool_bwd_f32')
  else:
    name = 'ra_bn_wide_act_pool_bwd_acc_f32' if wide else 'ra_bn_act_pool_bwd_acc_f32'
    check(getattr(rn.lib(), name)(*head, ptr(acc[0]), ptr(acc[1]), rn.stream_ptr()), name)
  return du, dgamma, dbeta


def bn_wide_moments(u, ws=None):
  return bn_moments(u, ws=ws, wide=True)


def bn_wide_act_pool(u, mean, var, gamma, beta, relu=True, pool=1, out=None):
  return bn_act_pool(u, mean, var, gamma, beta, relu=relu, pool=pool, out=out, wide=True)


def bn_wide_act_pool_bwd(u, dy, mean, var, gamma, beta, relu=True, pool=1, acc_gamma=None, acc_beta=None, ws=None):
  return bn_act_pool_bwd(u, dy, mean, var, gamma, beta, relu=relu, pool=pool, acc=(acc_gamma, acc_beta), ws=ws, wide=True)


def bn_act_pool_bwd_reduce(u, dy, mean, var, gamma, beta, relu=True, pool=1, acc=(None, None), ws=None, out=None):
  _need_cuda(u, dy, mean, var, gamma, beta, ws, *acc)
  C_ = u.shape[3]
  dgamma, dbeta = out if out is not None else (_f(C_, device=u.device), _f(C_, device=u.device))
  ws = bn_workspace(C_, u, ws)
  check(rn.lib().ra_bn_act_pool_bwd_reduce_f32(ptr(u), ptr(dy), ptr(mean), ptr(var), ptr(gamma), ptr(beta), C.c_float(BN_EPS), int(relu), int(pool),
                                               *u.shape, ptr(ws), ws.numel(), ptr(dgamma), ptr(dbeta), ptr(acc[0]), ptr(acc[1]), rn.stream_ptr()),
        'ra_bn_act_pool_bwd_reduce_f32')
  return dgamma, dbeta


def bn_act_pool_bwd_dx(u, dy, mean, var, gamma, beta, dgamma_sum, dbeta_sum, n_total, relu=True, pool=1, du=None):
  _need_cuda(u, dy, mean, var, gamma, beta, du)
  du = torch.empty_like(u) if du is None else du
  check(rn.lib().ra_bn_act_pool_bwd_dx_f32(ptr(u), ptr(dy), ptr(mean), ptr(var), ptr(gamma), ptr(beta), ptr(dgamma_sum), ptr(dbeta_sum),
                                           C.c_double(n_total), C.c_float(BN_EPS), int(relu), int(pool), *u.shape, ptr(du), rn.stream_ptr()),
        'ra_bn_act_pool_bwd_dx_f32')
  return du


def bn_act_pool_bwd_grouped(U, dY, tabs, G, relu=True, pool=1, store_flags=0, ws=None):
  _need_cuda(U, dY, tabs, ws, f32=False)
  N, H, W, C_ = U.shape
  du = torch.empty_like(U)
  dgamma, dbeta = _f(G, C_, device=U.device), _f(G, C_, device=U.device)
  ws = bn_workspace(C_, U, ws, groups=G)
  check(rn.lib().ra_bn_act_pool_bwd_grouped_bf16_f32(ptr(U), ptr(dY), ptr(tabs), int(G), C.c_float(BN_EPS), int(relu), int(pool), N // G, H, W,
                                                     C_, ptr(ws), ws.numel(), ptr(dgamma), ptr(dbeta), ptr(du), int(store_flags),
                                                     rn.stream_ptr()), 'ra_bn_act_pool_bwd_grouped_bf16_f32')
  return du, dgamma, dbeta


def wgrad3x3_workspace_floats(cin, cout, B, H, W):
  return rn.lib().ra_conv3x3_wgrad_workspace_floats(int(cin), int(cout), int(B), int(H), int(W))


def _wgrad3x3_ws(x, du, ws):
  n = wgrad3x3_workspace_floats(x.shape[3], du.shape[3], *du.shape[:3])
  return ws if ws is not None and ws.numel() >= n else _f(n, device=x.device)


def wgrad3x3(x, du, upsample=False, bf16=False, ws=None):
  _need_cuda(x, du, ws)
  B, Hs, Ws, cin = x.shape
  cout = du.shape[3]
  dw, db = _f(3, 3, cin, cout, device=x.device), _f(cout, device=x.device)
  ws = _wgrad3x3_ws(x, du, ws)
  name = 'ra_conv3x3_wgrad_bf16ops_f32' if bf16 else 'ra_conv3x3_wgrad_f32'
  check(getattr(rn.lib(), name)(ptr(x), cin, B, Hs, Ws, int(bool(upsample)), ptr(du), cout, ptr(ws), ws.numel(), ptr(dw), ptr(db),
                                rn.stream_ptr()), name)
  return dw, db


def wgrad3x3_acc(x, du, gw, gb=None, chan_map=None, transposed=False, upsample=False, bf16=False, ws=None):
  _need_cuda(x, du, f32=False)
  _need_cuda(gw, gb, ws)
  B, Hs, Ws, cin = x.shape
  ws = _wgrad3x3_ws(x, du, ws)
  head = (ptr(x), cin, B, Hs, Ws, int(bool(upsample)), ptr(du), du.shape[3], ptr(ws), ws.numel(), ptr(chan_map),
          int(gw.shape[3] if transposed else gw.shape[2]), int(bool(transposed)), ptr(gw), ptr(gb))
  fmt = (1 if x.dtype == torch.bfloat16 else 0) | (2 if du.dtype == torch.bfloat16 else 0)
  if fmt:
    check(rn.lib().ra_conv3x3_wgrad_acc_bf16_f32(*head, fmt, rn.stream_ptr()), 'ra_conv3x3_wgrad_acc_bf16_f32')
  else:
    name = 'ra_conv3x3_wgrad_acc_bf16ops_f32' if bf16 else 'ra_conv3x3_wgrad_acc_f32'
    check(getattr(rn.lib(), name)(*head, rn.stream_ptr()), name)
  return gw


def wgrad3x3_multi_acc(tab, n, seg_shape, cout, ws, gw, gb, chan_map=None, cin_w=None, transposed=False, upsample=False, bf16=False):
  _need_cuda(ws, gw, gb)
  B, Hs, Ws, cin = seg_shape
  check(rn.lib().ra_conv3x3_wgrad_multi_acc_f32(tab.data_ptr(), tab.data_ptr() + 8 * 64, int(n), cin, B, Hs, Ws, int(bool(upsample)), int(cout),
                                                ptr(ws), ws.numel(), ptr(chan_map), int(cin_w), int(bool(transposed)), ptr(gw), ptr(gb),
                                                int(bf16), rn.stream_ptr()), 'ra_conv3x3_wgrad_multi_acc_f32')
  return gw


def subsample(x, even=False, out=None):
  _need_cuda(x, out)
  B, H, W, C_ = x.shape
  out = _f(B, H // 2, W // 2, C_, device=x.device) if out is None else out
  if tuple(out.shape) != (B, H // 2, W // 2, C_):
    raise rn.RecAttendError('subsample: out of shape %r for x of %r' % (tuple(out.shape), tuple(x.shape)))
  name = 'ra_subsample_even_f32' if even else 'ra_subsample_odd_f32'
  check(getattr(rn.lib(), name)(ptr(x), B, H // 2, W // 2, C_, ptr(out), rn.stream_ptr()), name)
  return out


def fg_head(logits, nsc, no, quantise=False, y_out=None, d_out=None, x=None, packed=None, canvas_plane=None):
  _need_cuda(logits, y_out, d_out, x, packed, canvas_plane)
  B, H, W, C = logits.shape
  if C != nsc + no:
    raise rn.RecAttendError('fg_head: %d channels for nsc %d + no %d' % (C, nsc, no))
  npix = B * H * W
  f = lambda c: torch.empty((B, H, W, c), dtype=torch.float32, device=logits.device)
  if y_out is None:
    y_out = f(nsc)
  if d_out is None and no:
    d_out = f(no)
  if y_out.numel() != npix * nsc or (no and d_out.numel() != npix * no):
    raise rn.RecAttendError('fg_head: destination sizes')
  D = Cp = 0
  if packed is not None:
    if x is None or x.numel() % npix or packed.numel() % npix:
      raise rn.RecAttendError('fg_head: the packed destination needs x [B,H,W,D]')
    D, Cp = x.numel() // npix, packed.numel() // npix
    if canvas_plane is not None and canvas_plane.numel() != npix:
      raise rn.RecAttendError('fg_head: canvas plane size')
  check(rn.lib().ra_fg_head_f32(ptr(logits), npix, int(nsc), int(no), int(bool(quantise)), ptr(y_out), ptr(d_out if no else None),
                                ptr(x if packed is not None else None), D, ptr(packed), Cp,
                                ptr(canvas_plane if packed is not None else None), rn.stream_ptr()), 'ra_fg_head_f32')
  return y_out, (d_out if no else None)


def conv_wino_supported(cin, cout, pool, H, W):
  return bool(rn.lib().ra_conv_wino_supported(int(cin), int(cout), int(pool), int(H), int(W)))


def pack_wino_weights(w):
  w = _np32(w)
  cin, cout = w.shape[2], w.shape[3]
  n = rn.lib().ra_conv_wino_packed_floats(cin, cout)
  if w.shape[0] != 3 or w.shape[1] != 3 or n == 0:
    raise rn.RecAttendError('unsupported Winograd conv shape %r' % (w.shape,))
  out = np.empty(n, dtype=np.float32)
  check(rn.lib().ra_conv_wino_pack_weights(ptr(w), cin, cout, ptr(out)), 'ra_conv_wino_pack_weights')
  return out


def conv_split_supported(cin, cout, pool, H, W):
  return bool(rn.lib().ra_conv_split_supported(int(cin), int(cout), int(pool), int(H), int(W)))


def pack_split_weights(w, cin_kernel=None, chan_map=None):
  w = _np32(w)
  if cin_kernel is not None or chan_map is not None:
    ck = int(cin_kernel if cin_kernel is not None else len(chan_map))
    cm = list(chan_map) if chan_map is not None else list(range(w.shape[2])) + [-1] * (ck - w.shape[2])
    wk = np.zeros((3, 3, ck, w.shape[3]), np.float32)
    for c, m_ in enumerate(cm[:ck]):
      if m_ >= 0:
        wk[:, :, c, :] = w[:, :, m_, :]
    w = wk
  cin, cout = w.shape[2], w.shape[3]
  n = rn.lib().ra_conv_split_packed_halfs(cin, cout)
  if w.shape[0] != 3 or w.shape[1] != 3 or n == 0:
    raise rn.RecAttendError('unsupported split-precision conv shape %r' % (w.shape,))
  out = np.empty(n, dtype=np.int16)
  check(rn.lib().ra_conv_split_pack_weights(ptr(w), cin, cout, ptr(out)), 'ra_conv_split_pack_weights')
  return out.view(np.float32)


def pack_split_weights_dev(w, cin, cout, transposed=False):
  _need_cuda(w)
  n = rn.lib().ra_conv_split_packed_halfs(int(cin), int(cout))
  if n == 0 or w.numel() != 9 * cin * cout:
    raise rn.RecAttendError('unsupported split-precision conv shape Cin=%d Cout=%d' % (cin, cout))
  out = torch.empty(n // 2, dtype=torch.float32, device=w.device)
  check(rn.lib().ra_conv_split_pack_weights_dev(ptr(w.contiguous()), int(cin), int(cout), int(bool(transposed)), ptr(out),
                                                rn.stream_ptr()), 'ra_conv_split_pack_weights_dev')
  return out


def conv_split(x, wp, scale, shift, cout, relu=True, pool=1, out=None, plane=None, plane_chan=-1):
  _need_cuda(x, wp, scale, shift, out, plane)
  B, H, W, cin = x.shape
  out = _conv_out(x, cout, pool, out=out)
  if plane is not None:
    check(rn.lib().ra_conv_split_plane_f32(ptr(x), B, H, W, cin, ptr(plane), int(plane_chan), ptr(wp), ptr(scale), ptr(shift), int(cout),
                                           int(relu), int(pool), ptr(out), rn.stream_ptr()), 'ra_conv_split_plane_f32')
    return out
  check(rn.lib().ra_conv_split_f32(ptr(x), B, H, W, cin, ptr(wp), ptr(scale), ptr(shift), int(cout), int(relu), int(pool),
                                   ptr(out), rn.stream_ptr()), 'ra_conv_split_f32')
  return out


def conv_wino(x, wp, scale, shift, cout, relu=True, pool=1, out=None):
  _need_cuda(x, wp, scale, shift, out)
  B, H, W, cin = x.shape
  out = _conv_out(x, cout, pool, out=out)
  check(rn.lib().ra_conv_wino_f32(ptr(x), B, H, W, cin, ptr(wp), ptr(scale), ptr(shift), int(cout), int(relu), int(pool),
                                  ptr(out), rn.stream_ptr()), 'ra_conv_wino_f32')
  return out


def conv_pair_wino_supported(cin, cout_a, cout_b, pool_b, H, W):
  return bool(rn.lib().ra_conv_pair_wino_supported(int(cin), int(cout_a), int(cout_b), int(pool_b), int(H), int(W)))


def conv_pair_wino(x, wpA, scA, shA, wpB_wino, scB, shB, reluA=True, reluB=True, out=None):
  _need_cuda(x, wpA, scA, shA, wpB_wino, scB, shB, out)
  B, H, W, _ = x.shape
  out = _conv_out(x, 16, 2, out=out)
  check(rn.lib().ra_conv_pair_wino_f32(ptr(x), B, H, W, ptr(wpA), ptr(scA), ptr(shA), int(reluA), ptr(wpB_wino), ptr(scB),
                                       ptr(shB), int(reluB), ptr(out), rn.stream_ptr()), 'ra_conv_pair_wino_f32')
  return out


def conv_pair16_supported(cin, cout_a, cout_b, pool_b, H, W):
  return bool(rn.lib().ra_conv_pair16_supported(int(cin), int(cout_a), int(cout_b), int(pool_b), int(H), int(W)))


def conv_pair16(x, wpA, scA, shA, wpB, scB, shB, reluA=True, reluB=True, out=None):
  _need_cuda(x, wpA, scA, shA, wpB, scB, shB, out)
  B, H, W, _ = x.shape
  out = _conv_out(x, 16, 2, out=out)
  check(rn.lib().ra_conv_pair16_f32(ptr(x), B, H, W, ptr(wpA), ptr(scA), ptr(shA), int(reluA), ptr(wpB), ptr(scB), ptr(shB),
                                    int(reluB), ptr(out), rn.stream_ptr()), 'ra_conv_pair16_f32')
  return out


def poison_lds():
  check(rn.lib().ra_debug_poison_lds(rn.stream_ptr()), 'ra_debug_poison_lds')


def park_xcd(xcd, n_wg, lds_bytes=100 * 1024, millis=100, resident=None, stream=None):
  check(rn.lib().ra_debug_park_xcd(int(xcd), int(n_wg), int(lds_bytes), int(millis), ptr(resident) if resident is not None else None,
                                   rn.stream_ptr() if stream is None else stream.cuda_stream), 'ra_debug_park_xcd')


def conv_pair_supported(cin, cout_a, cout_b):
  return bool(rn.lib().ra_conv_pair_supported(int(cin), int(cout_a), int(cout_b)))


def conv_pair(src, wpA, scA, shA, coutA, wpB, scB, shB, coutB, poolB=1, upsampleA=False,
              reluA=True, reluB=True, out=None, plane=None, plane_chan=-1):
  _need_cuda(src, wpA, scA, shA, wpB, scB, shB, out)
  B, Hs, Ws, C0 = src.shape
  out = _conv_out(src, coutB, poolB, upsampleA, out)
  check(rn.lib().ra_conv_pair_f32(ptr(src), C0, B, Hs, Ws, int(upsampleA), ptr(wpA), ptr(scA),
                                  ptr(shA), int(coutA), int(reluA), ptr(wpB), ptr(scB), ptr(shB),
                                  int(coutB), int(reluB), int(poolB), ptr(plane), int(plane_chan),
                                  ptr(out), rn.stream_ptr()),
        'ra_conv_pair_f32')
  return out


def first_cache_supported(cin, cout_a, cout_b, pool_b, H, W):
  return bool(rn.lib().ra_conv_first_cache_supported(int(cin), int(cout_a), int(cout_b), int(pool_b), int(H), int(W)))


def first_cache_alloc(B, H, W, device):
  return torch.zeros((rn.lib().ra_conv_first_cache_floats(B, H, W),), dtype=torch.float32, device=device)


def first_cache(img, wpA, cout_a, plane_chan, cache):
  _need_cuda(img, wpA, cache)
  B, H, W, C = img.shape
  assert C == 4
  check(rn.lib().ra_conv_first_cache_f32(ptr(img), B, H, W, ptr(wpA), int(cout_a), int(plane_chan), ptr(cache),
                                         rn.stream_ptr()), 'ra_conv_first_cache_f32')


def fill_rider_ok(t):
  return t.is_contiguous() and t.data_ptr() % 16 == 0 and t.numel() % 4 == 0 and t.numel() * 4 < (1 << 31)


def conv_pair_fill_cache(img, plane, plane_chan, wpA, scA, shA, wpB, scB, shB, coutB, cache, out, reluA=True, reluB=True,
                         fill=None, fill_value=0.0):
  _need_cuda(img, plane, wpA, scA, shA, wpB, scB, shB, cache, out, fill)
  B, H, W = plane.shape
  if fill is not None and not fill_rider_ok(fill):
    raise rn.RecAttendError('conv_pair_fill_cache: the rider fill needs a contiguous, 16-byte aligned tensor of 4k floats < 2 GiB')
  check(rn.lib().ra_conv_pair_fill_cache_rider_f32(ptr(img), ptr(plane), int(plane_chan), B, H, W, ptr(wpA), ptr(scA),
                                                   ptr(shA), int(reluA), ptr(wpB), ptr(scB), ptr(shB), int(coutB),
                                                   int(reluB), ptr(cache), ptr(out), ptr(fill),
                                                   0 if fill is None else fill.numel(), C.c_float(fill_value),
                                                   rn.stream_ptr()),
        'ra_conv_pair_fill_cache_rider_f32')
  return out


def conv_pair_cached(cache, plane, plane_chan, wpA, scA, shA, wpB, scB, shB, coutB, out, reluA=True, reluB=True):
  _need_cuda(cache, plane, wpA, scA, shA, wpB, scB, shB, out)
  B, H, W = plane.shape
  check(rn.lib().ra_conv_pair_cached_f32(ptr(cache), ptr(plane), int(plane_chan), B, H, W, ptr(wpA), ptr(scA),
                                         ptr(shA), int(reluA), ptr(wpB), ptr(scB), ptr(shB), int(coutB),
                                         int(reluB), ptr(out), rn.stream_ptr()), 'ra_conv_pair_cached_f32')
  return out


def controller(desc, feat, wp, h_last, ctrl_out, gmaps, attn):
  _need_cuda(feat, wp, h_last, ctrl_out, gmaps, attn)
  B = feat.shape[0]
  check(rn.lib().ra_controller_f32(C.byref(desc), ptr(feat), ptr(wp), B, ptr(h_last),
                                   ptr(ctrl_out), ptr(gmaps), ptr(attn), rn.stream_ptr()),
        'ra_controller_f32')


def extract_direct(img, chan0, attn, Fh, Fw, Cp, use_gamma, patch, canvas=None, canvas_chan=-1):
  _need_cuda(img, attn, patch, canvas)
  B, H, W, Ci = img.shape
  check(rn.lib().ra_extract_direct_f32(ptr(img), Ci, chan0, ptr(canvas), int(canvas_chan), ptr(attn),
                                       B, H, W, Fh, Fw, Cp, int(use_gamma), ptr(patch),
                                       rn.stream_ptr()), 'ra_extract_direct_f32')


def extract_conv0_supported(Cp, Fh, Fw, cout, pool):
  return bool(rn.lib().ra_extract_conv0_supported(int(Cp), int(Fh), int(Fw), int(cout), int(pool)))


def extract_conv0(img, chan0, attn, Fh, Fw, use_gamma, patch, w0, scale, shift, cout, relu, y0, canvas=None, canvas_chan=-1):
  _need_cuda(img, attn, patch, canvas, w0, scale, shift, y0)
  B, H, W, Ci = img.shape
  check(rn.lib().ra_extract_conv0_f32(ptr(img), Ci, chan0, ptr(canvas), int(canvas_chan), ptr(attn), B, H, W, Fh, Fw,
                                      int(use_gamma), ptr(patch), ptr(w0), ptr(scale), ptr(shift), int(cout), int(relu), ptr(y0),
                                      rn.stream_ptr()), 'ra_extract_conv0_f32')


PASTE_Y_PREFILLED, PASTE_CANVAS_FLOORED = rn.RA_PASTE_Y_PREFILLED, rn.RA_PASTE_CANVAS_FLOORED


def paste_direct(patch, pc, attn, beta, disable_overwrite, y_out, y_stride_b, H, W, canvas=None,
                 img=None, canvas_chan=-1, flags=0):
  _need_cuda(patch, attn, canvas, img)
  B, Fh, Fw, Cp = patch.shape
  Ci = 0 if img is None else img.shape[3]
  check(rn.lib().ra_paste_direct_f32(ptr(patch), Cp, pc, ptr(attn), B, H, W, Fh, Fw, C.c_float(beta),
                                     int(disable_overwrite), ptr(canvas), ptr(img), Ci,
                                     int(canvas_chan), ptr(y_out), y_stride_b, int(flags),
                                     rn.stream_ptr()),
        'ra_paste_direct_f32')


def paste_score_direct(patch, pc, attn, beta, disable_overwrite, y_out, y_stride_b, H, W, canvas, flags,
                       h, core, w, bias, s_out_ptr, s_stride_b):
  _need_cuda(patch, attn, canvas, h, core, w, bias)
  B, Fh, Fw, Cp = patch.shape
  K1 = 0 if core is None else core.shape[1]
  check(rn.lib().ra_paste_score_direct_f32(ptr(patch), Cp, pc, ptr(attn), B, H, W, Fh, Fw, C.c_float(beta),
                                           int(disable_overwrite), ptr(canvas), ptr(y_out), y_stride_b,
                                           int(flags), ptr(h), h.shape[1], ptr(core), K1, ptr(w), ptr(bias),
                                           ptr(s_out_ptr), s_stride_b, rn.stream_ptr()),
        'ra_paste_score_direct_f32')


def paste_plan(mode, B, H, W, Fh, Fw, Cp=1, pc=0, has_canvas=True, has_img=False, y_stride_b=None, aligned16=True):
  rec = (C.c_int * rn.RA_PASTE_PLAN_INTS)()
  stride = H * W if y_stride_b is None else y_stride_b
  check(rn.lib().ra_paste_plan({'paste': 0, 'box': 1}[mode], int(B), int(H), int(W), int(Fh), int(Fw), int(Cp), int(pc),
                               int(bool(has_canvas)), int(bool(has_img)), int(stride), int(bool(aligned16)), rec), 'ra_paste_plan')
  return {'kernel': {rn.RA_PASTE_KERNEL_GENERAL: 'general', rn.RA_PASTE_KERNEL_WINDOW: 'window'}[rec[rn.RA_PASTE_PLAN_KERNEL]],
          'rows': rec[rn.RA_PASTE_PLAN_ROWS], 'grid_x': rec[rn.RA_PASTE_PLAN_GRID_X], 'threads': rec[rn.RA_PASTE_PLAN_THREADS],
          'lds': rec[rn.RA_PASTE_PLAN_LDS]}


RESAMPLE_READ, RESAMPLE_WRITE, RESAMPLE_BOX = rn.RA_RESAMPLE_READ, rn.RA_RESAMPLE_WRITE, rn.RA_RESAMPLE_BOX


def resample_bwd(mode, rec, H, W, Fh, Fw, X=None, chan0=0, C=None, dY=None, Y=None, Q=None, E=None, scale=None, div=None):
  _need_cuda(rec, X, dY, Y, Q, E)
  B = rec.shape[0]
  if mode == RESAMPLE_READ:
    Cx = X.shape[3]
    C = Cx - chan0 if C is None else C
  else:
    Cx, C = 1, 1
  lib = rn.lib()
  nws = lib.ra_resample_bwd_workspace_floats(B, Fh, C)
  ws = torch.empty(nws, dtype=torch.float32, device=rec.device)
  out = torch.empty((B, 8), dtype=torch.float32, device=rec.device)
  sstride = 0 if scale is None else int(scale.stride(0))
  dstride = 0 if div is None else int(div.stride(0))
  check(lib.ra_resample_bwd_f32(int(mode), ptr(X), int(Cx), int(chan0), int(C), ptr(dY), ptr(Y), ptr(rec), ptr(Q),
                                0 if Q is None else int(Q.shape[3]), ptr(E), 0 if E is None else int(E.shape[3]), B, H, W, Fh, Fw,
                                ptr(scale), sstride, ptr(div), dstride, ptr(ws), nws, ptr(out), rn.stream_ptr()),
        'ra_resample_bwd_f32')
  return out


def attn_box_direct(attn, H, W, Fh, Fw, beta, out, stride_b):
  _need_cuda(attn)
  check(rn.lib().ra_attn_box_direct_f32(ptr(attn), attn.shape[0], H, W, Fh, Fw, C.c_float(beta),
                                        ptr(out), stride_b, rn.stream_ptr()),
        'ra_attn_box_direct_f32')


def dense(x0, W, b, act, out, out_stride_b, x1=None):
  _need_cuda(x0, x1, W, b)
  code = {None: 0, 'relu': 1, 'sigmoid': 2, 'softmax': 3, 'tanh': 4}[act]
  K1 = 0 if x1 is None else x1.shape[1]
  check(rn.lib().ra_dense_f32(ptr(x0), x0.shape[1], ptr(x1), K1, ptr(W), ptr(b), x0.shape[0],
                              W.shape[1], code, ptr(out), out_stride_b, rn.stream_ptr()),
        'ra_dense_f32')


def pack_input(x, d_in, y_in, Cp, packed, canvas_plane=None):
  _need_cuda(x, d_in, y_in, packed, canvas_plane)
  B, H, W, D = x.shape
  Dd = 0 if d_in is None else d_in.shape[3]
  Dy = 0 if y_in is None else y_in.shape[3]
  check(rn.lib().ra_pack_input_plane_f32(ptr(x), D, ptr(d_in), Dd, ptr(y_in), Dy, B, H, W, Cp,
                                         ptr(packed), ptr(canvas_plane), rn.stream_ptr()), 'ra_pack_input_plane_f32')


def canvas_max(img, canvas_chan, ysel, noise):
  _need_cuda(img, ysel, noise)
  B, H, W, Ci = img.shape
  check(rn.lib().ra_canvas_max_f32(ptr(img), Ci, canvas_chan, ptr(ysel), ptr(noise), B, H, W,
                                   rn.stream_ptr()), 'ra_canvas_max_f32')


def gaussian_filter(center, size, lg_var, L, F):
  _need_cuda(center, size, lg_var)
  B = center.shape[0]
  out = torch.empty((B, L, F), dtype=torch.float32, device=center.device)
  check(rn.lib().ra_gaussian_filter_f32(ptr(center), ptr(size), ptr(lg_var), B, L, F, ptr(out),
                                        rn.stream_ptr()), 'ra_gaussian_filter_f32')
  return out


def extract_patch_dense(x, f_y, f_x):
  _need_cuda(x, f_y, f_x)
  B, H, W, D = x.shape
  FH, FW = f_y.shape[2], f_x.shape[2]
  out = torch.empty((B, FH, FW, D), dtype=torch.float32, device=x.device)
  check(rn.lib().ra_extract_patch_dense_f32(ptr(x), ptr(f_y), ptr(f_x), B, H, W, D, FH, FW,
                                            ptr(out), rn.stream_ptr()),
        'ra_extract_patch_dense_f32')
  return out


def affine_act(x, scale, shift, relu=False):
  _need_cuda(x, scale, shift)
  Cc = x.shape[-1]
  out = torch.empty_like(x)
  check(rn.lib().ra_affine_act_f32(ptr(x), ptr(scale), ptr(shift), x.numel() // Cc, Cc,
                                   int(relu), ptr(out), rn.stream_ptr()), 'ra_affine_act_f32')
  return out


def max_pool(x, ratio):
  _need_cuda(x)
  B, H, W, Cc = x.shape
  out = torch.empty((B, -(-H // ratio), -(-W // ratio), Cc), dtype=torch.float32,
                    device=x.device)
  check(rn.lib().ra_max_pool_f32(ptr(x), B, H, W, Cc, int(ratio), ptr(out), rn.stream_ptr()),
        'ra_max_pool_f32')
  return out


def hungarian(weights):
  is_t = isinstance(weights, torch.Tensor)
  two_d = (weights.ndim == 2)
  if weights.ndim not in (2, 3):
    raise rn.RecAttendError('Must have dimension 3 or 2.')
  if is_t and weights.is_cuda:
    w = weights.detach().to(torch.float32).contiguous()
    w3 = w[None] if two_d else w
    B, N, M = w3.shape
    m = torch.empty_like(w3)
    cx = torch.empty((B, N), dtype=torch.float32, device=w.device)
    cy = torch.empty((B, M), dtype=torch.float32, device=w.device)
    st = torch.zeros((max(B, 1),), dtype=torch.int32, device=w.device)
    nb = rn.lib().ra_hungarian_dev_workspace_bytes(max(B, 1), N, M)
    ws = torch.empty((nb,), dtype=torch.uint8, device=w.device)
    check(rn.lib().ra_hungarian_f32_dev(ptr(w3), B, N, M, ptr(m), ptr(cx), ptr(cy), ptr(st),
                                        ptr(ws), nb, rn.stream_ptr()), 'ra_hungarian_f32_dev')
    hungarian.last_status = st
    check_match_status(st, 'hungarian')
    cx, cy = cx[:, :, None], cy[:, None, :]
    return (m[0], cx[0], cy[0]) if two_d else (m, cx, cy)
  w = _np32(weights)
  w3 = w[None] if two_d else w
  B, N, M = w3.shape
  m = np.zeros_like(w3)
  cx = np.zeros((B, N), np.float32)
  cy = np.zeros((B, M), np.float32)
  rc = rn.lib().ra_hungarian_f32(ptr(w3), B, N, M, ptr(m), ptr(cx), ptr(cy))
  if rc < 0:
    check(rc, 'ra_hungarian_f32')
  hungarian.last_status = rc
  cx, cy = cx[:, :, None], cy[:, None, :]
  if two_d:
    m, cx, cy = m[0], cx[0], cy[0]
  if is_t:
    return torch.from_numpy(m), torch.from_numpy(cx), torch.from_numpy(cy)
  return m, cx, cy


hungarian.last_status = 0


def check_match_status(status, what='Hungarian'):
  if status is None or isinstance(status, int):
    worst, capped = (status or 0), (status == 1)
  else:
    worst = int(status.min().item())
    capped = bool((status == 1).any().item())
  if worst < 0:
    raise rn.RecAttendError('%s: the matching solver stopped with code %d (an iteration cap the '
                            'reference aborts on, hungarian.cc LOG(FATAL))' % (what, worst))
  if capped:
    import warnings
    warnings.warn('%s: outer iteration cap reached, partial matching returned (hungarian.cc:363-377)'
                  % what)


STAT_NAMES = ('loss', 'box_loss', 'segm_loss', 'conf_loss', 'iou_soft', 'iou_soft_box',
              'wt_cov_soft', 'unwt_cov_soft', 'iou_hard', 'wt_cov_hard', 'unwt_cov_hard', 'dice',
              'count_acc', 'dic', 'dic_abs')


def pair_stats(a, b, want=('iou_soft', 'iou_hard', 'dice_hard', 'sum_a', 'sum_b'), a_tmajor=False):
  a, b = a.contiguous(), b.contiguous()
  _need_cuda(a, b)
  if a_tmajor:
    N, B, H, W = a.shape
  else:
    B, N, H, W = a.shape
  M = b.shape[1]
  dev = a.device
  n = rn.lib().ra_pair_stats_workspace_floats(B, H * W)
  ws = torch.empty((n,), dtype=torch.float32, device=dev)
  out = {}
  for k, shp in (('iou_soft', (B, N, M)), ('iou_hard', (B, N, M)), ('dice_hard', (B, N, M)),
                 ('sum_a', (B, N)), ('sum_b', (B, M)), ('inter', (B, N, M)), ('sum_a_hard', (B, N))):
    out[k] = torch.empty(shp, dtype=torch.float32, device=dev) if k in want else None
  if a_tmajor:
    check(rn.lib().ra_pair_stats_strided_f32(ptr(a), H * W, B * H * W, ptr(b), B, N, M, H * W, ptr(ws), n, ptr(out['iou_soft']),
                                             ptr(out['iou_hard']), ptr(out['dice_hard']), ptr(out['sum_a']), ptr(out['sum_b']),
                                             ptr(out['inter']), ptr(out['sum_a_hard']), rn.stream_ptr()), 'ra_pair_stats_strided_f32')
    return out
  check(rn.lib().ra_pair_stats_f32(ptr(a), ptr(b), B, N, M, H * W, ptr(ws), n, ptr(out['iou_soft']),
                                   ptr(out['iou_hard']), ptr(out['dice_hard']), ptr(out['sum_a']),
                                   ptr(out['sum_b']), ptr(out['inter']), ptr(out['sum_a_hard']),
                                   rn.stream_ptr()), 'ra_pair_stats_f32')
  return out


def gt_box(y_gt, padding_ratio, min_padding, want_box=True, want_ws=False):
  y_gt = y_gt.contiguous()
  _need_cuda(y_gt)
  B, T, H, W = y_gt.shape
  params = torch.empty((B, T, 8), dtype=torch.float32, device=y_gt.device)
  box = torch.empty((B, T, H, W), dtype=torch.float32, device=y_gt.device) if want_box else None
  n = rn.lib().ra_gt_box_workspace_floats(B, T)
  ws = torch.empty((n,), dtype=torch.float32, device=y_gt.device)
  check(rn.lib().ra_gt_box_f32(ptr(y_gt), B, T, H, W, C.c_float(padding_ratio),
                               C.c_float(min_padding), ptr(ws), n, ptr(params), ptr(box),
                               rn.stream_ptr()), 'ra_gt_box_f32')
  return (params, box, ws) if want_ws else (params, box)


def knob_setup(gt_ws, B, T, pad, shift, u_box, u_segm, sched, min_padding, timescale):
  pad, shift, u_box, u_segm, sched = (t.contiguous() for t in (pad, shift, u_box, u_segm, sched))
  _need_cuda(gt_ws, pad, shift, u_box, u_segm, sched)
  dev = gt_ws.device
  ctr, size = torch.empty((B, T, 2), dtype=torch.float32, device=dev), torch.empty((B, T, 2), dtype=torch.float32, device=dev)
  kb, ks = torch.empty((B, T, 1), dtype=torch.float32, device=dev), torch.empty((B, T, 1), dtype=torch.float32, device=dev)
  check(rn.lib().ra_knob_setup_f32(ptr(gt_ws), B, T, ptr(pad), ptr(shift), ptr(u_box), ptr(u_segm), ptr(sched), C.c_float(min_padding),
                                   int(bool(timescale)), ptr(ctr), ptr(size), ptr(kb), ptr(ks), rn.stream_ptr()), 'ra_knob_setup_f32')
  return ctr, size, kb, ks


def box_iou_rects(box, params):
  box, params = box.contiguous(), params.contiguous()
  _need_cuda(box, params)
  B, H, W = box.shape
  T = params.shape[1]
  out = torch.empty((B, T), dtype=torch.float32, device=box.device)
  ws = torch.empty((rn.lib().ra_box_iou_rects_workspace_floats(B),), dtype=torch.float32, device=box.device)
  check(rn.lib().ra_box_iou_rects_f32(ptr(box), ptr(params), B, T, H, W, ptr(ws), ws.numel(), ptr(out), rn.stream_ptr()),
        'ra_box_iou_rects_f32')
  return out


def segm_match(iou, s_gt):
  iou, s_gt = iou.contiguous(), s_gt.contiguous()
  _need_cuda(iou, s_gt)
  B, N, _ = iou.shape
  nb = rn.lib().ra_segm_match_workspace_bytes(B, N)
# ... 1104 lines not shown
```

Before: 62240 instance-timesteps/s.

## Spread output prefill across timesteps via pair16 rider and use split-precision fill-cache pair

Moves the y_out prefill from one whole-tensor store in the first encoder pair to per-timestep slices carried by the pair16 conv kernel, so each step writes only its own slice. It also lets the uncached fill-cache pair8 kernel use the split-precision layer B variant, holding layer-A weights and scale/shift in LDS instead of registers. The rider logic is factored into a shared RiderDeal helper. This spreads the fill traffic across steps and may ease register pressure, at the cost of extra LDS use and more complex launch selection.

After: 62630 instance-timesteps/s, median of 6. About the same (+0.6%).

```diff
diff --git a/include/recattend.h b/include/recattend.h
--- a/include/recattend.h
+++ b/include/recattend.h
@@ -179,6 +179,10 @@
 int ra_conv_pair16_f32(const float *x, int B, int H, int W, const float *wpA, const float *scaleA, const float *shiftA,
                        int reluA, const float *wpB, const float *scaleB, const float *shiftB, int reluB, float *y,
                        void *stream);
+int ra_conv_pair16_rider_f32(const float *x, int B, int H, int W, const float *wpA, const float *scaleA, const float *shiftA,
+                             int reluA, const float *wpB, const float *scaleB, const float *shiftB, int reluB, float *y,
+                             float *fill_dst, size_t fill_batch_stride, size_t fill_floats_per_image, float fill_value,
+                             void *stream);
 
 int ra_conv_first_cache_supported(int Cin, int CoutA, int CoutB, int poolB, int H, int W);
 size_t ra_conv_first_cache_floats(int B, int H, int W);
@@ -190,6 +194,11 @@
                                 const float *shiftB, int CoutB, int reluB, float *cache, float *y,
                                 void *stream);
 int ra_conv_pair_fill_cache_rider_f32(const float *src, const float *plane, int plane_chan, int B, int H, int W,
+                                      const float *wpA, const float *scaleA, const float *shiftA, int reluA,
+                                      const float *wpB, const float *scaleB, const float *shiftB, int CoutB,
+                                      int reluB, float *cache, float *y, float *fill_dst, size_t fill_floats,
+                                      float fill_value, void *stream);
+int ra_conv_pair_fill_cache_split_f32(const float *src, const float *plane, int plane_chan, int B, int H, int W,
                                       const float *wpA, const float *scaleA, const float *shiftA, int reluA,
                                       const float *wpB, const float *scaleB, const float *shiftB, int CoutB,
                                       int reluB, float *cache, float *y, float *fill_dst, size_t fill_floats,
diff --git a/rec-attend-public_amd/csrc/ra_conv_pair.hip b/rec-attend-public_amd/csrc/ra_conv_pair.hip
--- a/rec-attend-public_amd/csrc/ra_conv_pair.hip
+++ b/rec-attend-public_amd/csrc/ra_conv_pair.hip
@@ -553,9 +553,9 @@
   if (!plan) return fail(RA_E_INVALID, "ra_conv_pair_plan: bad argument");
   for (int i = 0; i < RA_PLAN_INTS; ++i) plan[i] = 0;
   static float mark;
-  if (cache_form == 1)
+  if (cache_form == 1 || cache_form == 3)
     return cpair::fill_cache_entry(nullptr, &mark, 3, B, Hs, Ws, nullptr, nullptr, nullptr, 0, nullptr, nullptr, nullptr, CoutB, 0, nullptr, nullptr,
-                                   nullptr, 0, 0.0f, nullptr, plan);
+                                   nullptr, 0, 0.0f, cache_form == 3, nullptr, plan);
   if (cache_form == 2)
     return cpair::cached_entry(nullptr, &mark, 3, B, Hs, Ws, nullptr, nullptr, nullptr, 0, nullptr, nullptr, nullptr, CoutB, 0, nullptr, nullptr, plan);
   if (cache_form) return fail(RA_E_INVALID, "ra_conv_pair_plan: cache_form %d", cache_form);
diff --git a/rec-attend-public_amd/csrc/ra_conv_pair16.hip b/rec-attend-public_amd/csrc/ra_conv_pair16.hip
--- a/rec-attend-public_amd/csrc/ra_conv_pair16.hip
+++ b/rec-attend-public_amd/csrc/ra_conv_pair16.hip
@@ -1,5 +1,5 @@
-#include "ra_common.h"
 #include "ra_split3.h"
+#include "ra_conv_pair_parts.h"
 
 #ifndef RA_PAIR16_OCC
 #define RA_PAIR16_OCC 3
@@ -24,6 +24,9 @@
   int bytes_x;
   int xcd_map;
   unsigned *tickets;
+  float *rider_dst;
+  int rider_quads, rider_stride_quads;
+  float rider_val;
 };
 
 struct P16Walk {
@@ -163,6 +166,9 @@
     tile = tk.cur >= 0 ? tk.cur : t_end;
   }
   if (tile < t_end) fetch(tile);
+  RiderDeal<true> rd;
+  rd.begin(a.rider_dst, a.rider_quads, a.B, a.rider_stride_quads, a.rider_val,
+           dyn ? (ntiles + (int)gridDim.x - 1) / (int)gridDim.x : (tw.end > tw.first ? (tw.end - tw.first + tw.step - 1) / tw.step : 1), a.y);
   RA_PHASE_DECL;
   for (; tile < t_end; tile = tnext) {
     const int b = tile / per, trem = tile - b * per;
@@ -193,6 +199,7 @@
       tnext = tile + tw.step;
     }
     if (tnext < t_end) fetch(tnext);
+    rd.tile();
 
     {
       const int oyA = ty * TSY - 1, oxA = tx * TS - 1;
@@ -277,6 +284,7 @@
     }
   }
   RA_PHASE_END;
+  rd.finish();
 }
 
 int launch_pair16(const P16Args &a, hipStream_t st, int *plan) {
@@ -312,12 +320,17 @@
 }
 
 static int pair16_entry(const float *x, int B, int H, int W, const float *wpA, const float *scaleA, const float *shiftA, int reluA,
-                        const float *wpB, const float *scaleB, const float *shiftB, int reluB, float *y, void *stream, int *plan) {
+                        const float *wpB, const float *scaleB, const float *shiftB, int reluB, float *y, float *fill_dst,
+                        size_t fill_batch_stride, size_t fill_floats_per_image, float fill_value, void *stream, int *plan) {
   if ((!plan && (!x || !wpA || !scaleA || !shiftA || !wpB || !scaleB || !shiftB || !y)) || B <= 0)
     return fail(RA_E_INVALID, "ra_conv_pair16_f32: bad argument");
   if (!ra_conv_pair16_supported(8, 16, 16, 2, H, W)) return fail(RA_E_SHAPE, "ra_conv_pair16_f32: %dx%d", H, W);
   const size_t bytes = (size_t)B * H * W * 8 * sizeof(float);
   if (bytes >= (1ull << 31)) return fail(RA_E_SHAPE, "ra_conv_pair16_f32: input exceeds 2 GiB");
+  const bool rider = fill_dst && fill_floats_per_image;
+  if (rider && ((reinterpret_cast<uintptr_t>(fill_dst) & 15) || (fill_floats_per_image & 3) || (fill_batch_stride & 3) ||
+                fill_batch_stride < fill_floats_per_image || ((size_t)B + 1) * fill_batch_stride * 4 >= (1ull << 31)))
+    return fail(RA_E_SHAPE, "ra_conv_pair16_rider_f32: the fill must be 16-byte aligned, blocks and stride multiples of 4 floats, < 2 GiB");
   cpair::P16Args a{};
   a.x = x;
   a.wpA = wpA;
@@ -335,18 +348,30 @@
   a.reluB = reluB;
   a.bytes_x = (int)bytes;
   a.xcd_map = 0;
+  a.rider_dst = rider ? fill_dst : nullptr;
+  a.rider_quads = rider ? (int)(fill_floats_per_image / 4) : 0;
+  a.rider_stride_quads = rider ? (int)(fill_batch_stride / 4) : 0;
+  a.rider_val = fill_value;
   return cpair::launch_pair16(a, as_stream(stream), plan);
+}
+
+extern "C" int ra_conv_pair16_rider_f32(const float *x, int B, int H, int W, const float *wpA, const float *scaleA, const float *shiftA,
+                                        int reluA, const float *wpB, const float *scaleB, const float *shiftB, int reluB, float *y,
+                                        float *fill_dst, size_t fill_batch_stride, size_t fill_floats_per_image, float fill_value,
+                                        void *stream) {
+  return pair16_entry(x, B, H, W, wpA, scaleA, shiftA, reluA, wpB, scaleB, shiftB, reluB, y, fill_dst, fill_batch_stride,
+                      fill_floats_per_image, fill_value, stream, nullptr);
 }
 
 extern "C" int ra_conv_pair16_f32(const float *x, int B, int H, int W, const float *wpA, const float *scaleA, const float *shiftA,
                                   int reluA, const float *wpB, const float *scaleB, const float *shiftB, int reluB, float *y,
                                   void *stream) {
-  return pair16_entry(x, B, H, W, wpA, scaleA, shiftA, reluA, wpB, scaleB, shiftB, reluB, y, stream, nullptr);
+  return ra_conv_pair16_rider_f32(x, B, H, W, wpA, scaleA, shiftA, reluA, wpB, scaleB, shiftB, reluB, y, nullptr, 0, 0, 0.0f, stream);
 }
 
 extern "C" int ra_conv_pair16_plan(int B, int H, int W, int *plan) {
   if (!plan) return fail(RA_E_INVALID, "ra_conv_pair16_plan: bad argument");
   for (int i = 0; i < RA_PLAN_INTS; ++i) plan[i] = 0;
   if (!plan_have_device()) return fail(RA_E_INVALID, "ra_conv_pair16_plan: the grid follows the device's CU count and occupancy: no device");
-  return pair16_entry(nullptr, B, H, W, nullptr, nullptr, nullptr, 0, nullptr, nullptr, nullptr, 0, nullptr, nullptr, plan);
-}
+  return pair16_entry(nullptr, B, H, W, nullptr, nullptr, nullptr, 0, nullptr, nullptr, nullptr, 0, nullptr, nullptr, 0, 0, 0.0f, nullptr, plan);
+}
diff --git a/rec-attend-public_amd/csrc/ra_conv_pair8.hip b/rec-attend-public_amd/csrc/ra_conv_pair8.hip
--- a/rec-attend-public_amd/csrc/ra_conv_pair8.hip
+++ b/rec-attend-public_amd/csrc/ra_conv_pair8.hip
@@ -56,8 +56,12 @@
     return SPLIT ? 3 * PLANE_B / 4 : AHS * AW * 8;
   }
   template <bool CACHED, bool SPLIT>
+  static constexpr int wa_floats() {
+    return (!CACHED && SPLIT) ? 12 * NCGA * 64 + 16 : 0;
+  }
+  template <bool CACHED, bool SPLIT>
   static constexpr int lds_floats() {
-    return tin_floats<CACHED>() + tmid_floats<SPLIT>();
+    return tin_floats<CACHED>() + tmid_floats<SPLIT>() + wa_floats<CACHED, SPLIT>();
   }
 };
 static_assert(NGeo<4>::map_exact() && NGeo<8>::map_exact(), "phase A's groups cover the 18 x 18 pair-rows exactly once");
@@ -81,13 +85,15 @@
   using G = NGeo<CINA>;
   constexpr int NCGA = G::NCGA;
   static_assert(!CACHED || CINA == 4, "cached form: 4 input channels");
-  static_assert(!SPLIT || CACHED, "the split-precision layer B exists for the cached (steady-state) form");
+  static_assert(!SPLIT || CINA == 4, "the split-precision layer B exists for the first pair's two forms (4 input channels)");
   constexpr int PLANE_B = G::PLANE_B;
   constexpr int RECA = CACHED ? 1 : CINA;
   extern __shared__ __attribute__((aligned(16))) float lds[];
   constexpr int IN_FLOATS = G::template tin_floats<CACHED>();
   float *tin = lds;
   float *tmid = lds + IN_FLOATS;
+  constexpr bool WLDS = G::template wa_floats<CACHED, SPLIT>() > 0;
+  float *twa = tmid + G::template tmid_floats<SPLIT>();
   typedef typename vec_of<NCGA>::type avecA;
 
   const int tid = threadIdx.x, lane = tid & 63;
@@ -107,8 +113,11 @@
   f32x4 scA4, shA4;
 #pragma unroll
   for (int j = 0; j < 4; ++j) scA4[j] = a.scA[coA0 + j], shA4[j] = a.shA[coA0 + j];
+  if constexpr (WLDS) {
+    if (tid < 16) twa[12 * NCGA * 64 + tid] = (tid & 4) ? a.shA[4 * (tid >> 3) + (tid & 3)] : a.scA[4 * (tid >> 3) + (tid & 3)];
+  }
   const bool fill = !CACHED && a.cache != nullptr;
-  float bA[CACHED ? 1 : 12][NCGA], bB[12][2];
+  float bA[(CACHED || WLDS) ? 1 : 12][NCGA], bB[12][2];
   float bAc[3];
 #pragma unroll
   for (int ky = 0; ky < 3; ++ky) {
@@ -129,7 +138,12 @@
 #pragma unroll
         for (int cg = 0; cg < NCGA; ++cg) {
           const float w = a.wpA[((tap * NCGA + cg) * 4 + ksub) * a.CoutAP + co];
-          bA[ky * 4 + kxp][cg] = ok ? w * (fill ? 1.f : scA) : 0.f;
+          const float wv = ok ? w * (fill ? 1.f : scA) : 0.f;
+          if constexpr (WLDS) {
+            if (tid < 64) twa[((ky * 4 + kxp) * NCGA + cg) * 64 + lane] = wv;
+          } else {
+            bA[ky * 4 + kxp][cg] = wv;
+          }
         }
       }
 #pragma unroll
@@ -283,18 +297,11 @@
   TC cur = split(have ? tile : 0), nxt = cur;
   if (have) fetch(cur);
   RA_PHASE_DECL;
-  for (int e = tid; e < G::template lds_floats<CACHED, SPLIT>() / 4; e += 256)
+  for (int e = tid; e < (G::template lds_floats<CACHED, SPLIT>() - G::template wa_floats<CACHED, SPLIT>()) / 4; e += 256)
     reinterpret_cast<f32x4 *>(lds)[e] = f32x4{0.f, 0.f, 0.f, 0.f};
   __syncthreads();
-  const bool rider = !CACHED && a.rider_dst != nullptr;
-  const __amdgpu_buffer_rsrc_t rr = __builtin_amdgcn_make_buffer_rsrc(rider ? a.rider_dst : a.y, 0,
-                                                                       rider ? a.rider_quads * 16 : 0, 0x00020000);
-  const int r_chunk = rider ? (a.rider_quads + (int)gridDim.x - 1) / (int)gridDim.x : 0;
-  int r_idx = (int)blockIdx.x * r_chunk + tid;
-  const int r_end = ((int)blockIdx.x + 1) * r_chunk < a.rider_quads ? ((int)blockIdx.x + 1) * r_chunk : a.rider_quads;
-  const int my_tiles = t_end > t_first ? (t_end - t_first + nwx - 1) / nwx : 1;
-  const int r_per_tile = (r_chunk + 256 * my_tiles - 1) / (256 * my_tiles);
-  const u32x4 r_bits = __builtin_bit_cast(u32x4, f32x4{a.rider_val, a.rider_val, a.rider_val, a.rider_val});
+  RiderDeal<false> rd;
+  if constexpr (!CACHED) rd.begin(a.rider_dst, a.rider_quads, 1, 0, a.rider_val, t_end > t_first ? (t_end - t_first + nwx - 1) / nwx : 1, a.y);
   bool have_n = false;
   f32x4 cpre[CACHED ? G::NSLOT : 1];
   LaneCell cell_c{};
@@ -355,11 +362,7 @@
       nxt = advance(cur);
     }
     if (have_n) fetch(nxt);
-    if constexpr (!CACHED) {
-      if (rider)
-        for (int u = 0; u < r_per_tile; ++u, r_idx += 256)
-          __builtin_amdgcn_raw_buffer_store_b128(r_bits, rr, r_idx < r_end ? r_idx * 16 : 0x7fffffff, 0, 0);
-    }
+    if constexpr (!CACHED) rd.tile();
 
     {
       const bool interior = (ty0 >= 1) & (ty0 + G::TH + 1 <= a.H) & (tx0 >= 2) & (tx0 + G::TW + 1 <= a.W);
@@ -368,14 +371,19 @@
         constexpr int S0 = decltype(s0c)::value, NS = decltype(s1c)::value - S0;
         f32x4 acc[NS];
         int gin[NS];
+        f32x4 sc4 = scA4, sh4 = shA4;
+        if constexpr (WLDS) {
+          sc4 = *reinterpret_cast<const f32x4 *>(&twa[12 * NCGA * 64 + 2 * coA0]);
+          sh4 = *reinterpret_cast<const f32x4 *>(&twa[12 * NCGA * 64 + 2 * coA0 + 4]);
+        }
 #pragma unroll
         for (int s = 0; s < NS; ++s) gin[s] = S0 + s < 4 ? cell_i.in + 4 * (S0 + s) * G::LW * RECA : edge.in;
 #pragma unroll
         for (int s = 0; s < NS; ++s) {
           if constexpr (CACHED) {
-            acc[s] = cpre[S0 + s] * scA4 + shA4;
+            acc[s] = cpre[S0 + s] * sc4 + sh4;
           } else {
-            acc[s] = fill ? f32x4{0.f, 0.f, 0.f, 0.f} : shA4;
+            acc[s] = fill ? f32x4{0.f, 0.f, 0.f, 0.f} : sh4;
           }
         }
         if constexpr (S0 == 0) RA_PHASE_AT(1);
@@ -399,10 +407,13 @@
               for (int s = 0; s < NS; ++s)
                 av[s] = *reinterpret_cast<const avecA *>(&tin[gin[s] + (ky * G::LW + kxp) * CINA]);
 #pragma unroll
-              for (int cg = 0; cg < NCGA; ++cg)
-#pragma unroll
-                for (int s = 0; s < NS; ++s)
-                  acc[s] = __builtin_amdgcn_mfma_f32_16x16x4f32(bA[ky * 4 + kxp][cg], av[s][cg], acc[s], 0, 0, 0);
+              for (int cg = 0; cg < NCGA; ++cg) {
+                float wv;
+                if constexpr (WLDS) wv = twa[((ky * 4 + kxp) * NCGA + cg) * 64 + lane];
+                else wv = bA[ky * 4 + kxp][cg];
+#pragma unroll
+                for (int s = 0; s < NS; ++s) acc[s] = __builtin_amdgcn_mfma_f32_16x16x4f32(wv, av[s][cg], acc[s], 0, 0, 0);
+              }
             }
         }
 #pragma unroll
@@ -413,7 +424,7 @@
           if (fill) {
             const int off = live ? tile_c + (inner ? S * rows4_c + cell_i.c : edge.c) : 0x7fffffff;
             __builtin_amdgcn_raw_buffer_store_b128(__builtin_bit_cast(__attribute__((ext_vector_type(4))) unsigned, acc[s]), rc, off, 0, 0);
-            acc[s] = acc[s] * scA4 + shA4;
+            acc[s] = acc[s] * sc4 + sh4;
           }
           float o[4];
 #pragma unroll
@@ -521,10 +532,7 @@
     RA_PHASE_AT(4);
   }
   RA_PHASE_END;
-  if constexpr (!CACHED) {
-    if (rider)
-      for (; r_idx < r_end; r_idx += 256) __builtin_amdgcn_raw_buffer_store_b128(r_bits, rr, r_idx * 16, 0, 0);
-  }
+  if constexpr (!CACHED) rd.finish();
 }
 
 template <int CINA, bool CACHED = false, bool SPLIT = false>
@@ -608,7 +616,7 @@
 
 int fill_cache_entry(const float *src, const float *plane, int plane_chan, int B, int H, int W, const float *wpA, const float *scaleA,
                      const float *shiftA, int reluA, const float *wpB, const float *scaleB, const float *shiftB, int CoutB, int reluB,
-                     float *cache, float *y, float *fill_dst, size_t fill_floats, float fill_value, void *stream, int *plan) {
+                     float *cache, float *y, float *fill_dst, size_t fill_floats, float fill_value, int splitB, void *stream, int *plan) {
   if (missing_pointer(plan, {src, plane, cache, wpA, scaleA, shiftA, wpB, scaleB, shiftB, y}) || B <= 0)
     return fail(RA_E_INVALID, "ra_conv_pair_fill_cache_f32: bad argument");
   if (fill_dst && ((reinterpret_cast<uintptr_t>(fill_dst) & 15) || (fill_floats & 3) || fill_floats * 4 >= (1ull << 31)))
@@ -623,6 +631,8 @@
   a.rider_dst = fill_floats ? fill_dst : nullptr;
   a.rider_quads = (int)(fill_floats / 4);
   a.rider_val = fill_value;
+  static const int split_all = env_int("RA_PAIR8_SPLIT", 1);
+  if (splitB && split_all) return launch8<4, false, true>(a, B, as_stream(stream), plan);
   return launch8<4, false>(a, B, as_stream(stream), plan);
 }
 
@@ -676,7 +686,16 @@
                                                  int reluB, float *cache, float *y, float *fill_dst, size_t fill_floats,
                                                  float fill_value, void *stream) {
   return cpair::fill_cache_entry(src, plane, plane_chan, B, H, W, wpA, scaleA, shiftA, reluA, wpB, scaleB, shiftB, CoutB, reluB, cache, y,
-                                 fill_dst, fill_floats, fill_value, stream, nullptr);
+                                 fill_dst, fill_floats, fill_value, 0, stream, nullptr);
+}
+
+extern "C" int ra_conv_pair_fill_cache_split_f32(const float *src, const float *plane, int plane_chan, int B, int H, int W,
+                                                 const float *wpA, const float *scaleA, const float *shiftA, int reluA,
+                                                 const float *wpB, const float *scaleB, const float *shiftB, int CoutB,
+                                                 int reluB, float *cache, float *y, float *fill_dst, size_t fill_floats,
+                                                 float fill_value, void *stream) {
+  return cpair::fill_cache_entry(src, plane, plane_chan, B, H, W, wpA, scaleA, shiftA, reluA, wpB, scaleB, shiftB, CoutB, reluB, cache, y,
+                                 fill_dst, fill_floats, fill_value, 1, stream, nullptr);
 }
 
 extern "C" int ra_conv_pair_fill_cache_f32(const float *src, const float *plane, int plane_chan, int B, int H, int W,
diff --git a/rec-attend-public_amd/csrc/ra_conv_pair_parts.h b/rec-attend-public_amd/csrc/ra_conv_pair_parts.h
--- a/rec-attend-public_amd/csrc/ra_conv_pair_parts.h
+++ b/rec-attend-public_amd/csrc/ra_conv_pair_parts.h
@@ -3,6 +3,7 @@
 #include <initializer_list>
 
 #include "ra_common.h"
+#include "ra_split3.h"
 
 namespace ra {
 namespace cpair {
@@ -70,6 +71,49 @@
   return a;
 }
 
+template <bool STRIDED>
+struct RiderDeal {
+  __amdgpu_buffer_rsrc_t rr;
+  int idx, end, per_tile;
+  int in_blk, blk_off;
+  int blk_quads, stride_b;
+  float val;
+  __device__ __forceinline__ void begin(float *dst, int blk_quads_, int nblk, int stride_quads, float val_, int my_tiles,
+                                        float *idle) {
+    const bool on = dst != nullptr;
+    const int total = on ? blk_quads_ * nblk : 0;
+    rr = __builtin_amdgcn_make_buffer_rsrc(on ? dst : idle, 0, on ? ((nblk - 1) * stride_quads + blk_quads_) * 16 : 0, 0x00020000);
+    const int chunk = (total + (int)gridDim.x - 1) / (int)gridDim.x;
+    idx = (int)blockIdx.x * chunk + (int)threadIdx.x;
+    end = ((int)blockIdx.x + 1) * chunk < total ? ((int)blockIdx.x + 1) * chunk : total;
+    per_tile = (chunk + 256 * my_tiles - 1) / (256 * my_tiles);
+    val = val_;
+    if constexpr (STRIDED) {
+      blk_quads = on ? blk_quads_ : 1;
+      stride_b = stride_quads * 16;
+      const int blk = idx / blk_quads;
+      in_blk = idx - blk * blk_quads;
+      blk_off = blk * stride_b;
+    }
+  }
+  __device__ __forceinline__ void store() {
+    const u32x4 bits = __builtin_bit_cast(u32x4, f32x4{val, val, val, val});
+    const int off = STRIDED ? blk_off + in_blk * 16 : idx * 16;
+    __builtin_amdgcn_raw_buffer_store_b128(bits, rr, idx < end ? off : 0x7fffffff, 0, 0);
+    idx += 256;
+    if constexpr (STRIDED) {
+      in_blk += 256;
+      while (in_blk >= blk_quads) in_blk -= blk_quads, blk_off += stride_b;
+    }
+  }
+  __device__ __forceinline__ void tile() {
+    for (int u = 0; u < per_tile; ++u) store();
+  }
+  __device__ __forceinline__ void finish() {
+    while (idx < end) store();
+  }
+};
+
 void cache_dims(int H, int W, int &rows, int &ngx);
 
 inline int pair_args_cache(PArgs &a, const float *cache, int B, const char *what) {
@@ -84,7 +128,7 @@
 int launch_npacked(const PArgs &a, int B, hipStream_t st, int *plan);
 int fill_cache_entry(const float *src, const float *plane, int plane_chan, int B, int H, int W, const float *wpA, const float *scaleA,
                      const float *shiftA, int reluA, const float *wpB, const float *scaleB, const float *shiftB, int CoutB, int reluB,
-                     float *cache, float *y, float *fill_dst, size_t fill_floats, float fill_value, void *stream, int *plan);
+                     float *cache, float *y, float *fill_dst, size_t fill_floats, float fill_value, int splitB, void *stream, int *plan);
 int cached_entry(const float *cache, const float *plane, int plane_chan, int B, int H, int W, const float *wpA, const float *scaleA,
                  const float *shiftA, int reluA, const float *wpB, const float *scaleB, const float *shiftB, int CoutB, int reluB,
                  float *y, void *stream, int *plan);
diff --git a/rec-attend-public_amd/ra_engine.py b/rec-attend-public_amd/ra_engine.py
--- a/rec-attend-public_amd/ra_engine.py
+++ b/rec-attend-public_amd/ra_engine.py
@@ -40,11 +40,13 @@
     self.use_wino = True
     self.cache_first = True
     self.fill_cache_inline = True
+    self.fill_cache_split = os.environ.get('RA_PAIR8_FILL_SPLIT', '1') != '0'
     self.co_resident = 1
     self.tile_tickets = os.environ.get('RA_ENGINE_TICKETS', '0') != '0'
     self.nsub = 0
     self.use_graph = True
     self.prefill_ride = True
+    self.prefill_slices = os.environ.get('RA_PREFILL_SLICES', '1') != '0'
     self.use_split = os.environ.get('RA_USE_SPLIT', '1') != '0'
     self.split_first = os.environ.get('RA_SPLIT_FIRST', '1') != '0'
     self.ctrl_batch_xcd = os.environ.get('RA_CTRL_BATCH_XCD', '1') != '0'
@@ -401,14 +403,31 @@
         ops.tickets_unbind()
 
   def _launch_encoder(self, b, tt):
-    fill = b['y_out'] if (tt == 0 and b.pop('_fill_rider', False)) else None
+    ride = b.get('_fill_rider')
     return self._run_cnn(self.plan['ccnn'], self.W['ccnn'], b['img'], b['ccnn'], tt, 'ctrl_cnn',
-                         plane=b['canvas'], cache=b.get('l0cache'), fill=fill)
+                         plane=b['canvas'], cache=b.get('l0cache'), fill=b['y_out'] if (ride == 'whole' and tt == 0) else None,
+                         fill_slice=b['y_out'][:, tt] if ride == 'slices' else None)
 
   def _prefill_rides(self, b):
     st0 = self.plan['ccnn'][0]
     return (self.prefill_ride and 'l0cache' in b and self.fill_cache_inline and st0[0] == 'pair' and
             ops.fill_rider_ok(b['y_out']))
+
+  def _pair16_step(self, b):
+    if not (self.pair_direct16 and self.pair_wino):
+      return None
+    src = b['img']
+    for step in self.plan['ccnn']:
+      if step[0] == 'pair':
+        (_, _, _, ca, _), (_, _, _, cb, poolb) = self.W['ccnn'][step[1]], self.W['ccnn'][step[2]]
+        if step[1] != 0 and ops.conv_pair16_supported(src.shape[3], ca, cb, poolb, src.shape[1], src.shape[2]):
+          return step
+      src = b['ccnn'][step[2] if step[0] == 'pair' else step[1]]
+    return None
+
+  def _prefill_slices(self, b):
+    return (self.prefill_slices and self._prefill_rides(b) and ops.fill_slices_ok(b['y_out']) and
+            self._pair16_step(b) is not None)
 
   def _launch_pack(self, b):
     if self._prepacked:
@@ -417,10 +436,15 @@
       ops.pack_input(b['x'], b.get('d_in'), b.get('y_in'), self.d['C0p'], b['img'],
                      canvas_plane=b['canvas'])
     if not self.box and not self.d['disable_overwrite']:
-      if self._prefill_rides(b):
-        b['_fill_rider'] = True
+      b['_fill_rider'] = None
+      if self._prefill_slices(b):
+        b['_fill_rider'] = 'slices'
+      elif self._prefill_rides(b):
+        b['_fill_rider'] = 'whole'
       else:
         ops.fill(b['y_out'], 1.0 / (1.0 + math.exp(5.0)))
+    else:
+      b['_fill_rider'] = None
     if 'l0cache' in b and not self.fill_cache_inline:
       ops.first_cache(b['img'], self.W['ccnn'][0][0], self.d['ccnn_channels'][1], self.d['D'], b['l0cache'])
     self._mark('pack')
@@ -495,7 +519,8 @@
                        b['y_out'].data_ptr() + tt * H * W * 4, T * H * W, H, W, canvas=b['canvas'], flags=flags)
     self._mark('paste')
 
-  def _run_cnn(self, steps, layers, src, bufs, tt, name, plane=None, cache=None, fill=None):
+  def _run_cnn(self, steps, layers, src, bufs, tt, name, plane=None, cache=None, fill=None, fill_slice=None):
+    fv = 1.0 / (1.0 + math.exp(5.0))
     pc = self.d['D'] if plane is not None else -1
     ks = self.ksize['acnn'] if layers is self.W.get('acnn') else self.ksize['ccnn']
     for step in steps:
@@ -504,12 +529,13 @@
         (wpa, sca, sha, ca, _), (wpb, scb, shb, cb, poolb) = layers[step[1]], layers[step[2]]
         if cache is not None and pl is not None and tt == 0 and self.fill_cache_inline:
           ops.conv_pair_fill_cache(src, pl, pc, wpa, sca[tt], sha[tt], wpb, scb[tt], shb[tt], cb, cache, bufs[step[2]],
-                                   fill=fill, fill_value=1.0 / (1.0 + math.exp(5.0)))
+                                   fill=fill, fill_value=fv, split=self.fill_cache_split)
         elif cache is not None and pl is not None:
           ops.conv_pair_cached(cache, pl, pc, wpa, sca[tt], sha[tt], wpb, scb[tt], shb[tt], cb, bufs[step[2]])
         elif (self.pair_direct16 and self.pair_wino and layers is self.W.get('ccnn') and pl is None and
               ops.conv_pair16_supported(src.shape[3], ca, cb, poolb, src.shape[1], src.shape[2])):
-          ops.conv_pair16(src, wpa, sca[tt], sha[tt], wpb, scb[tt], shb[tt], out=bufs[step[2]])
+          ops.conv_pair16(src, wpa, sca[tt], sha[tt], wpb, scb[tt], shb[tt], out=bufs[step[2]], fill=fill_slice, fill_value=fv)
+          fill_slice = None
         elif (self.use_wino and self.pair_wino and layers is self.W.get('ccnn') and pl is None and
               self.W['ccnn_wino'][step[2]] is not None and
               ops.conv_pair_wino_supported(src.shape[3], ca, cb, poolb, src.shape[1], src.shape[2])):
diff --git a/rec-attend-public_amd/ra_ops.py b/rec-attend-public_amd/ra_ops.py
--- a/rec-attend-public_amd/ra_ops.py
+++ b/rec-attend-public_amd/ra_ops.py
@@ -736,12 +736,27 @@
   return bool(rn.lib().ra_conv_pair16_supported(int(cin), int(cout_a), int(cout_b), int(pool_b), int(H), int(W)))
 
 
-def conv_pair16(x, wpA, scA, shA, wpB, scB, shB, reluA=True, reluB=True, out=None):
+def fill_slices_ok(t):
+  if t.dim() < 2 or not t.is_contiguous() or t.data_ptr() % 16:
+    return False
+  per = t[0, 0].numel()
+  return per % 4 == 0 and t.stride(0) % 4 == 0 and (t.shape[0] + 1) * t.stride(0) * 4 < (1 << 31)
+
+
+def conv_pair16(x, wpA, scA, shA, wpB, scB, shB, reluA=True, reluB=True, out=None, fill=None, fill_value=0.0):
   _need_cuda(x, wpA, scA, shA, wpB, scB, shB, out)
   B, H, W, _ = x.shape
   out = _conv_out(x, 16, 2, out=out)
-  check(rn.lib().ra_conv_pair16_f32(ptr(x), B, H, W, ptr(wpA), ptr(scA), ptr(shA), int(reluA), ptr(wpB), ptr(scB), ptr(shB),
-                                    int(reluB), ptr(out), rn.stream_ptr()), 'ra_conv_pair16_f32')
+  if fill is None:
+    check(rn.lib().ra_conv_pair16_f32(ptr(x), B, H, W, ptr(wpA), ptr(scA), ptr(shA), int(reluA), ptr(wpB), ptr(scB), ptr(shB),
+                                      int(reluB), ptr(out), rn.stream_ptr()), 'ra_conv_pair16_f32')
+    return out
+  per = fill[0].numel()
+  if (not fill.is_cuda or fill.dtype != torch.float32 or fill.shape[0] != B or not fill[0].is_contiguous() or fill.data_ptr() % 16 or per % 4 or fill.stride(0) % 4 or fill.stride(0) < per):
+    raise rn.RecAttendError('conv_pair16: the rider fill needs one contiguous, 16-byte aligned block of 4k floats per image')
+  check(rn.lib().ra_conv_pair16_rider_f32(ptr(x), B, H, W, ptr(wpA), ptr(scA), ptr(shA), int(reluA), ptr(wpB), ptr(scB), ptr(shB),
+                                          int(reluB), ptr(out), ptr(fill), fill.stride(0), per, C.c_float(fill_value),
+                                          rn.stream_ptr()), 'ra_conv_pair16_rider_f32')
   return out
 
 
@@ -792,17 +807,18 @@
 
 
 def conv_pair_fill_cache(img, plane, plane_chan, wpA, scA, shA, wpB, scB, shB, coutB, cache, out, reluA=True, reluB=True,
-                         fill=None, fill_value=0.0):
+                         fill=None, fill_value=0.0, split=False):
   _need_cuda(img, plane, wpA, scA, shA, wpB, scB, shB, cache, out, fill)
   B, H, W = plane.shape
   if fill is not None and not fill_rider_ok(fill):
     raise rn.RecAttendError('conv_pair_fill_cache: the rider fill needs a contiguous, 16-byte aligned tensor of 4k floats < 2 GiB')
-  check(rn.lib().ra_conv_pair_fill_cache_rider_f32(ptr(img), ptr(plane), int(plane_chan), B, H, W, ptr(wpA), ptr(scA),
+  name = 'ra_conv_pair_fill_cache_split_f32' if split else 'ra_conv_pair_fill_cache_rider_f32'
+  check(getattr(rn.lib(), name)(ptr(img), ptr(plane), int(plane_chan), B, H, W, ptr(wpA), ptr(scA),
                                                    ptr(shA), int(reluA), ptr(wpB), ptr(scB), ptr(shB), int(coutB),
                                                    int(reluB), ptr(cache), ptr(out), ptr(fill),
                                                    0 if fill is None else fill.numel(), C.c_float(fill_value),
                                                    rn.stream_ptr()),
-        'ra_conv_pair_fill_cache_rider_f32')
+        name)
   return out
 
 
```
